# hsinnan75/Dart

Hardware: AMD Instinct MI355X
Metric: M paired-end reads/sec (2x101 bp vs GRCh38-sized index), host to host; records bit-identical to CPU dart (higher is better)
Workload: dtype u64/u8 integer

## Files before the change

dart_amd/csrc/dg_api.hip:

```cpp
#include "../../include/dartgpu.h"
#include "dg_common.h"
#include "dg_fm.h"
#include "dg_seedq.h"
#include "dg_chain.h"
#include "dg_report.h"
#include "dg_pair.h"
#include "dg_reseed.h"
#include "dg_sort.h"
#include "dg_samfmt.h"
#include <stdio.h>
#include <stdlib.h>
#include <string.h>
#include <string>
#include <algorithm>
#include <vector>
#include <atomic>
#include <mutex>
#include <chrono>
#include <thread>
#include <condition_variable>
#include <fcntl.h>
#include <unistd.h>
#include <sys/stat.h>

static char g_init_error[512] = "";

#define DG_HW_QUEUES_NEED 16
static_assert(DG_HW_QUEUES_NEED <= 32, "more hardware queues than 32 are not asked for");
static char g_hwq_found[24] = "unset";
static int g_hwq_left = DG_HW_QUEUES_NEED;
__attribute__((constructor)) static void dg_default_hw_queues()
{
    const char *v = getenv("GPU_MAX_HW_QUEUES");
    long have = 0;
    if (v) {
        size_t i = 0;
        for (; v[i] && i + 1 < sizeof g_hwq_found; i++) g_hwq_found[i] = (v[i] > ' ' && v[i] < 127 && v[i] != ';' && v[i] != '=') ? v[i] : '?';
        g_hwq_found[i] = 0;
        if (!i) snprintf(g_hwq_found, sizeof g_hwq_found, "empty");
        char *end = nullptr;
        have = strtol(v, &end, 10);
        if (end == v || *end) have = 0; else if (have > 1000000) have = 1000000;
    }
    if (have < DG_HW_QUEUES_NEED) {
        char b[8];
        snprintf(b, sizeof b, "%d", DG_HW_QUEUES_NEED);
        setenv("GPU_MAX_HW_QUEUES", b, 1);
        have = DG_HW_QUEUES_NEED;
    }
    g_hwq_left = (int)have;
}
static std::atomic<int> g_live_ctx[64];
static std::atomic<bool> g_hwq_warned{false};

template <typename T> struct DBuf {
    T *p = nullptr; size_t cap = 0;
    hipError_t ensure(size_t n) {
        if (n <= cap) return hipSuccess;
        if (p) (void)hipFree(p);
        p = nullptr; cap = 0;
        size_t want = n + n / 8 + 64;
        hipError_t e = hipMalloc((void **)&p, want * sizeof(T));
        if (e == hipSuccess) cap = want;
        return e;
    }
    void release() { if (p) (void)hipFree(p); p = nullptr; cap = 0; }
};

#define N_TIMERS 20
#define N_TOPS 128
enum { TOP_CIG = 0, TOP_SJ, TOP_JOBS, TOP_REPORT_MAIN, TOP_REPORT_JOBS , TOP_HEAVY_UNITS, TOP_SEED_NEXT, TOP_SEED_HEAVY,
       TOP_WORK = 16, TOP_TICKET_PAIR = 17, TOP_TICKET_EMIT = 18, TOP_RESEED_COUNT = 19 , TOP_RESEED_TICKET = 23 , TOP_TICKET_SEED = 26, TOP_RS_POOL = 27, TOP_RS_OUT = 31,
       TOP_ORDER_INFO = 28 , TOP_CLASS_HIST = 32 , TOP_CLASS_FILL = 64  };

struct IndexShared {
    std::mutex mu;
    std::condition_variable cv;
    DIndex ix{};
    std::atomic<uint32_t> gen{1};
    std::thread aids;
    std::atomic<int> aids_state{0};
    char aids_msg[256] = "";
    bool upload_done = false, upload_ok = false;
    void *d_ktab = nullptr, *d_sa_dense = nullptr;
    std::string report, report_out;
    int device = 0;
    uint32_t *d_chr_name_off = nullptr; char *d_chr_names = nullptr; bool chr_names_set = false; uint64_t chr_names_gen = 0;
};

struct dg_ctx {
    int device = 0;
    IndexShared *shared_ix = nullptr; uint32_t ix_gen = 0;
    bool owns_index = true;
    hipStream_t stream = nullptr;
    hipEvent_t ev_dl = nullptr, ev_dl_block = nullptr;
    bool dl_on_copy_stream = false;
    int env_copy_stream = 1;
    hipEvent_t ev_wait = nullptr;
    char err[512] = "";
    DIndex ix{};
    DParams pr{};
    void *d_bwt = nullptr, *d_sa = nullptr, *d_pac = nullptr, *d_lockey = nullptr, *d_locchr = nullptr, *d_chroff = nullptr;
    int n_reads = 0, max_rlen = 0;
    size_t seq_bytes = 0;
    bool enc_ready = false;
    DBuf<unsigned char> seq; DBuf<uint32_t> seq_off; DBuf<uint16_t> rlen; DBuf<uint32_t> enc; DBuf<uint32_t> packed_in, nlist_in;
    DBuf<DHit> hits; DBuf<uint32_t> nhits, nseeds, seed_off, ncand, rep_off, tile_sums, tile_read, slow_units;
    DBuf<SKey> seeds; DBuf<DSeed> work; DBuf<DCand> cands; DBuf<DJob> jobs; DBuf<unsigned long long> job_items, job_pool; DBuf<RsChunkOut> job_outs; DBuf<uint32_t> job_pool_next; DBuf<unsigned long long> items; DBuf<uint32_t> hist, heavy; DBuf<DHeavy> seed_heavy; DBuf<int32_t> seed_heavy_sfail; DBuf<int16_t> chain_picks; DBuf<uint8_t> chain_todo;
    DBuf<dg_read_out> reads_out; DBuf<dg_report_out> reports; DBuf<uint32_t> cigpool, cigfinal;
    DBuf<dg_sj_out> sjpool, sjfinal;
    DBuf<dg_read_c> reads_c; DBuf<dg_report_c> reports_c; DBuf<uint32_t> cig_c;
    DBuf<unsigned char> ws;
    DBuf<unsigned long long> scan_state, scan_trace;
    int wall_khz = 100000;
    uint32_t scan_epoch = 0;
    size_t cap_seeds = 0, cap_rep = 0, cap_work = 0, cap_cig = 0;
    struct SharedCaps { std::atomic<size_t> seeds{0}, rep{0}, work{0}, cig{0}; } *shared_caps = nullptr;
    bool owns_shared_caps = false;
    unsigned long long *d_ctr = nullptr; unsigned int *d_tops = nullptr; int *d_err = nullptr; DSizes *d_sizes = nullptr; unsigned int *d_input_bad = nullptr;
    struct HostTail { DSizes sizes; int err; unsigned int input_bad; unsigned int tops[N_TOPS]; unsigned long long ctr[CTR_STRIDE]; __host__ __device__ uint32_t *sizes_words() { return (uint32_t *)&sizes; } } *h_tail = nullptr;
    bool state_zeroed = false;
    size_t used[3] = {0, 0, 0};
    bool enqueued = false;
    hipEvent_t ev[N_TIMERS + 1]; const char *tname[N_TIMERS]; int n_t = 0; float tms[N_TIMERS];
    uint64_t counters[CTR_N];
    uint64_t reruns_capacity = 0, reruns_scan = 0;
    bool want_compact = true, packed_valid = false;
    DBuf<uint32_t> sam_hdr_off, sam_qual_off, sam_qlen; DBuf<char> sam_hdr, sam_qual, sam_text; DBuf<uint64_t> sam_read_off, sam_tile;
    unsigned long long *d_sam_stat = nullptr, *h_sam_stat = nullptr;
    hipEvent_t ev_sam[2] = {nullptr, nullptr};
    bool batch_done = false, sam_valid = false; size_t sam_bytes = 0;
    size_t env_sam_first_cap = 0;
    bool want_full = true, full_valid = false;
    int n_cu = 256, runs_of_last_batch = 0, attempt_no = 0;
    int env_seed_waves = 4, env_bail_trips = 0 , env_report_bpc = 8, env_no_fast = 0, env_seed_legacy = 0, env_seed_slots_lg = 0, env_seed_wgs = 0, env_blocking_sync = 0;
    int env_seed_phases = 0, env_seed_wg_waves = 4, env_seed_partial = 32, env_seed_multi = 4;
    bool seed_qf_used = false;
    int env_scan_mask = 7;
    int env_chain_bpc = 8, env_seedh_bpc = 8, env_reseed_pct = 100;
    int env_rs_chunk = RS_CHUNK_DIAGS, env_rs_inline = RS_ENT_INLINE, env_rs_pool = 0;
    int env_scan_budget = 0;
};

static void read_env(dg_ctx *c)
{
    auto geti = [](const char *k, int dflt) { const char *v = getenv(k); return v ? atoi(v) : dflt; };
    c->env_seed_waves = geti("DG_SEED_WAVES", 4); c->env_bail_trips = geti("DG_SEED_BAIL_TRIPS", 0);
    c->env_seed_legacy = geti("DG_SEED_LEGACY", 0); c->env_seed_slots_lg = geti("DG_SEED_SLOTS_LG", 0); c->env_seed_wgs = geti("DG_SEED_WGS", 0); c->env_blocking_sync = geti("DG_BLOCKING_SYNC", 0);
    c->env_report_bpc = geti("DG_REPORT_BPC", 8); c->env_no_fast = geti("DG_NO_FAST_PAIR", 0);
    c->env_scan_budget = geti("DG_SCAN_POLL_BUDGET", 0); c->env_scan_mask = geti("DG_SCAN_POLL_SCANS", 7);
    c->env_seed_phases = geti("DG_SEED_PHASES", 0); c->env_seed_wg_waves = geti("DG_SEED_WG_WAVES", 4); c->env_seed_partial = geti("DG_SEED_PARTIAL_MIN", 32);
    c->env_copy_stream = geti("DG_COPY_STREAM", 1);
    c->env_chain_bpc = std::max(1, geti("DG_CHAIN_BPC", 8)); c->env_seedh_bpc = std::max(1, geti("DG_SEEDH_BPC", 8)); c->env_reseed_pct = std::max(10, geti("DG_RESEED_PCT", 100));
    c->env_rs_chunk = geti("DG_RS_CHUNK", RS_CHUNK_DIAGS); c->env_rs_chunk = std::min(1 << 24, std::max(RS_SUPER, c->env_rs_chunk / RS_SUPER * RS_SUPER));
    c->env_rs_inline = std::min(RS_ENT_INLINE, std::max(0, geti("DG_RS_ENT_MAX", RS_ENT_INLINE))); c->env_rs_pool = std::max(0, geti("DG_RS_POOL_BLOCKS", 0));
    c->env_sam_first_cap = (size_t)std::max(0, geti("DG_SAM_TEXT_FIRST_CAP", 0));
    c->env_seed_multi = geti("DG_SEED_MULTI", 4); if (c->env_seed_multi < 0 || c->env_seed_multi > SQF_MULTI_MAX) c->env_seed_multi = SQF_MULTI_MAX;
}

static inline void refresh_index(dg_ctx *c)
{
    IndexShared *sh = c->shared_ix;
    if (sh && c->ix_gen != sh->gen.load(std::memory_order_acquire)) { std::lock_guard<std::mutex> lk(sh->mu); c->ix = sh->ix; c->ix_gen = sh->gen.load(); }
}

static int fail(dg_ctx *c, int code, const char *what, hipError_t e)
{
    snprintf(c ? c->err : g_init_error, 512, "%s: %s", what, e == hipSuccess ? "error" : hipGetErrorString(e));
    return code;
}
#define HIPCHK(call) do { hipError_t _e = (call); if (_e != hipSuccess) return fail(c, DG_ERR_HIP, #call, _e); } while (0)

#define SCAN_TILE 2048
__global__ void __launch_bounds__(256) k_scan_tiles(const uint32_t *in, uint32_t *out, uint32_t *tile_sums, uint32_t n)
{
    __shared__ uint32_t sh[256];
    const uint32_t base = blockIdx.x * SCAN_TILE + threadIdx.x * 8;
    uint32_t v[8], sum = 0;
    for (int i = 0; i < 8; i++) { v[i] = base + i < n ? in[base + i] : 0; sum += v[i]; }
    sh[threadIdx.x] = sum;
    __syncthreads();
    for (int o = 1; o < 256; o <<= 1) {
        uint32_t t = threadIdx.x >= o ? sh[threadIdx.x - o] : 0;
        __syncthreads();
        sh[threadIdx.x] += t;
        __syncthreads();
    }
    uint32_t run = sh[threadIdx.x] - sum;
    for (int i = 0; i < 8; i++) { if (base + i < n) out[base + i] = run; run += v[i]; }
    if (threadIdx.x == 255) tile_sums[blockIdx.x] = sh[255];
}
__global__ void __launch_bounds__(256) k_scan_top(uint32_t *tile_sums, uint32_t n_tiles, uint32_t *total_out, uint32_t *total_copy, uint32_t cap, int *err, int code)
{
    __shared__ uint32_t sh[256];
    __shared__ uint32_t carry;
    if (threadIdx.x == 0) carry = 0;
    __syncthreads();
    for (uint32_t b = 0; b < n_tiles; b += 256) {
        const uint32_t i = b + threadIdx.x;
        const uint32_t v = i < n_tiles ? tile_sums[i] : 0;
        sh[threadIdx.x] = v;
        __syncthreads();
        for (int o = 1; o < 256; o <<= 1) {
            uint32_t t = threadIdx.x >= o ? sh[threadIdx.x - o] : 0;
            __syncthreads();
            sh[threadIdx.x] += t;
            __syncthreads();
        }
        if (i < n_tiles) tile_sums[i] = carry + sh[threadIdx.x] - v;
        __syncthreads();
        if (threadIdx.x == 255) carry += sh[255];
        __syncthreads();
    }
    if (threadIdx.x == 0) {
        *total_out = carry;
        if (total_copy) *total_copy = carry;
        if (err && carry > cap) atomicMax(err, code);
    }
}
__global__ void __launch_bounds__(256) k_scan_add(uint32_t *out, const uint32_t *tile_sums, uint32_t n)
{
    const uint32_t i = blockIdx.x * 256 + threadIdx.x;
    if (i < n) out[i] += tile_sums[i / SCAN_TILE];
}

#define SO_PER 8
__global__ void __launch_bounds__(256)
k_seed_offsets(int n_reads, int paired, const uint32_t *__restrict__ nseeds, uint32_t *__restrict__ seed_off, uint32_t *__restrict__ tile_read, uint32_t n_tile_read,
               uint32_t *__restrict__ heavy_list, unsigned int *n_heavy, uint32_t *total_copy, uint32_t cap, TileScan ts, int *err)
{
    __shared__ unsigned long long s_scan[20];
    __shared__ unsigned int s_tile;
    const unsigned int tile = d_tile_ticket_unless(ts, &s_tile, threadIdx.x == 0 && __hip_atomic_load(err, __ATOMIC_RELAXED, __HIP_MEMORY_SCOPE_AGENT) >= DG_ABORT);
    if (tile == SCAN_LEAVE) return;
    const uint32_t first = tile * (256u * SO_PER) + threadIdx.x * SO_PER;
    uint32_t v[SO_PER], sum = 0;
    if (first + SO_PER <= (uint32_t)n_reads) {
        const uint4 a = *(const uint4 *)(nseeds + first), b = *(const uint4 *)(nseeds + first + 4);
        v[0] = a.x; v[1] = a.y; v[2] = a.z; v[3] = a.w; v[4] = b.x; v[5] = b.y; v[6] = b.z; v[7] = b.w;
    } else {
#pragma unroll
        for (int i = 0; i < SO_PER; i++) v[i] = first + i < (uint32_t)n_reads ? nseeds[first + i] : 0u;
    }
#pragma unroll
    for (int i = 0; i < SO_PER; i++) sum += v[i];
    Triple mine, tot;
    mine.x = sum; mine.y = 0; mine.z = 0; mine.w = 0;
    const Triple inb = d_block_exclusive(mine, tot, s_scan);
    const Triple base = d_tile_exclusive(ts, tile, tot, s_scan + 16, err);
    uint32_t run = base.x + inb.x;
    const int lane = threadIdx.x & 63;
#pragma unroll
    for (int i = 0; i < SO_PER; i++) {
        const uint32_t r = first + i;
        if (r < (uint32_t)n_reads) {
            seed_off[r] = run;
            for (uint32_t t = (run + 63u) >> 6; (t << 6) < run + v[i] && t < n_tile_read; t++) tile_read[t] = r;
        }
        const bool unit_end = paired ? (i & 1) == 1 : true;
        const uint32_t useeds = paired ? ((i & 1) ? v[i - ((i & 1) ? 1 : 0)] + v[i] : 0u) : v[i];
        const bool heavy = unit_end && r < (uint32_t)n_reads && useeds > (uint32_t)UNIT_MAX_SEEDS;
        const unsigned long long m = __ballot(heavy);
        if (m) {
            unsigned int hb = 0;
            const int leader = __ffsll((long long)m) - 1;
            if (lane == leader) hb = atomicAdd(n_heavy, (unsigned int)__popcll(m));
            hb = (unsigned int)__shfl((int)hb, leader, 64);
            if (heavy) heavy_list[hb + (unsigned int)__popcll(m & ((1ull << lane) - 1ull))] = paired ? r >> 1 : r;
        }
        run += v[i];
    }
    if (tile == gridDim.x - 1 && threadIdx.x == 0) {
        const uint32_t total = base.x + tot.x;
        seed_off[n_reads] = total;
        if (total_copy) *total_copy = total;
        if (total > cap) atomicMax(err, DG_E_SEEDS);
    }
}

static std::atomic<uint64_t> g_phase_ns[4];
static void caps_publish(std::atomic<size_t> &a, size_t v) { size_t cur = a.load(); while (cur < v && !a.compare_exchange_weak(cur, v)) { } }
static void caps_adopt(size_t &mine, const std::atomic<size_t> &a) { const size_t v = a.load(); if (v > mine) mine = v; }
static std::mutex g_copy_mu[64];
static hipStream_t g_copy_stream[64][2];
static hipError_t copy_stream(int device, int dir, hipStream_t *out)
{
    hipStream_t &sl = g_copy_stream[device & 63][dir];
    if (!sl) {
        int lo = 0, hi = 0;
        hipError_t e = hipDeviceGetStreamPriorityRange(&lo, &hi);
        if (e == hipSuccess) e = hipStreamCreateWithPriority(&sl, hipStreamNonBlocking, hi);
        if (e != hipSuccess) { sl = nullptr; return e; }
    }
    *out = sl;
    return hipSuccess;
}

static bool host_page_locked(const void *p)
{
    if (!p) return false;
    hipPointerAttribute_t a;
    if (hipPointerGetAttributes(&a, p) != hipSuccess) { (void)hipGetLastError(); return false; }
    return a.type == hipMemoryTypeHost;
}

static hipError_t wait_stream(dg_ctx *c)
{
    if (!c->env_blocking_sync || !c->ev_wait) return hipStreamSynchronize(c->stream);
    const hipError_t e = hipEventRecord(c->ev_wait, c->stream);
    return e != hipSuccess ? e : hipEventSynchronize(c->ev_wait);
}

#ifdef DG_PROFILE_CLASSES
__device__ unsigned long long g_class_cycles[DG_COST_CLASSES + 1], g_class_chunks[DG_COST_CLASSES + 1];
#endif
template <int MINW>
__global__ void __launch_bounds__(64, MINW)
k_report(const DIndex ix, const DParams pr, int n_reads, int paired, const unsigned char *__restrict__ seq,
         const uint32_t *__restrict__ seq_off, const uint16_t *__restrict__ rlen, const uint32_t *__restrict__ seed_off,
         const DJob *__restrict__ jobs, DCand *__restrict__ cands,
         const uint32_t *__restrict__ rep_off, DSeed *__restrict__ work, const unsigned long long *__restrict__ items,
         const uint32_t *__restrict__ n_items_p, dg_report_out *__restrict__ reports, uint32_t *cigpool, uint32_t cigcap,
         unsigned int *tops, unsigned char *ws, const WSLayout L, unsigned long long *ctr, int *err)
{
    const unsigned long long t_wave0 = wall_clock64();
    const int lane = blockIdx.x * blockDim.x + threadIdx.x;
    __shared__ uint32_t lds_pm[64 * PM_LDS_WORDS];
    if (*err >= DG_ABORT) return;
    LaneCtx cx;
#ifdef DG_PROFILE_CLASSES
    __shared__ unsigned long long ph_acc[DG_NCLS * DG_NPHASE], cls_acc[2 * DG_NCLS];
    for (int q = threadIdx.x; q < DG_NCLS * DG_NPHASE; q += 64) ph_acc[q] = 0;
    for (int q = threadIdx.x; q < 2 * DG_NCLS; q += 64) cls_acc[q] = 0;
    __syncthreads();
    cx.ph = ph_acc;
#endif
    cx.lds = lds_pm + (threadIdx.x & 63) * PM_LDS_WORDS;
    cx.ix = &ix; cx.pr = &pr; cx.L = &L;
    cx.ws = ws + (size_t)lane * L.stride;
    cx.n_nw = cx.nw_cells = cx.n_reseed = cx.reseed_w = 0;
    const unsigned int lo = 0u, hi = *n_items_p;
    unsigned int *next = tops + TOP_REPORT_MAIN;
    while (true) {
        unsigned int ticket = 0;
        if ((threadIdx.x & 63) == 0) ticket = atomicAdd(next, 1u);
        ticket = (unsigned int)__shfl((int)ticket, 0, 64);
        const unsigned int base = lo + ticket * 64u;
        if (base >= hi) break;
        const unsigned int idx = base + (threadIdx.x & 63);
        const bool valid = idx < hi;
        const unsigned long long item = valid ? items[idx] : 0ull;
        const int r = (int)(item >> 32);
        const uint32_t ci = (uint32_t)item, rep_i = valid ? rep_off[r] + (ci - seed_off[r]) : 0u;
        DRead rd;
        rd.sub_score = 0; rd.mis_num = 0; rd.mapq = 0;
        cx.seq = seq + seq_off[r]; cx.rlen = rlen[r];
#ifdef DG_PROFILE_CLASSES
        const long long t_begin = clock64();
        cx.cls = (int)(cands[(uint32_t)items[base]].final_n & 31); cx.t_last = t_begin;
#endif
        d_gen_mapping_report(cx, valid, paired ? (r & 1) == 0 : true, rd, cands + ci, valid ? 1 : 0, jobs, work,
                             reports + rep_i, rep_i, cigpool, tops + 0, cigcap, err, 0, 1, true);
#ifdef DG_PROFILE_CLASSES
        if ((threadIdx.x & 63) == 0) { cls_acc[cx.cls] += (unsigned long long)(clock64() - t_begin); cls_acc[DG_NCLS + cx.cls] += 1ull; }
#endif
    }
#ifdef DG_PROFILE_CLASSES
    __syncthreads();
    for (int q = threadIdx.x; q < DG_NCLS * DG_NPHASE; q += 64) if (ph_acc[q]) atomicAdd(&g_phase[q / DG_NPHASE][q % DG_NPHASE], ph_acc[q]);
    if (threadIdx.x < DG_NCLS && cls_acc[DG_NCLS + threadIdx.x]) { atomicAdd(&g_class_cycles[threadIdx.x], cls_acc[threadIdx.x]); atomicAdd(&g_class_chunks[threadIdx.x], cls_acc[DG_NCLS + threadIdx.x]); }
#endif
    d_wave_add(ctr + CTR_NW, cx.n_nw);
    d_wave_add(ctr + CTR_NWCELLS, cx.nw_cells);
    d_wave_add(ctr + CTR_RESEED, cx.n_reseed);
    d_wave_add(ctr + CTR_RESEEDW, cx.reseed_w);
    d_wave_resident(ctr, CTR_WT_REPORT, t_wave0);
}

__global__ void __launch_bounds__(256)
k_finalize(const DIndex ix, const DParams pr, int paired, const uint32_t *__restrict__ slow_units, const DSizes *__restrict__ sizes,
           const uint32_t *__restrict__ seed_off, const DCand *__restrict__ cands, const uint32_t *__restrict__ ncand, const uint32_t *__restrict__ rep_off, const DSeed *__restrict__ work,
           dg_read_out *__restrict__ rout, dg_report_out *__restrict__ reports, dg_sj_out *sjpool, uint32_t sjcap, unsigned int *tops, int *err)
{
    if (*err >= DG_ABORT) return;
    const unsigned int n_units = sizes->n_slow_units;
    for (unsigned int it = blockIdx.x * blockDim.x + threadIdx.x; it < n_units; it += gridDim.x * blockDim.x) {
        const int u = (int)slow_units[it];
        const int nm = paired ? 2 : 1;
        DRead rd[2];
        dg_read_out o[2];
        RepMem<dg_report_out> rp[2];
        for (int m = 0; m < nm; m++) {
            const int r = paired ? 2 * u + m : u;
            const int nc = (int)ncand[r];
            dg_report_out *rep = reports + rep_off[r];
            rd[m].score = 0; rd[m].sub_score = 0; rd[m].mis_num = 0; rd[m].mapq = 0; rd[m].iBest = 0; rd[m].CanNum = nc > 0 ? nc : 1;
            for (int i = 0; i < nc; i++) {
                const int aln = rep[i].aln_score, mis_num = rep[i].flag;
                if (mis_num) rep[i].flag = 0;
                if (aln <= 0) continue;
                if (aln > rd[m].score) { rd[m].iBest = i; rd[m].mis_num = mis_num; rd[m].sub_score = rd[m].score; rd[m].score = aln; }
                else if (aln == rd[m].score) rd[m].sub_score = rd[m].score;
            }
            o[m].score = rd[m].score; o[m].sub_score = rd[m].sub_score; o[m].mis_num = rd[m].mis_num; o[m].mapq = 0;
            o[m].n_rep = rd[m].CanNum; o[m].best = rd[m].iBest; o[m].rep_off = (int32_t)rep_off[r]; o[m].sj_off = 0; o[m].n_sj = 0;
            rp[m].p = rep;
        }
        if (paired) {
            d_settle_pair(pr, rd[0], rp[0], rd[1], rp[1]);
            d_flag_pair(rd[0], rp[0], rd[1], rp[1]);
        } else d_flag_single(rd[0], rp[0]);
        for (int m = 0; m < nm; m++) {
            const int r = paired ? 2 * u + m : u;
            d_mapq(rd[m], rp[m]);
            o[m].score = rd[m].score; o[m].mapq = rd[m].mapq; o[m].best = rd[m].iBest;
            if (ncand[r] > 0 && (rd[m].mapq == 50 || (pr.all_sj && rd[m].score > 0)))
                d_collect_sj(ix, pr, cands[seed_off[r] + rd[m].iBest], work, r, sjpool, tops + TOP_SJ, sjcap, o[m].sj_off, o[m].n_sj, err);
            rout[r] = o[m];
        }
    }
}

__global__ void __launch_bounds__(256)
k_emit_slow(int paired, const uint32_t *__restrict__ slow_units, DSizes *sizes, dg_read_out *__restrict__ rout, dg_report_out *__restrict__ reports,
            const uint32_t *__restrict__ cigpool, uint32_t *__restrict__ cigfinal, uint32_t cap_cig, const dg_sj_out *__restrict__ sjpool, dg_sj_out *__restrict__ sjfinal,
            TileScan ts, int *err, const uint16_t *__restrict__ rlen, const CompactOut co)
{
    __shared__ unsigned long long s_scan[20];
    __shared__ unsigned int s_tile;
    bool leave = false;
    if (threadIdx.x == 0) { const int e0 = __hip_atomic_load(err, __ATOMIC_RELAXED, __HIP_MEMORY_SCOPE_AGENT); leave = e0 >= DG_ABORT && e0 != DG_E_CIGFINAL; }
    const unsigned int tile = d_tile_ticket_unless(ts, &s_tile, leave);
    if (tile == SCAN_LEAVE) return;
    const unsigned int n_items = sizes->n_slow_units * (paired ? 2u : 1u);
    if (tile > 0 && tile * 256u >= n_items) return;
    const unsigned int it = tile * 256u + threadIdx.x;
    const bool on = it < n_items;
    const int r = on ? (paired ? (int)(2u * slow_units[it >> 1] + (it & 1u)) : (int)slow_units[it]) : 0;
    dg_read_out o;
    o.n_rep = 0; o.rep_off = 0; o.n_sj = 0; o.sj_off = 0;
    if (on) o = rout[r];
    uint32_t ncig = 0, ncigc = 0;
    const uint32_t full_match = on ? (uint32_t)rlen[r] << 4 : 0u;
    for (int i = 0; i < (on ? o.n_rep : 0); i++) {
        const dg_report_out &rp = reports[o.rep_off + i];
        ncig += rp.n_cigar;
        if (co.reads) ncigc += (rp.n_cigar == 1u && cigpool[rp.cigar_off] == full_match) ? 0u : rp.n_cigar;
    }
    Triple mine, tot;
    mine.x = ncig; mine.y = on ? (uint32_t)o.n_sj : 0u; mine.z = 0; mine.w = ncigc;
    const Triple inb = d_block_exclusive(mine, tot, s_scan);
    const Triple base = d_tile_exclusive(ts, tile, tot, s_scan + 16, err);
    const uint32_t cig_fast = sizes->cig_fast, cigc_fast = sizes->pad[2];
    if (on) {
        uint32_t dst = cig_fast + base.x + inb.x, dstc = cigc_fast + base.w + inb.w;
        bool fits = true;
        if ((uint64_t)dst + ncig > cap_cig) atomicMax(err, DG_E_CIGFINAL);
        else for (int i = 0; i < o.n_rep; i++) {
            dg_report_out &rp = reports[o.rep_off + i];
            const uint32_t m = rp.n_cigar, src = rp.cigar_off;
            const bool plain = m == 1u && cigpool[src] == full_match;
            for (uint32_t k = 0; k < m; k++) cigfinal[dst + k] = cigpool[src + k];
            if (co.reads) {
                if (!plain) { for (uint32_t k = 0; k < m; k++) co.cigar[dstc + k] = cigpool[src + k]; dstc += m; }
                dg_report_c q; fits = d_compact_report(rp, plain, true, q) && fits; co.reports[o.rep_off + i] = q;
            }
            rp.cigar_off = dst; dst += m;
        }
        if (o.n_sj > 0) {
            const uint32_t sd = base.y + inb.y;
            for (int k = 0; k < o.n_sj; k++) sjfinal[sd + k] = sjpool[o.sj_off + k];
            rout[r].sj_off = (int32_t)sd;
        }
        if (co.reads) { dg_read_c oc; fits = d_compact_read(o, oc) && fits; co.reads[r] = oc; if (!fits) *co.bad = 1u; }
    }
    const unsigned int last = n_items ? (n_items - 1u) / 256u : 0u;
    if (tile == last && threadIdx.x == 0) { sizes->total_cig = cig_fast + base.x + tot.x; sizes->total_sj = base.y + tot.y; sizes->pad[0] = cigc_fast + base.w + tot.w; }
}

extern "C" void dg_params_default(dg_params *p)
{
    p->max_gaps = 5; p->max_dup = 100; p->max_intron = 500000; p->min_intron = 5;
    p->max_mismatch = 0; p->multi_hit = 0; p->all_sj = 0; p->paired = 0;
}

static void set_params(dg_ctx *c, const dg_params *p)
{
    c->pr.max_gaps = p->max_gaps; c->pr.max_dup = p->max_dup; c->pr.max_intron = p->max_intron; c->pr.min_intron = p->min_intron;
    c->pr.max_mismatch = p->max_mismatch; c->pr.multi_hit = p->multi_hit; c->pr.all_sj = p->all_sj; c->pr.paired = p->paired;
}

extern "C" int dg_set_params(dg_ctx *c, const dg_params *p)
{
    if (!c || !p) return DG_ERR_ARG;
    set_params(c, p);
    read_env(c);
    return DG_OK;
}

extern "C" int dg_device_count(void)
{
    int n = 0;
    return hipGetDeviceCount(&n) == hipSuccess ? n : 0;
}

extern "C" const char *dg_last_error(const dg_ctx *c) { return c ? c->err : g_init_error; }

extern "C" void dg_destroy(dg_ctx *c)
{
    if (!c) return;
    (void)hipSetDevice(c->device);
    if (c->stream) (void)hipStreamSynchronize(c->stream);
    if (c->owns_index && c->shared_ix) {
        IndexShared *sh = c->shared_ix;
        { std::lock_guard<std::mutex> lk(sh->mu); if (!sh->upload_done) { sh->upload_done = true; sh->upload_ok = false; } }
        sh->cv.notify_all();
        if (sh->aids.joinable()) sh->aids.join();
        if (sh->d_ktab) (void)hipFree(sh->d_ktab);
        if (sh->d_sa_dense) (void)hipFree(sh->d_sa_dense);
        if (sh->d_chr_name_off) (void)hipFree(sh->d_chr_name_off);
        if (sh->d_chr_names) (void)hipFree(sh->d_chr_names);
        delete sh; c->shared_ix = nullptr;
    }
    void *ptrs[] = { c->d_bwt, c->d_sa, c->d_pac, c->d_lockey, c->d_locchr, c->d_chroff };
    if (c->owns_index) for (void *p : ptrs) if (p) (void)hipFree(p);
    void *own[] = { c->d_ctr, c->d_tops, c->d_err, c->d_sizes, c->d_input_bad };
    for (void *p : own) if (p) (void)hipFree(p);
    if (c->h_tail) (void)hipHostFree(c->h_tail);
    c->seq.release(); c->seq_off.release(); c->rlen.release(); c->enc.release(); c->packed_in.release(); c->nlist_in.release(); c->hits.release(); c->nhits.release(); c->nseeds.release();
    c->seed_off.release(); c->ncand.release(); c->rep_off.release(); c->tile_sums.release(); c->tile_read.release(); c->slow_units.release();
    c->seeds.release(); c->work.release(); c->cands.release(); c->jobs.release(); c->job_items.release(); c->job_outs.release(); c->job_pool.release(); c->job_pool_next.release(); c->items.release(); c->hist.release(); c->heavy.release(); c->seed_heavy.release(); c->seed_heavy_sfail.release(); c->chain_picks.release(); c->chain_todo.release();
    c->reads_out.release(); c->reports.release(); c->cigpool.release(); c->cigfinal.release(); c->sjpool.release(); c->sjfinal.release();
    c->sam_hdr_off.release(); c->sam_qual_off.release(); c->sam_qlen.release(); c->sam_hdr.release(); c->sam_qual.release(); c->sam_text.release(); c->sam_read_off.release(); c->sam_tile.release();
    if (c->d_sam_stat) (void)hipFree(c->d_sam_stat);
    if (c->h_sam_stat) (void)hipHostFree(c->h_sam_stat);
    for (hipEvent_t e : c->ev_sam) if (e) (void)hipEventDestroy(e);
    c->ws.release(); c->scan_state.release(); c->scan_trace.release(); c->reads_c.release(); c->reports_c.release(); c->cig_c.release();
    for (int i = 0; i <= N_TIMERS; i++) if (c->ev[i]) (void)hipEventDestroy(c->ev[i]);
    if (c->ev_wait) (void)hipEventDestroy(c->ev_wait);
    if (c->ev_dl) (void)hipEventDestroy(c->ev_dl);
    if (c->ev_dl_block) (void)hipEventDestroy(c->ev_dl_block);
    if (c->stream) { (void)hipStreamDestroy(c->stream); g_live_ctx[c->device & 63].fetch_sub(1); }
    if (c->owns_shared_caps) delete c->shared_caps;
    delete c;
}

static hipError_t make_ctx_objects(dg_ctx *c)
{
    hipError_t e;
    for (int i = 0; i <= N_TIMERS; i++) c->ev[i] = nullptr;
    if ((e = hipStreamCreate(&c->stream)) != hipSuccess) return e;
    g_live_ctx[c->device & 63].fetch_add(1);
    if ((e = hipEventCreateWithFlags(&c->ev_wait, hipEventBlockingSync | hipEventDisableTiming)) != hipSuccess ||
        (e = hipEventCreateWithFlags(&c->ev_dl, hipEventDisableTiming)) != hipSuccess || (e = hipEventCreateWithFlags(&c->ev_dl_block, hipEventBlockingSync | hipEventDisableTiming)) != hipSuccess) return e;
    for (int i = 0; i <= N_TIMERS; i++) if ((e = hipEventCreate(&c->ev[i])) != hipSuccess) return e;
    if ((e = hipMalloc((void **)&c->d_ctr, CTR_STRIPES * CTR_STRIDE * 8)) != hipSuccess || (e = hipMalloc((void **)&c->d_tops, N_TOPS * 4)) != hipSuccess ||
        (e = hipMalloc((void **)&c->d_err, 4)) != hipSuccess || (e = hipMalloc((void **)&c->d_sizes, sizeof(DSizes))) != hipSuccess ||
        (e = hipMalloc((void **)&c->d_input_bad, 4)) != hipSuccess) return e;
    if ((e = hipHostMalloc((void **)&c->h_tail, sizeof(dg_ctx::HostTail), hipHostMallocDefault)) != hipSuccess) return e;
    memset(c->h_tail, 0, sizeof(dg_ctx::HostTail));
    { int khz = 0; if (hipDeviceGetAttribute(&khz, hipDeviceAttributeWallClockRate, c->device) == hipSuccess && khz > 0) c->wall_khz = khz; }
    read_env(c);
    return hipSuccess;
}

static double now_s() { return std::chrono::duration<double>(std::chrono::steady_clock::now().time_since_epoch()).count(); }

struct UpSrc { int fd = -1; const uint8_t *mem = nullptr; };
struct UpChunk { UpSrc src; uint64_t src_off; uint8_t *dst; size_t bytes; uint64_t relayout_blocks; };

static hipError_t upload_chunks(int device, const std::vector<UpChunk> &chunks, size_t chunk_cap, int n_threads, std::string &what)
{
    std::atomic<size_t> next{0};
    std::atomic<int> failed{0};
    std::mutex mu;
    hipError_t first = hipSuccess;
    auto fail_with = [&](hipError_t e, const char *w) { std::lock_guard<std::mutex> lk(mu); if (!failed.exchange(1)) { first = e == hipSuccess ? hipErrorUnknown : e; what = w; } };
    auto work = [&]() {
        hipError_t e;
        if ((e = hipSetDevice(device)) != hipSuccess) { fail_with(e, "hipSetDevice (index upload)"); return; }
        hipStream_t s = nullptr; uint8_t *pin[2] = {nullptr, nullptr}; hipEvent_t ev[2] = {nullptr, nullptr}; bool used[2] = {false, false};
        if ((e = hipStreamCreateWithFlags(&s, hipStreamNonBlocking)) != hipSuccess) { fail_with(e, "hipStreamCreate (index upload)"); return; }
        for (int b = 0; b < 2 && e == hipSuccess; b++) {
            if ((e = hipHostMalloc((void **)&pin[b], chunk_cap, hipHostMallocDefault)) == hipSuccess) e = hipEventCreateWithFlags(&ev[b], hipEventDisableTiming);
        }
        if (e != hipSuccess) fail_with(e, "page-locked staging buffers (index upload)");
        int b = 0;
        while (e == hipSuccess && !failed.load()) {
            const size_t i = next.fetch_add(1);
            if (i >= chunks.size()) break;
            const UpChunk &ch = chunks[i];
            if (used[b] && (e = hipEventSynchronize(ev[b])) != hipSuccess) { fail_with(e, "hipEventSynchronize (index upload)"); break; }
            if (ch.src.mem) memcpy(pin[b], ch.src.mem + ch.src_off, ch.bytes);
            else {
                size_t got = 0;
                while (got < ch.bytes) {
                    const ssize_t r = pread(ch.src.fd, pin[b] + got, ch.bytes - got, (off_t)(ch.src_off + got));
                    if (r <= 0) break;
                    got += (size_t)r;
                }
                if (got < ch.bytes) { fail_with(hipErrorUnknown, "an index file is shorter than its header says"); break; }
            }
            if (ch.bytes && (e = hipMemcpyAsync(ch.dst, pin[b], ch.bytes, hipMemcpyHostToDevice, s)) != hipSuccess) { fail_with(e, "hipMemcpyAsync (index upload)"); break; }
            if (ch.relayout_blocks) {
                k_relayout_bwt<<<(unsigned)((ch.relayout_blocks + 255) / 256), 256, 0, s>>>((uint4 *)ch.dst, ch.relayout_blocks);
                if ((e = hipGetLastError()) != hipSuccess) { fail_with(e, "k_relayout_bwt"); break; }
            }
            if ((e = hipEventRecord(ev[b], s)) != hipSuccess) { fail_with(e, "hipEventRecord (index upload)"); break; }
            used[b] = true; b ^= 1;
        }
        if (s && (e = hipStreamSynchronize(s)) != hipSuccess) fail_with(e, "index upload");
        for (int k = 0; k < 2; k++) { if (ev[k]) (void)hipEventDestroy(ev[k]); if (pin[k]) (void)hipHostFree(pin[k]); }
        if (s) (void)hipStreamDestroy(s);
    };
    std::vector<std::thread> th;
    for (int t = 0; t < n_threads; t++) th.emplace_back(work);
    for (auto &t : th) t.join();
    return failed.load() ? first : hipSuccess;
}

static void add_chunks(std::vector<UpChunk> &out, UpSrc src, uint64_t src_off, uint8_t *dst, size_t bytes, size_t chunk, bool relayout, uint64_t total_blocks)
{
    for (size_t o = 0; o < bytes || (relayout && o / 64 < total_blocks); o += chunk) {
        const size_t nb = o < bytes ? std::min(chunk, bytes - o) : 0;
        uint64_t rb = 0;
        if (relayout) { const uint64_t first = o / 64; rb = std::min<uint64_t>(chunk / 64, total_blocks > first ? total_blocks - first : 0); }
        out.push_back(UpChunk{src, src_off + o, dst + o, nb, rb});
    }
}

static void aids_thread(IndexShared *sh, int sa_file_intv, uint64_t n_sa, bool async, uint64_t expected_reads)
{
    auto failed = [&](const char *w, hipError_t e) {
        std::lock_guard<std::mutex> lk(sh->mu);
        snprintf(sh->aids_msg, sizeof sh->aids_msg, "%s: %s", w, hipGetErrorString(e));
        sh->aids_state.store(-1); sh->cv.notify_all();
    };
    hipError_t e;
    if ((e = hipSetDevice(sh->device)) != hipSuccess) return failed("hipSetDevice (aids)", e);
    DIndex ix;
    { std::lock_guard<std::mutex> lk(sh->mu); ix = sh->ix; }
    const uint64_t seq_len = ix.seq_len;
    double t0 = now_s();
    const bool lean = expected_reads != 0 && expected_reads < 400000000ull;
    int intv = seq_len <= (12ull << 30) ? 1 : (seq_len <= (24ull << 30) ? 2 : 4);
    if (lean && intv < 4) intv = 4;
    if (const char *v = getenv("DG_SA_DENSE")) intv = atoi(v);
    const bool want_dense = intv >= 1 && intv < sa_file_intv && (intv & (intv - 1)) == 0 && seq_len < (1ull << 39);
    const uint64_t n_entries = want_dense ? seq_len / (uint64_t)intv + 1 : 0;
    int K = 8;
    while (K < 16 && (1ull << (2 * K)) < seq_len) K++;
    if (lean && K > 14) K = 14;
    if (async) {
        std::unique_lock<std::mutex> lk(sh->mu);
        sh->cv.wait(lk, [&]() { return sh->upload_done; });
        if (!sh->upload_ok) { lk.unlock(); sh->aids_state.store(-1); sh->cv.notify_all(); return; }
    }
    if (want_dense && (e = hipMalloc(&sh->d_sa_dense, n_entries * 8)) != hipSuccess) return failed("hipMalloc dense SA", e);
    {
        size_t free_b = 0, total_b = 0;
        if (hipMemGetInfo(&free_b, &total_b) == hipSuccess)
            while (K > 8 && ((size_t)16 << (2 * K)) + ((size_t)48 << 30) > free_b) K--;
    }
    if (const char *v = getenv("DG_KTAB_K")) K = atoi(v);
    if (K > 16) K = 16;
    if (K >= 2 && (e = hipMalloc(&sh->d_ktab, ((size_t)16) << (2 * K))) != hipSuccess) return failed("hipMalloc k-mer table", e);
    const double t_alloc = now_s() - t0;
    int lo = 0, hi = 0;
    hipStream_t s = nullptr;
    (void)hipDeviceGetStreamPriorityRange(&lo, &hi);
    if ((e = hipStreamCreateWithPriority(&s, hipStreamNonBlocking, lo)) != hipSuccess) return failed("hipStreamCreate (aids)", e);
    {
        std::unique_lock<std::mutex> lk(sh->mu);
        sh->cv.wait(lk, [&]() { return sh->upload_done; });
        if (!sh->upload_ok) { lk.unlock(); (void)hipStreamDestroy(s); sh->aids_state.store(-1); sh->cv.notify_all(); return; }
    }
    double t_dense = 0, t_ktab = 0;
    int n_cu = 256;
    { hipDeviceProp_t prop; if (hipGetDeviceProperties(&prop, sh->device) == hipSuccess && prop.multiProcessorCount > 0) n_cu = prop.multiProcessorCount; }
    int per_cu = 4;
    if (const char *v = getenv("DG_AIDS_WGS_PER_CU")) per_cu = std::max(1, atoi(v));
    const uint64_t grid_cap = async ? (uint64_t)n_cu * (uint64_t)per_cu : (uint64_t)1 << 22;
    if (want_dense) {
// ... 271 lines not shown
    const uint32_t bit = 3u << (30 - 2 * (pos & 15u));
    atomicAnd(&enc[(size_t)r * 2 * W2 + (pos >> 4)], ~bit);
    atomicOr(&enc[(size_t)r * 2 * W2 + W2 + (pos >> 4)], bit);
}

static int enqueue_upload_packed(dg_ctx *c, int n_reads, int rlen_all, const uint16_t *rlen, int words_per_read, const uint32_t *words, const uint32_t *nlist, size_t n_n)
{
    if (!c || n_reads < 0 || words_per_read < 1 || (n_reads > 0 && !words) || (n_n > 0 && !nlist)) return DG_ERR_ARG;
    HIPCHK(hipSetDevice(c->device));
    const int W2 = words_per_read;
    int mx = rlen_all;
    if (rlen) { mx = 0; for (int i = 0; i < n_reads; i++) mx = rlen[i] > mx ? rlen[i] : mx; }
    if (mx > DG_MAX_RLEN || mx > 16 * W2 || (size_t)n_reads * 16 * W2 > 0xFFFFFFF0ull) { snprintf(c->err, 512, "packed batch: read length %d does not fit %d words (or exceeds DG_MAX_RLEN / 2^32 bases)", mx, W2); return DG_ERR_ARG; }
    if (n_reads && (mx + 15) / 16 != W2) { snprintf(c->err, 512, "packed batch: words_per_read must be ceil(longest read / 16) = %d", (mx + 15) / 16); return DG_ERR_ARG; }
    const size_t nw = (size_t)n_reads * W2, bytes = nw * 16;
    c->n_reads = n_reads; c->max_rlen = mx; c->seq_bytes = bytes; c->enqueued = false; c->batch_done = false; c->sam_valid = false;
    HIPCHK(c->seq.ensure(bytes + 64)); HIPCHK(c->seq_off.ensure((size_t)n_reads + 1)); HIPCHK(c->rlen.ensure((size_t)n_reads + 1));
    HIPCHK(c->enc.ensure(2 * nw + 16)); HIPCHK(c->packed_in.ensure(nw + 1)); HIPCHK(c->nlist_in.ensure(n_n + 1));
    c->enc_ready = true;
    if (n_reads == 0) return DG_OK;
    HIPCHK(hipMemcpyAsync(c->packed_in.p, words, nw * 4, hipMemcpyHostToDevice, c->stream));
    if (rlen) HIPCHK(hipMemcpyAsync(c->rlen.p, rlen, (size_t)n_reads * 2, hipMemcpyHostToDevice, c->stream));
    if (n_n) HIPCHK(hipMemcpyAsync(c->nlist_in.p, nlist, n_n * 4, hipMemcpyHostToDevice, c->stream));
    k_unpack<<<(unsigned)((nw + 255) / 256), 256, 0, c->stream>>>(c->packed_in.p, (uint32_t)nw, W2, 1.0 / (double)W2, rlen_all, rlen ? c->rlen.p : nullptr, c->seq.p, c->seq_off.p, c->rlen.p, c->enc.p, c->d_input_bad);
    if (n_n) {
        k_unpack_n<<<(unsigned)((n_n + 255) / 256), 256, 0, c->stream>>>(c->nlist_in.p, (uint32_t)n_n, W2, (uint32_t)(nw * 16), c->seq.p, c->enc.p, c->d_input_bad);
        HIPCHK(hipMemcpyAsync(&c->h_tail->input_bad, c->d_input_bad, 4, hipMemcpyDeviceToHost, c->stream));
    } else c->h_tail->input_bad = 0;
    HIPCHK(hipGetLastError());
    return DG_OK;
}

extern "C" int dg_batch_upload_packed(dg_ctx *c, int n_reads, int rlen_all, const uint16_t *rlen, int words_per_read, const uint32_t *words, const uint32_t *nlist, size_t n_n)
{
    const int rc = enqueue_upload_packed(c, n_reads, rlen_all, rlen, words_per_read, words, nlist, n_n);
    if (rc) return rc;
    HIPCHK(hipStreamSynchronize(c->stream));
    return DG_OK;
}

extern "C" void *dg_host_alloc(size_t bytes)
{
    void *p = nullptr;
    return hipHostMalloc(&p, bytes ? bytes : 1, hipHostMallocDefault) == hipSuccess ? p : nullptr;
}
extern "C" void dg_host_free(void *p) { if (p) (void)hipHostFree(p); }

static WSLayout make_ws_layout(int R)
{
    WSLayout L;
    auto al = [](uint32_t x) { return (x + 15u) & ~15u; };
    uint32_t o = 0;
    const uint32_t nmax = 2u * (uint32_t)R + 32u;
    L.max_rlen = (uint32_t)R;
    L.cig_off = o; L.cig_cap = 4u * (uint32_t)R + 64u; o = al(o + L.cig_cap * 4u);
    L.nwbits_off = o; L.nwbits_words = ((uint32_t)R + 1u) * ((nmax + 7u) / 8u); o = al(o + L.nwbits_words * 4u);
    L.rows_off = o; L.row_cap = (uint32_t)R + 8u; o = al(o + 2u * L.row_cap * 4u);
    L.str_off = o; L.str_cap = al(3u * (uint32_t)R + 64u); o = al(o + 6u * L.str_cap);
    L.kmer_off = o; L.kmer_cap = (uint32_t)R + 8u > 48u ? (uint32_t)R + 8u : 48u; o = al(o + L.kmer_cap * 8u);
    uint32_t rd = 64; while (rd < (uint32_t)R + 1u) rd <<= 1;
    L.ring_diag = rd; L.ring_words = ((uint32_t)R + 64u) / 64u; L.ring_off = o; o = al(o + rd * L.ring_words * 8u);
    L.stride = (o + 255u) & ~255u;
    return L;
}

#define DG_MAX_DEVICES 64
static std::mutex g_lds_mu;
static size_t g_lds_set[2][DG_MAX_DEVICES];
static hipError_t raise_dynamic_lds(const void *fn, int which, int device, size_t lds)
{
    std::lock_guard<std::mutex> lk(g_lds_mu);
    size_t &cur = g_lds_set[which][device & (DG_MAX_DEVICES - 1)];
    if (lds <= cur) return hipSuccess;
    const hipError_t e = hipFuncSetAttribute(fn, hipFuncAttributeMaxDynamicSharedMemorySize, (int)lds);
    if (e == hipSuccess) cur = lds;
    return e;
}

static hipError_t launch_seed(dg_ctx *c, int n, int H, hipEvent_t after_encode = nullptr)
{
    const int W = 2 * ((c->max_rlen + 15) / 16 > 0 ? (c->max_rlen + 15) / 16 : 1);
    hipError_t e = c->enc.ensure((size_t)W * n + 16);
    if (e != hipSuccess) return e;
    int lg = 0;
    while ((1 << lg) < W / 2) lg++;
    if (!c->enc_ready) k_encode<<<(unsigned)((((size_t)n << lg) + 255) / 256), 256, 0, c->stream>>>(c->seq.p, c->seq_off.p, c->rlen.p, n, W, lg, c->enc.p);
    if (after_encode) { e = hipEventRecord(after_encode, c->stream); if (e != hipSuccess) return e; }
    if ((e = c->seed_heavy.ensure((size_t)n + 16)) != hipSuccess) return e;
    unsigned blocks = (unsigned)c->n_cu * (unsigned)c->env_seed_waves;
    if ((size_t)blocks * 64 > (size_t)n) blocks = (unsigned)((n + 63) / 64);
    const bool use_qf = !c->env_seed_legacy && !c->env_seed_phases && W <= 62 && c->pr.max_dup <= 30000;
    const int bail_trips = c->env_bail_trips > 0 ? c->env_bail_trips : (use_qf ? 64 : 128);
    unsigned int *tops = c->d_tops;
    c->seed_qf_used = false;
    if (use_qf) {
        int lg = c->env_seed_slots_lg >= 6 && c->env_seed_slots_lg <= 11 ? c->env_seed_slots_lg : 9;
        int nw = c->env_seed_wg_waves >= 1 && c->env_seed_wg_waves <= 8 ? c->env_seed_wg_waves : 4;
        while (lg > 6 && sqf_lds_bytes(lg, W, nw) > (size_t)156 * 1024) lg--;
        if (c->env_seed_slots_lg == 0) while (lg > 6 && sqf_lds_bytes(lg, W, nw) > (size_t)80 * 1024) lg--;
        const size_t lds = sqf_lds_bytes(lg, W, nw);
        if ((e = raise_dynamic_lds((const void *)k_seed_qf, 0, c->device, lds)) != hipSuccess) return e;
        unsigned per_cu = (unsigned)(((size_t)160 * 1024) / lds);
        if (per_cu * (unsigned)nw > 16u) per_cu = 16u / (unsigned)nw;
        if (per_cu > 2u) per_cu = 2u;
        if (per_cu < 1u) per_cu = 1u;
        if (c->env_seed_wgs > 0) per_cu = (unsigned)c->env_seed_wgs;
        unsigned wgs = (unsigned)c->n_cu * per_cu;
        const unsigned need = (unsigned)(((size_t)n + ((size_t)1 << lg) - 1) >> lg);
        if (wgs > need) wgs = need;
        c->seed_qf_used = true;
        k_seed_qf<<<wgs, nw * 64, lds, c->stream>>>(c->ix, c->pr, c->enc.p, c->rlen.p, n, W, H, lg, c->hits.p, c->nhits.p, c->nseeds.p, tops + TOP_SEED_NEXT,
                                                    c->seed_heavy.p, tops + TOP_SEED_HEAVY, c->d_ctr, bail_trips, c->env_seed_partial, c->env_seed_multi, c->d_err, bail_trips);
    } else
    if (!c->env_seed_legacy && W <= 62) {
        int lg = c->env_seed_slots_lg >= 6 && c->env_seed_slots_lg <= 10 ? c->env_seed_slots_lg : 9;
        while (lg > 6 && sq_lds_bytes(lg, W) > (size_t)80 * 1024) lg--;
        const size_t lds = sq_lds_bytes(lg, W);
        if ((e = raise_dynamic_lds((const void *)k_seed_q, 1, c->device, lds)) != hipSuccess) return e;
        unsigned per_cu = (unsigned)(((size_t)160 * 1024) / lds);
        if (per_cu > 4u) per_cu = 4u;
        if (c->env_seed_wgs > 0) per_cu = (unsigned)c->env_seed_wgs;
        unsigned wgs = (unsigned)c->n_cu * per_cu;
        const unsigned need = (unsigned)(((size_t)n + ((size_t)1 << lg) - 1) >> lg);
        if (wgs > need) wgs = need;
        k_seed_q<<<wgs, SQ_THREADS, lds, c->stream>>>(c->ix, c->pr, c->enc.p, c->rlen.p, n, W, H, lg, c->hits.p, c->nhits.p, c->nseeds.p, tops + TOP_SEED_NEXT,
                                                      c->seed_heavy.p, tops + TOP_SEED_HEAVY, c->d_ctr, bail_trips, c->d_err);
    } else
    if (W <= 78) k_seed<true><<<blocks, 64, ((size_t)2 * W * 64 + 64) * 4, c->stream>>>(c->ix, c->pr, c->enc.p, c->rlen.p, n, W, H, c->hits.p, c->nhits.p, c->nseeds.p, tops + TOP_SEED_NEXT, c->seed_heavy.p, tops + TOP_SEED_HEAVY, c->d_ctr, bail_trips);
    else k_seed<false><<<blocks, 64, 0, c->stream>>>(c->ix, c->pr, c->enc.p, c->rlen.p, n, W, H, c->hits.p, c->nhits.p, c->nseeds.p, tops + TOP_SEED_NEXT, c->seed_heavy.p, tops + TOP_SEED_HEAVY, c->d_ctr, bail_trips);
    if ((e = c->seed_heavy_sfail.ensure((size_t)n + 16)) != hipSuccess) return e;
    k_seed_heavy_walk<<<(unsigned)c->n_cu * 8u, 64, 0, c->stream>>>(c->ix, c->pr, c->enc.p, c->rlen.p, W, c->seed_heavy.p, tops + TOP_SEED_HEAVY, c->seed_heavy_sfail.p, c->d_ctr);
    k_seed_heavy<<<(unsigned)c->n_cu * (unsigned)c->env_seedh_bpc, 64, (size_t)W * 4 + 16, c->stream>>>(c->ix, c->pr, c->enc.p, c->rlen.p, W, H, c->hits.p, c->nhits.p, c->nseeds.p, c->seed_heavy.p, tops + TOP_SEED_HEAVY, c->seed_heavy_sfail.p, c->d_ctr);
    return hipGetLastError();
}

static TileScan make_tile_scan(dg_ctx *c, size_t first_tile, unsigned int *ticket, int which )
{
    TileScan ts;
    ts.w = c->scan_state.p + SCAN_WORDS * first_tile; ts.ticket = ticket; ts.epoch = c->scan_epoch;
    ts.budget = (c->env_scan_budget > 0 && c->attempt_no == 0 && (c->env_scan_mask & which)) ? (uint32_t)c->env_scan_budget : 0u;
    ts.dbg = c->d_sizes->scan_dbg;
    ts.ticks = (unsigned long long)c->wall_khz * 2000ull;
    ts.trace = c->scan_trace.p ? c->scan_trace.p + SCAN_TRACE_WORDS * first_tile : nullptr;
    return ts;
}

#define TICK(name) do { if (c->n_t < N_TIMERS) { c->tname[c->n_t] = name; HIPCHK(hipEventRecord(c->ev[c->n_t + 1], c->stream)); c->n_t++; } } while (0)

static int enqueue_seeding(dg_ctx *c, int n, int H, bool timed, bool paired_units)
{
    HIPCHK(c->hits.ensure((size_t)n * H)); HIPCHK(c->nhits.ensure(n)); HIPCHK(c->nseeds.ensure(n)); HIPCHK(c->seed_off.ensure((size_t)n + 1));
    if (c->shared_caps) caps_adopt(c->cap_seeds, c->shared_caps->seeds);
    if (c->cap_seeds < (size_t)n * 3 + 1024) c->cap_seeds = (size_t)n * 3 + 1024;
    HIPCHK(c->seeds.ensure(c->cap_seeds + 1)); HIPCHK(c->cands.ensure(c->cap_seeds + 1)); HIPCHK(c->tile_read.ensure(c->cap_seeds / 64 + 16));
    if (timed) c->tname[c->n_t] = "k_encode";
    HIPCHK(launch_seed(c, n, H, timed ? c->ev[c->n_t + 1] : nullptr));
    if (timed) { c->n_t++; TICK("k_seed"); }
    {
        const int paired = (paired_units && (n % 2 == 0)) ? 1 : 0;
        HIPCHK(c->heavy.ensure((size_t)n + 16));
        const TileScan ts_seed = make_tile_scan(c, 0, c->d_tops + TOP_TICKET_SEED, 1);
        k_seed_offsets<<<(unsigned)((n + 256 * SO_PER - 1) / (256 * SO_PER)), 256, 0, c->stream>>>(n, paired, c->nseeds.p, c->seed_off.p, c->tile_read.p, (uint32_t)c->tile_read.cap,
                                                                                                 c->heavy.p, c->d_tops + TOP_HEAVY_UNITS, &c->d_sizes->total_seeds, (uint32_t)c->cap_seeds, ts_seed, c->d_err);
        HIPCHK(hipGetLastError());
    }
    if (timed) TICK("seed_offsets");
    k_locate<<<(unsigned)((c->cap_seeds + 255) / 256), 256, 0, c->stream>>>(c->ix, n, H, c->hits.p, c->tile_read.p, c->seed_off.p, c->seeds.p, c->d_ctr, c->d_err);
    HIPCHK(hipGetLastError());
    if (timed) TICK("k_locate");
    return DG_OK;
}

__global__ void __launch_bounds__(256)
k_batch_begin(unsigned long long *ctr, unsigned int *tops, int *err, DSizes *sizes)
{
    for (int i = threadIdx.x; i < CTR_STRIPES * CTR_STRIDE; i += 256) ctr[i] = 0ull;
    if (threadIdx.x < N_TOPS) tops[threadIdx.x] = 0u;
    if (threadIdx.x < (int)(sizeof(DSizes) / 4)) ((uint32_t *)sizes)[threadIdx.x] = 0u;
    if (threadIdx.x == 0) *err = 0;
}

static size_t scan_tiles_seed(int n_reads) { return (size_t)(n_reads + 256 * SO_PER - 1) / (256 * SO_PER) + 1; }
static size_t scan_tiles_pair(int n_units) { return (size_t)(n_units + PU_THREADS - 1) / PU_THREADS + 1; }

__global__ void __launch_bounds__(256)
k_batch_end(DSizes *__restrict__ sizes, int *__restrict__ err, unsigned int *__restrict__ tops, unsigned long long *__restrict__ ctr, dg_ctx::HostTail *out)
{
    const int t = threadIdx.x;
    if (t < (int)(sizeof(DSizes) / 4)) { out->sizes_words()[t] = ((const uint32_t *)sizes)[t]; ((uint32_t *)sizes)[t] = 0u; }
    if (t < N_TOPS) { out->tops[t] = tops[t]; tops[t] = 0u; }
    if (t == 0) { out->err = *err; *err = 0; }
    if (t < CTR_STRIDE) {
        const bool is_max = t == CTR_MAXTRIPS || t == CTR_WTRIPS_MAX;
        unsigned long long v = 0;
        for (int s_ = 0; s_ < CTR_STRIPES; s_++) { const unsigned long long x = ctr[s_ * CTR_STRIDE + t]; ctr[s_ * CTR_STRIDE + t] = 0ull; v = is_max ? (x > v ? x : v) : v + x; }
        out->ctr[t] = v;
    }
}

static int zero_batch_state(dg_ctx *c, int n_reads, int n_units)
{
    if (!c->state_zeroed) {
        k_batch_begin<<<1, 256, 0, c->stream>>>(c->d_ctr, c->d_tops, c->d_err, c->d_sizes);
        HIPCHK(hipGetLastError());
    }
    c->state_zeroed = false;
    const size_t tiles2 = (size_t)(2 * n_units + 255) / 256 + 1;
    const size_t words = SCAN_WORDS * (scan_tiles_seed(n_reads) + scan_tiles_pair(n_units) + tiles2);
    if (words > c->scan_state.cap) {
        HIPCHK(c->scan_state.ensure(words));
        HIPCHK(hipMemsetAsync(c->scan_state.p, 0, c->scan_state.cap * 8, c->stream));
        static_assert(SCAN_TRACE_WORDS == SCAN_WORDS, "the trace array is sized like the state array");
        HIPCHK(c->scan_trace.ensure(c->scan_state.cap));
        HIPCHK(hipMemsetAsync(c->scan_trace.p, 0, c->scan_trace.cap * 8, c->stream));
    }
    c->scan_epoch = (c->scan_epoch + 1u) & 0x3FFFFFFFu;
    if (c->scan_epoch == 0) c->scan_epoch = 1;
    return DG_OK;
}


static int enqueue_run(dg_ctx *c)
{
    const int n = c->n_reads;
    const int paired = (c->pr.paired && (n % 2 == 0)) ? 1 : 0;
    const int n_units = paired ? n / 2 : n;
    refresh_index(c);
    c->n_t = 0;
    const int H = c->max_rlen / 16 + 1;
    const uint32_t nb = (uint32_t)((n + 255) / 256);
    { const int zr = zero_batch_state(c, n, n_units); if (zr) return zr; }
    HIPCHK(hipEventRecord(c->ev[0], c->stream));
    { const int rc = enqueue_seeding(c, n, H, true, c->pr.paired != 0); if (rc) return rc; }

    if (c->shared_caps) { caps_adopt(c->cap_rep, c->shared_caps->rep); caps_adopt(c->cap_cig, c->shared_caps->cig); caps_adopt(c->cap_work, c->shared_caps->work); }
    if (c->cap_rep < (size_t)n + (size_t)n / 4 + 1024) c->cap_rep = (size_t)n + (size_t)n / 4 + 1024;
    if (c->cap_cig < 3 * c->cap_rep) c->cap_cig = 3 * c->cap_rep;
    if (c->cap_work < (size_t)n * 8 + 65536) c->cap_work = (size_t)n * 8 + 65536;
    const size_t cigcap = (size_t)n * 48 + c->cap_rep * (16 + CIG_SLOT) + 4096, sjcap = (size_t)n * 4 + 1024;
    HIPCHK(c->ncand.ensure(n)); HIPCHK(c->rep_off.ensure((size_t)n + 1)); HIPCHK(c->reads_out.ensure(n));
    HIPCHK(c->heavy.ensure((size_t)n_units + 16)); HIPCHK(c->slow_units.ensure((size_t)n_units + 16));
    HIPCHK(c->reports.ensure(c->cap_rep + 1)); HIPCHK(c->work.ensure(c->cap_work + 16)); HIPCHK(c->jobs.ensure(c->cap_seeds + 16));
    const uint32_t rs_out_cap = (uint32_t)std::max<size_t>(16384, (size_t)n / 8), rs_list_cap = (uint32_t)std::min<size_t>(c->jobs.cap + rs_out_cap, 0xFFFFFFF0u);
    HIPCHK(c->job_outs.ensure(rs_out_cap)); HIPCHK(c->job_items.ensure(3 * (size_t)rs_list_cap + 16));
    const uint32_t rs_pool_cap = (uint32_t)std::max<size_t>(16384, (size_t)n / 32);
    HIPCHK(c->job_pool.ensure((size_t)rs_pool_cap * 64)); HIPCHK(c->job_pool_next.ensure(rs_pool_cap));
    HIPCHK(c->cigpool.ensure(cigcap)); HIPCHK(c->cigfinal.ensure(c->cap_cig + 16)); HIPCHK(c->sjpool.ensure(sjcap)); HIPCHK(c->sjfinal.ensure(sjcap));
    HIPCHK(c->items.ensure(c->cap_seeds + 16));
    unsigned int *tops = c->d_tops;

    HIPCHK(c->chain_picks.ensure(c->cap_seeds + 16)); HIPCHK(c->chain_todo.ensure((size_t)n_units + 16));
    k_chain_heavy<<<c->n_cu * c->env_chain_bpc, 64, 0, c->stream>>>(c->ix, c->pr, n_units, paired, c->rlen.p, c->seed_off.p, c->seeds.p, c->cands.p, c->ncand.p,
                                                     c->heavy.p, tops + TOP_HEAVY_UNITS, c->chain_picks.p, c->chain_todo.p, c->d_ctr, c->d_err);
    k_chain_rules<<<c->n_cu * 4, 64, 0, c->stream>>>(paired, c->seed_off.p, c->cands.p, c->ncand.p, c->heavy.p, tops + TOP_HEAVY_UNITS, c->chain_picks.p, c->chain_todo.p, c->d_err);
    HIPCHK(hipGetLastError());
#ifdef DG_PROFILE_CLASSES
    {
        unsigned long long v[3], z = 0;
        HIPCHK(hipStreamSynchronize(c->stream));
        HIPCHK(hipMemcpyFromSymbol(&v[0], HIP_SYMBOL(g_chain_max), 8)); HIPCHK(hipMemcpyFromSymbol(&v[1], HIP_SYMBOL(g_chain_units), 8)); HIPCHK(hipMemcpyFromSymbol(&v[2], HIP_SYMBOL(g_chain_cycles), 8));
        HIPCHK(hipMemcpyToSymbol(HIP_SYMBOL(g_chain_max), &z, 8)); HIPCHK(hipMemcpyToSymbol(HIP_SYMBOL(g_chain_units), &z, 8)); HIPCHK(hipMemcpyToSymbol(HIP_SYMBOL(g_chain_cycles), &z, 8));
        fprintf(stderr, "[chain_heavy] units %llu  mean cycles %llu  max cycles %llu (seeds %llu/%llu cands %llu/%llu)\n", v[1], v[1] ? v[2] / v[1] : 0, v[0] >> 40,
                (v[0] >> 30) & 1023, (v[0] >> 20) & 1023, (v[0] >> 10) & 1023, v[0] & 1023);
    }
#endif
    TICK("k_chain_heavy");
    const size_t tiles_s = scan_tiles_seed(n), tiles = scan_tiles_pair(n_units);
    const TileScan ts_pair = make_tile_scan(c, tiles_s, tops + TOP_TICKET_PAIR, 2), ts_emit = make_tile_scan(c, tiles_s + tiles, tops + TOP_TICKET_EMIT, 4);
    const int try_fast = (c->env_no_fast || c->ix.n_chr > 0xFFFF) ? 0 : 1;
    CompactOut co{nullptr, nullptr, nullptr, nullptr};
    if (c->want_compact) {
        HIPCHK(c->reads_c.ensure((size_t)n + 1)); HIPCHK(c->reports_c.ensure(c->cap_rep + 1)); HIPCHK(c->cig_c.ensure(c->cap_cig + 16));
        co = CompactOut{c->reads_c.p, c->reports_c.p, c->cig_c.p, &c->d_sizes->pad[1]};
    }
    const int W2p = (c->max_rlen + 15) / 16 > 0 ? (c->max_rlen + 15) / 16 : 1;
    const bool packed_pair = c->enc_ready;
    auto launch_pair = [&](auto kernel) {
        kernel<<<(unsigned)((n_units + PU_THREADS - 1) / PU_THREADS), PU_THREADS, 0, c->stream>>>(
            c->ix, c->pr, n_units, paired, try_fast, (c->want_full || !c->want_compact) ? 0 : 2, c->seq.p, c->seq_off.p, c->enc.p, W2p, c->rlen.p, c->seed_off.p, c->seeds.p, c->cands.p, c->ncand.p, c->rep_off.p,
            c->slow_units.p, c->reads_out.p, c->reports.p, c->cigfinal.p, (uint32_t)c->cap_rep, (uint32_t)c->cap_cig, ts_pair, c->d_sizes, tops + TOP_CIG, c->d_ctr, c->d_err, co);
    };
    if (packed_pair) launch_pair(k_pair<true>); else launch_pair(k_pair<false>);
    HIPCHK(hipGetLastError());
    TICK("k_pair");

    const WSLayout L = make_ws_layout(c->max_rlen < 32 ? 32 : c->max_rlen);
    int blocks = c->n_cu * c->env_report_bpc;
    if ((size_t)blocks * 64 > (size_t)n) blocks = (n + 63) / 64;
    {
        const size_t budget = (size_t)12 << 30, per_block = (size_t)64 * L.stride;
        if ((size_t)blocks * per_block > budget) blocks = (int)(budget / per_block);
        if (blocks < 1) blocks = 1;
    }
    HIPCHK(c->ws.ensure((size_t)blocks * 64 * L.stride));
    unsigned slow_grid = (unsigned)c->n_cu * 4u;
    if ((size_t)slow_grid * 256 > (size_t)n) slow_grid = nb;
    k_prep<dg_report_out><<<slow_grid, 256, 0, c->stream>>>(c->pr, paired, c->slow_units.p, c->d_sizes, c->seed_off.p, c->seeds.p, c->cands.p, c->ncand.p, c->work.p, tops + TOP_WORK,
                                             (uint32_t)c->cap_work, c->jobs.p, tops + TOP_JOBS, (uint32_t)c->jobs.cap, c->d_err, c->rlen.p, c->rep_off.p, c->reports.p, tops + TOP_CLASS_HIST,
                                             packed_pair ? c->enc.p : nullptr, W2p, c->seq.p);
    HIPCHK(hipGetLastError());
    TICK("k_prep");
    const uint32_t jobcap = (uint32_t)c->jobs.cap;
    const RsPool rs_pool{c->job_pool.p, c->job_pool_next.p, tops + TOP_RS_POOL, c->env_rs_pool > 0 ? std::min<uint32_t>((uint32_t)c->env_rs_pool, rs_pool_cap) : rs_pool_cap};
    const int rs_gap_max = c->max_rlen - 32, rs_need = rs_gap_max >= 8 ? (rs_gap_max - 8) / 64 + 1 : 1;
    const RsOrder rs_order{c->jobs.p, tops + TOP_JOBS, jobcap, c->job_items.p, rs_list_cap, rs_out_cap, rs_need <= 1 ? 1 : (rs_need <= 2 ? 2 : 4), (uint32_t)c->env_rs_chunk, tops + TOP_RESEED_COUNT, tops + TOP_RS_OUT};
    k_order<<<slow_grid, 256, 0, c->stream>>>(paired, c->slow_units.p, c->d_sizes, c->seed_off.p, c->cands.p, c->ncand.p, tops + TOP_CLASS_HIST, tops + TOP_CLASS_FILL, c->items.p, tops + TOP_ORDER_INFO, rs_order, c->d_err);
    HIPCHK(hipGetLastError());
    TICK("order");
    k_reseed<1><<<c->n_cu * 10 * c->env_reseed_pct / 100, 64, 0, c->stream>>>(c->ix, c->seq.p, c->seq_off.p, c->jobs.p, c->job_items.p, tops + TOP_RESEED_COUNT, tops + TOP_RESEED_COUNT + 3, tops + TOP_RESEED_TICKET, c->job_outs.p, rs_pool, c->env_rs_inline, c->d_ctr, c->d_err);
    if (rs_need > 1) k_reseed<2><<<c->n_cu * 6 * c->env_reseed_pct / 100, 64, 0, c->stream>>>(c->ix, c->seq.p, c->seq_off.p, c->jobs.p, c->job_items.p + rs_list_cap, tops + TOP_RESEED_COUNT + 1, tops + TOP_RESEED_COUNT + 3, tops + TOP_RESEED_TICKET + 1, c->job_outs.p, rs_pool, c->env_rs_inline, c->d_ctr, c->d_err);
    if (rs_need > 2) k_reseed<4><<<c->n_cu * 4 * c->env_reseed_pct / 100, 64, 0, c->stream>>>(c->ix, c->seq.p, c->seq_off.p, c->jobs.p, c->job_items.p + 2 * (size_t)rs_list_cap, tops + TOP_RESEED_COUNT + 2, tops + TOP_RESEED_COUNT + 3, tops + TOP_RESEED_TICKET + 2, c->job_outs.p, rs_pool, c->env_rs_inline, c->d_ctr, c->d_err);
    HIPCHK(hipGetLastError());
    TICK("k_reseed");
    const uint32_t *n_items_p = tops + TOP_ORDER_INFO + 1;
    k_report<2><<<blocks, 64, 0, c->stream>>>(c->ix, c->pr, n, paired, c->seq.p, c->seq_off.p, c->rlen.p, c->seed_off.p, c->jobs.p, c->cands.p,
                                               c->rep_off.p, c->work.p, c->items.p, n_items_p, c->reports.p, c->cigpool.p,
                                               (uint32_t)cigcap, tops, c->ws.p, L, c->d_ctr, c->d_err);
    HIPCHK(hipGetLastError());
#ifdef DG_PROFILE_CLASSES
    {
        unsigned long long cyc[DG_COST_CLASSES + 1], cnt[DG_COST_CLASSES + 1], z[DG_COST_CLASSES + 1] = {0};
        HIPCHK(hipStreamSynchronize(c->stream));
        HIPCHK(hipMemcpyFromSymbol(cyc, HIP_SYMBOL(g_class_cycles), sizeof cyc)); HIPCHK(hipMemcpyFromSymbol(cnt, HIP_SYMBOL(g_class_chunks), sizeof cnt));
        HIPCHK(hipMemcpyToSymbol(HIP_SYMBOL(g_class_cycles), z, sizeof z)); HIPCHK(hipMemcpyToSymbol(HIP_SYMBOL(g_class_chunks), z, sizeof z));
        unsigned long long tot = 0; for (int k = 0; k <= DG_COST_CLASSES; k++) tot += cyc[k];
        unsigned long long ph[DG_NCLS][DG_NPHASE], zp[DG_NCLS][DG_NPHASE] = {{0}};
        HIPCHK(hipMemcpyFromSymbol(ph, HIP_SYMBOL(g_phase), sizeof ph)); HIPCHK(hipMemcpyToSymbol(HIP_SYMBOL(g_phase), zp, sizeof zp));
        for (int k = 0; k < DG_COST_CLASSES; k++) if (cnt[k]) {
            fprintf(stderr, "[class %2d] chunks %7llu  cycles/chunk %8llu  share %5.1f %%  phases/chunk:", k, cnt[k], cyc[k] / cnt[k], 100.0 * cyc[k] / (tot ? tot : 1));
            for (int q = 0; q < DG_NPHASE; q++) fprintf(stderr, " %llu", ph[k][q] / cnt[k]);
            fprintf(stderr, "\n");
        }
    }
#endif
    TICK("k_report");
    k_finalize<<<slow_grid, 256, 0, c->stream>>>(c->ix, c->pr, paired, c->slow_units.p, c->d_sizes, c->seed_off.p, c->cands.p, c->ncand.p, c->rep_off.p, c->work.p,
                                                 c->reads_out.p, c->reports.p, c->sjpool.p, (uint32_t)sjcap, tops, c->d_err);
    k_emit_slow<<<(unsigned)((n + 255) / 256), 256, 0, c->stream>>>(paired, c->slow_units.p, c->d_sizes, c->reads_out.p, c->reports.p, c->cigpool.p, c->cigfinal.p,
                                                                    (uint32_t)c->cap_cig, c->sjpool.p, c->sjfinal.p, ts_emit, c->d_err, c->rlen.p, co);
    HIPCHK(hipGetLastError());
    TICK("k_finalize");
    k_batch_end<<<1, 256, 0, c->stream>>>(c->d_sizes, c->d_err, c->d_tops, c->d_ctr, c->h_tail);
    HIPCHK(hipGetLastError());
    c->state_zeroed = true;
    TICK("tail");
    c->enqueued = true;
    return DG_OK;
}

static int finish_run(dg_ctx *c, size_t used[3])
{
    c->runs_of_last_batch = 0;
    for (int attempt = 0; attempt < 6; attempt++) {
        c->runs_of_last_batch++;
        HIPCHK(wait_stream(c));
        if (c->enc_ready && c->h_tail->input_bad) { snprintf(c->err, 512, "packed batch: the N list holds a position outside the batch"); c->enqueued = false; return DG_ERR_ARG; }
        const DSizes &sz = c->h_tail->sizes;
        const int derr = c->h_tail->err;
        if (derr < DG_ABORT) break;
        auto grow = [](size_t need) { return need + need / 4 + 1024; };
        if (derr == DG_E_SEEDS) c->cap_seeds = grow(sz.total_seeds);
        else if (derr == DG_E_REPORTS) {
            c->cap_rep = std::max(grow(sz.total_rep), 2 * c->cap_rep);
            if (c->cap_cig < 3 * c->cap_rep) c->cap_cig = 3 * c->cap_rep;
        }
        else if (derr == DG_E_WORK) c->cap_work = grow(c->h_tail->tops[TOP_WORK]);
        else if (derr == DG_E_CIGFINAL) c->cap_cig = grow(sz.total_cig > 2 * c->cap_cig ? sz.total_cig : 2 * c->cap_cig);
        if (c->shared_caps) { caps_publish(c->shared_caps->seeds, c->cap_seeds); caps_publish(c->shared_caps->rep, c->cap_rep); caps_publish(c->shared_caps->work, c->cap_work); caps_publish(c->shared_caps->cig, c->cap_cig); }
        if (derr == DG_E_SEEDS || derr == DG_E_REPORTS || derr == DG_E_WORK || derr == DG_E_CIGFINAL) {  }
        else if ((derr == DG_E_SCAN || derr == DG_E_SEEDQ) && attempt < 5) {
            c->reruns_scan++;
            const unsigned long long *d = sz.scan_dbg;
            const double tick_ms = 1.0 / (double)c->wall_khz;
            const bool same_epoch = (d[8] >> 32) == d[5];
            snprintf(c->err, 512, "batch run again (device status %d): look-back of tile %llu gave up on tile %lld after %llu polls / %.1f ms (lane %llu, epoch %llu): words %016llx %016llx %016llx; "
                     "stuck tile's trace: epoch %llu%s HW_ID %08llx (wave %llu simd %llu cu %llu sh %llu se %llu) XCC %llu, ticket %.3f ms before the give-up, own totals %s, prefix %s",
                     derr, d[0] ? d[0] - 1 : 0ull, (long long)d[1], d[6], (double)(d[12] - d[13]) * tick_ms, d[7], d[5], d[2], d[3], d[4],
                     d[8] >> 32, same_epoch ? "" : " (NOT this run's: it never took its ticket here)", d[8] & 0xFFFFFFFFull, d[8] & 15, (d[8] >> 4) & 3, (d[8] >> 8) & 15, (d[8] >> 12) & 1, (d[8] >> 13) & 7, d[11] >> 56,
                     (double)(d[12] - d[9]) * tick_ms, d[10] ? "published" : "NOT published", (d[11] & 0x00FFFFFFFFFFFFFFull) ? "published" : "NOT published");
            if (!c->env_scan_budget) fprintf(stderr, "[libdartgpu] %s\n", c->err);
        }
        else { snprintf(c->err, 512, "device-side scan did not complete (status %d)", derr); return DG_ERR_INTERNAL; }
        if (attempt == 5) { snprintf(c->err, 512, "buffer capacities did not converge (status %d)", derr); return DG_ERR_INTERNAL; }
        if (derr != DG_E_SCAN && derr != DG_E_SEEDQ) c->reruns_capacity++;
        c->attempt_no = attempt + 1;
        const int rc = enqueue_run(c);
        if (rc) return rc;
    }
    c->enqueued = false;
    for (int i = 0; i < c->n_t; i++) { float ms = 0; (void)hipEventElapsedTime(&ms, c->ev[i], c->ev[i + 1]); c->tms[i] = ms; }
    static_assert(CTR_N <= CTR_STRIDE, "the work counters fill one stripe");
    for (int k = 0; k < CTR_N; k++) c->counters[k] = c->h_tail->ctr[k];
    if (c->seed_qf_used) {
        c->counters[CTR_STEPS_ACT] += c->counters[CTR_SQ_LANES + SQ_STEP]; c->counters[CTR_BLOCKS_ACT] += c->counters[CTR_SQ_LANES + SQ_STEP];
        c->counters[CTR_KTAB] += c->counters[CTR_SQ_LANES + SQ_BEGIN]; c->counters[CTR_DIRECT] += c->counters[CTR_SQ_LANES + SQ_LOC] + c->counters[CTR_SQ_LANES + SQ_CMP];
    }
    const DSizes &sz = c->h_tail->sizes;
    c->counters[CTR_SEEDS] = sz.total_seeds;
    const int derr = c->h_tail->err;
    if (derr) { snprintf(c->err, 512, "device pool exhausted (%s)", derr == DG_E_CIGAR ? "cigar" : (derr == DG_E_SJ ? "splice junction" : "reseed jobs")); return DG_ERR_INTERNAL; }
    c->used[0] = sz.total_rep; c->used[1] = sz.total_cig; c->used[2] = sz.total_sj;
    c->packed_valid = c->want_compact; c->full_valid = c->want_full || !c->want_compact;
    if (used) { used[0] = c->used[0]; used[1] = c->used[1]; used[2] = c->used[2]; }
    return DG_OK;
}

extern "C" int dg_batch_run(dg_ctx *c, size_t used[3])
{
    if (!c) return DG_ERR_ARG;
    HIPCHK(hipSetDevice(c->device));
    c->used[0] = c->used[1] = c->used[2] = 0;
    memset(c->counters, 0, sizeof c->counters);
    if (used) used[0] = used[1] = used[2] = 0;
    c->n_t = 0;
    c->packed_valid = false; c->full_valid = false; c->batch_done = false; c->sam_valid = false;
    if (c->n_reads == 0) { c->batch_done = true; return DG_OK; }
    c->attempt_no = 0;
    int rc = enqueue_run(c);
    if (rc) return rc;
    rc = finish_run(c, used);
    c->batch_done = rc == DG_OK;
    return rc;
}

static int enqueue_download(dg_ctx *c, dg_read_out *ro, dg_report_out *po, uint32_t *cig, dg_sj_out *so, const size_t caps[3])
{
    if (caps[0] < c->used[0] || caps[1] < c->used[1] || caps[2] < c->used[2]) {
        snprintf(c->err, 512, "output capacity too small: reports %zu of %zu, cigar ops %zu of %zu, junction tuples %zu of %zu", c->used[0], caps[0], c->used[1], caps[1], c->used[2], caps[2]);
        return DG_ERR_CAPACITY;
    }
    c->dl_on_copy_stream = false;
    if (c->env_copy_stream >= 1 && c->ev_dl && host_page_locked(ro)) {
// ... 294 lines not shown
extern "C" int dg_batch_device_sam(dg_ctx *c, void **ptr, size_t *n_bytes)
{
    if (!c || !ptr || !n_bytes) return DG_ERR_ARG;
    if (!c->sam_valid) { snprintf(c->err, 512, "dg_batch_device_sam: no SAM text (dg_batch_format_sam first)"); return DG_ERR_ARG; }
    *ptr = c->sam_bytes ? c->sam_text.p : nullptr; *n_bytes = c->sam_bytes;
    return DG_OK;
}

__global__ void __launch_bounds__(256)
k_rand_blocks(const uint4 *__restrict__ bwt, uint64_t n_blocks, int iters, int dependent, uint32_t *__restrict__ sink)
{
    uint64_t x = (uint64_t)(blockIdx.x * blockDim.x + threadIdx.x) * 0x9E3779B97F4A7C15ull + 12345;
    uint32_t acc = 0;
    for (int it = 0; it < iters; it++) {
        x ^= x >> 33; x *= 0xff51afd7ed558ccdull; x ^= x >> 33; x *= 0xc4ceb9fe1a85ec53ull; x ^= x >> 33;
        const uint4 *p = bwt + ((x % n_blocks) << 2);
        const uint4 a = p[0], b = p[1], cc = p[2], d = p[3];
        const uint32_t v = a.x ^ b.y ^ cc.z ^ d.w;
        acc += v;
        if (dependent) x += v;
    }
    if (acc == 0x12345678u) sink[0] = acc;
}
__global__ void __launch_bounds__(256)
k_rand_blocks_quad(const uint4 *__restrict__ bwt, uint64_t n_blocks, int iters, int dependent, uint32_t *__restrict__ sink)
{
    const int tid = blockIdx.x * blockDim.x + threadIdx.x;
    uint64_t x = (uint64_t)(tid >> 2) * 0x9E3779B97F4A7C15ull + 12345;
    uint32_t acc = 0;
    for (int it = 0; it < iters; it++) {
        x ^= x >> 33; x *= 0xff51afd7ed558ccdull; x ^= x >> 33; x *= 0xc4ceb9fe1a85ec53ull; x ^= x >> 33;
        const uint4 a = bwt[((x % n_blocks) << 2) + (tid & 3)];
        uint32_t v = a.x ^ a.y ^ a.z ^ a.w;
        v ^= __shfl_xor((int)v, 1, 64); v ^= __shfl_xor((int)v, 2, 64);
        acc += v;
        if (dependent) x += v;
    }
    if (acc == 0x12345678u) sink[0] = acc;
}

extern "C" int dg_debug_random_blocks(dg_ctx *c, int iters, int dependent, int waves_per_cu, float *ms, unsigned long long *n_loads)
{
    if (!c) return DG_ERR_ARG;
    HIPCHK(hipSetDevice(c->device));
    const uint64_t n_blocks = (c->ix.seq_len + 127) / 128;
    const unsigned blocks = (unsigned)(c->n_cu * waves_per_cu / 4);
    hipEvent_t e0, e1;
    HIPCHK(hipEventCreate(&e0)); HIPCHK(hipEventCreate(&e1));
    const int quad = dependent >> 1; dependent &= 1;
    if (quad) k_rand_blocks_quad<<<blocks, 256, 0, c->stream>>>(c->ix.bwt, n_blocks, 4, dependent, (uint32_t *)c->d_err);
    else k_rand_blocks<<<blocks, 256, 0, c->stream>>>(c->ix.bwt, n_blocks, 4, dependent, (uint32_t *)c->d_err);
    HIPCHK(hipEventRecord(e0, c->stream));
    if (quad) k_rand_blocks_quad<<<blocks, 256, 0, c->stream>>>(c->ix.bwt, n_blocks, iters, dependent, (uint32_t *)c->d_err);
    else k_rand_blocks<<<blocks, 256, 0, c->stream>>>(c->ix.bwt, n_blocks, iters, dependent, (uint32_t *)c->d_err);
    HIPCHK(hipEventRecord(e1, c->stream));
    HIPCHK(hipEventSynchronize(e1));
    HIPCHK(hipEventElapsedTime(ms, e0, e1));
    *n_loads = (unsigned long long)blocks * (quad ? 64ull : 256ull) * (unsigned long long)iters;
    (void)hipEventDestroy(e0); (void)hipEventDestroy(e1);
    return DG_OK;
}

extern "C" int dg_debug_jobs(dg_ctx *c, void *out, int cap)
{
    unsigned int n = c->h_tail ? c->h_tail->tops[TOP_JOBS] : 0u;
    if ((int)n > cap) n = (unsigned)cap;
    if (n && hipMemcpy(out, c->jobs.p, (size_t)n * sizeof(DJob), hipMemcpyDeviceToHost) != hipSuccess) return -1;
    return (int)n;
}

extern "C" int dg_last_timings(dg_ctx *c, const char **names, float *ms, int cap)
{
    if (!c) return 0;
    int k = c->n_t < cap ? c->n_t : cap;
    for (int i = 0; i < k; i++) { names[i] = c->tname[i]; ms[i] = c->tms[i]; }
    return k;
}

extern "C" int dg_last_counters(dg_ctx *c, uint64_t *out, int cap)
{
    if (!c) return 0;
    int k = CTR_R4_N < cap ? CTR_R4_N : cap;
    for (int i = 0; i < k; i++) out[i] = c->counters[i];
    const uint64_t extra[5] = { c->h_tail ? c->h_tail->sizes.n_slow_units : 0u, c->h_tail ? c->h_tail->tops[TOP_HEAVY_UNITS] : 0u, (uint64_t)c->runs_of_last_batch,
                                c->reruns_capacity, c->reruns_scan };
    for (int i = 0; i < 5 && k < cap; i++) out[k++] = extra[i];
    for (int i = CTR_R4_N; i < CTR_N && k < cap; i++) out[k++] = c->counters[i];
    return k;
}

extern "C" int dg_debug_scan_trace(dg_ctx *c, int which, uint64_t *out, size_t cap_tiles, size_t *n_tiles, double *ticks_per_ms)
{
    if (!c || !out || !n_tiles || which < 0 || which > 2) return DG_ERR_ARG;
    HIPCHK(hipSetDevice(c->device));
    const int n = c->n_reads, paired = (c->pr.paired && (n % 2 == 0)) ? 1 : 0, n_units = paired ? n / 2 : n;
    const size_t ts = scan_tiles_seed(n), tp = scan_tiles_pair(n_units), te = (size_t)(2 * n_units + 255) / 256 + 1;
    const size_t first = which == 0 ? 0 : (which == 1 ? ts : ts + tp), cnt = (which == 0 ? ts : (which == 1 ? tp : te)) - 1;
    *n_tiles = cnt;
    if (ticks_per_ms) *ticks_per_ms = (double)c->wall_khz;
    if (!c->scan_trace.p || cnt > cap_tiles) return cnt > cap_tiles ? DG_ERR_CAPACITY : DG_ERR_ARG;
    HIPCHK(hipMemcpy(out, c->scan_trace.p + SCAN_TRACE_WORDS * first, cnt * SCAN_TRACE_WORDS * 8, hipMemcpyDeviceToHost));
    return DG_OK;
}

extern "C" int dg_sort_pairs(int device, uint64_t *keys, int64_t *vals, uint64_t *keys_tmp, int64_t *vals_tmp, size_t n, int key_bits)
{
    dg_ctx *c = nullptr;
    if (!keys || !vals || !keys_tmp || !vals_tmp || key_bits < 1 || key_bits > 64 || n >= 0xFFFFF000ull) return DG_ERR_ARG;
    HIPCHK(hipSetDevice(device));
    if (n < 2) return DG_OK;
    const uint32_t tiles = (uint32_t)((n + RS_TILE - 1) / RS_TILE), m = 16u * tiles;
    const uint32_t scan_tiles = (m + SCAN_TILE - 1) / SCAN_TILE;
    uint32_t *hist = nullptr, *sums = nullptr;
    HIPCHK(hipMalloc((void **)&hist, ((size_t)m + 1) * 4));
    if (hipMalloc((void **)&sums, ((size_t)scan_tiles + 1) * 4) != hipSuccess) { (void)hipFree(hist); return DG_ERR_HIP; }
    uint64_t *ka = keys, *kb = keys_tmp; int64_t *va = vals, *vb = vals_tmp;
    hipError_t e = hipSuccess;
    for (int shift = 0; shift < key_bits && e == hipSuccess; shift += 4) {
        k_rs_hist<<<tiles, 256, 0, 0>>>(ka, (uint32_t)n, shift, tiles, hist);
        k_scan_tiles<<<scan_tiles, 256, 0, 0>>>(hist, hist, sums, m);
        k_scan_top<<<1, 256, 0, 0>>>(sums, scan_tiles, hist + m, nullptr, 0, nullptr, 0);
        k_scan_add<<<(m + 255) / 256, 256, 0, 0>>>(hist, sums, m);
        k_rs_scatter<<<tiles, 256, 0, 0>>>(ka, va, kb, vb, (uint32_t)n, shift, tiles, hist);
        e = hipGetLastError();
        std::swap(ka, kb); std::swap(va, vb);
    }
    if (e == hipSuccess && ka != keys) {
        e = hipMemcpyAsync(keys, ka, n * 8, hipMemcpyDeviceToDevice, 0);
        if (e == hipSuccess) e = hipMemcpyAsync(vals, va, n * 8, hipMemcpyDeviceToDevice, 0);
    }
    if (e == hipSuccess) e = hipStreamSynchronize(0);
    (void)hipFree(hist); (void)hipFree(sums);
    if (e != hipSuccess) return fail(nullptr, DG_ERR_HIP, "dg_sort_pairs", e);
    return DG_OK;
}

extern "C" int dg_probe_seeds(dg_ctx *c, int n_reads, const uint32_t *seq_off, const uint16_t *rlen, const char *seq,
                              uint32_t *seed_off, int32_t *rpos, int32_t *slen, int64_t *gpos, size_t cap, size_t *used)
{
    int rc = dg_batch_upload(c, n_reads, seq_off, rlen, seq);
    if (rc) return rc;
    const int n = n_reads;
    if (used) *used = 0;
    if (n == 0) return DG_OK;
    const int H = c->max_rlen / 16 + 1;
    uint32_t total = 0;
    for (int attempt = 0; ; attempt++) {
        c->n_t = 0;
        if ((rc = zero_batch_state(c, n, n))) return rc;
        if ((rc = enqueue_seeding(c, n, H, false, false))) return rc;
        HIPCHK(c->ncand.ensure(n)); HIPCHK(c->rep_off.ensure((size_t)n + 1)); HIPCHK(c->reads_out.ensure(n));
        HIPCHK(c->heavy.ensure((size_t)n + 16)); HIPCHK(c->slow_units.ensure((size_t)n + 16)); HIPCHK(c->reports.ensure(16)); HIPCHK(c->cigfinal.ensure(16));
        HIPCHK(c->chain_picks.ensure(c->cap_seeds + 16)); HIPCHK(c->chain_todo.ensure((size_t)n + 16));
        k_chain_heavy<<<c->n_cu * 4, 64, 0, c->stream>>>(c->ix, c->pr, n, 0, c->rlen.p, c->seed_off.p, c->seeds.p, c->cands.p, c->ncand.p, c->heavy.p, c->d_tops + TOP_HEAVY_UNITS, c->chain_picks.p, c->chain_todo.p, c->d_ctr, c->d_err);
        k_chain_rules<<<c->n_cu * 4, 64, 0, c->stream>>>(0, c->seed_off.p, c->cands.p, c->ncand.p, c->heavy.p, c->d_tops + TOP_HEAVY_UNITS, c->chain_picks.p, c->chain_todo.p, c->d_err);
        const TileScan ts = make_tile_scan(c, scan_tiles_seed(n), c->d_tops + TOP_TICKET_PAIR, 2);
        k_pair<false><<<(unsigned)((n + PU_THREADS - 1) / PU_THREADS), PU_THREADS, 0, c->stream>>>(
            c->ix, c->pr, n, 0, 0, 1, c->seq.p, c->seq_off.p, c->enc.p, 1, c->rlen.p, c->seed_off.p, c->seeds.p, c->cands.p, c->ncand.p, c->rep_off.p,
            c->slow_units.p, c->reads_out.p, c->reports.p, c->cigfinal.p, 0xFFFFFFFFu, 0xFFFFFFFFu, ts, c->d_sizes, c->d_tops + TOP_CIG, c->d_ctr, c->d_err, CompactOut{nullptr, nullptr, nullptr, nullptr});
        HIPCHK(hipGetLastError());
        k_batch_end<<<1, 256, 0, c->stream>>>(c->d_sizes, c->d_err, c->d_tops, c->d_ctr, c->h_tail);
        HIPCHK(hipGetLastError());
        c->state_zeroed = true;
        HIPCHK(hipStreamSynchronize(c->stream));
        total = c->h_tail->sizes.total_seeds;
        if (c->h_tail->err == DG_E_SEEDS && attempt < 3) { c->cap_seeds = (size_t)total + total / 4 + 1024; continue; }
        if (c->h_tail->err) { snprintf(c->err, 512, "dg_probe_seeds: device status %d", c->h_tail->err); return DG_ERR_INTERNAL; }
        break;
    }
    if (used) *used = total;
    if (total > cap) return DG_ERR_CAPACITY;
    std::vector<SKey> h(total);
    HIPCHK(hipMemcpyAsync(seed_off, c->seed_off.p, ((size_t)n + 1) * 4, hipMemcpyDeviceToHost, c->stream));
    if (total) HIPCHK(hipMemcpyAsync(h.data(), c->seeds.p, (size_t)total * sizeof(SKey), hipMemcpyDeviceToHost, c->stream));
    HIPCHK(hipStreamSynchronize(c->stream));
    for (uint32_t i = 0; i < total; i++) { rpos[i] = sk_rpos(h[i]); slen[i] = sk_rlen(h[i]); gpos[i] = sk_gpos(h[i]); }
    return DG_OK;
}

__global__ void __launch_bounds__(64)
k_probe_nw(int n, const uint32_t *a_off, const uint32_t *b_off, const char *a, const char *b, const uint32_t *out_off,
           uint32_t *out_len, char *out_a, char *out_b, unsigned char *ws, const WSLayout L, const DIndex ix, const DParams pr)
{
    const int i = blockIdx.x * blockDim.x + threadIdx.x;
    if (i >= n) return;
    LaneCtx cx;
    cx.ix = &ix; cx.pr = &pr; cx.L = &L; cx.ws = ws + (size_t)i * L.stride; cx.seq = nullptr; cx.rlen = 0; cx.lds = nullptr;
    cx.n_nw = cx.nw_cells = cx.n_reseed = cx.reseed_w = 0;
    out_len[i] = (uint32_t)d_nw(cx, a + a_off[i], (int)(a_off[i + 1] - a_off[i]), b + b_off[i], (int)(b_off[i + 1] - b_off[i]), out_a + out_off[i], out_b + out_off[i]);
}
__global__ void __launch_bounds__(64)
k_probe_nw_strips(int n, const uint32_t *a_off, const uint32_t *b_off, const char *a, const char *b, const uint32_t *out_off,
                  uint32_t *out_len, char *out_a, char *out_b, const DIndex ix, const DParams pr)
{
    __shared__ uint32_t lds_pm[64 * PM_LDS_WORDS];
    const int i = blockIdx.x * blockDim.x + threadIdx.x;
    if (i >= n) return;
    LaneCtx cx;
    cx.ix = &ix; cx.pr = &pr; cx.L = nullptr; cx.ws = nullptr; cx.seq = nullptr; cx.rlen = 0; cx.lds = lds_pm + (threadIdx.x & 63) * PM_LDS_WORDS;
    cx.n_nw = cx.nw_cells = cx.n_reseed = cx.reseed_w = 0;
    const char *pa = a + a_off[i], *pb = b + b_off[i];
    const int m = (int)(a_off[i + 1] - a_off[i]), nn = (int)(b_off[i + 1] - b_off[i]);
    uint64_t w[6] = {0, 0, 0, 0, 0, 0};
    for (int k = 0; k < m; k++) w[k >> 3] |= (uint64_t)(unsigned char)pa[k] << ((k & 7) << 3);
    for (int k = 0; k < nn; k++) w[3 + (k >> 3)] |= (uint64_t)(unsigned char)pb[k] << ((k & 7) << 3);
    PairStr ps; ps.A0 = w[0]; ps.A1 = w[1]; ps.A2 = w[2]; ps.B0 = w[3]; ps.B1 = w[4]; ps.B2 = w[5];
    ColList cl;
    d_pair_nw(cx, m, nn, ps, cl);
    char *oa = out_a + out_off[i], *ob = out_b + out_off[i];
    int x = 0, y = 0;
    for (int p_ = 0; p_ < cl.K; p_++) {
        const uint32_t ty = d_colcode(cl, p_) & 3u;
        oa[p_] = ty == 1 ? '-' : pa[x++];
        ob[p_] = ty == 2 ? '-' : pb[y++];
    }
    out_len[i] = (uint32_t)cl.K;
}
__global__ void __launch_bounds__(64)
k_probe_nw_wave(int n, int all_wide, const uint32_t *a_off, const uint32_t *b_off, const char *a, const uint32_t *out_off,
                uint32_t *out_len, char *out_a, char *out_b, unsigned char *ws, const WSLayout L, const DIndex ix, const DParams pr)
{
    const int i = blockIdx.x * blockDim.x + threadIdx.x, lane = threadIdx.x & 63;
    const bool has = i < n;
    LaneCtx cx;
    cx.ix = &ix; cx.pr = &pr; cx.L = &L; cx.ws = ws + (size_t)(has ? i : 0) * L.stride; cx.seq = nullptr; cx.rlen = 0; cx.lds = nullptr;
    cx.n_nw = cx.nw_cells = cx.n_reseed = cx.reseed_w = 0;
    const int m = has ? (int)(a_off[i + 1] - a_off[i]) : 0, nn = has ? (int)(b_off[i + 1] - b_off[i]) : 0;
    const unsigned char *pa = (const unsigned char *)a + (has ? a_off[i] : 0);
    const int64_t gPos = has ? (int64_t)b_off[i] : 0;
    d_nw_wave(cx, has, pa, m, gPos, nn, lane, all_wide != 0);
    if (has) {
        char *g = ws_str(cx, 0);
        d_ref_fill(ix, gPos, nn, g);
        out_len[i] = (uint32_t)d_tb_traceback(cx, (const char *)pa, m, g, nn, out_a + out_off[i], out_b + out_off[i]);
    }
}

struct DevTmp {
    std::vector<void *> ptrs;
    hipError_t alloc(void **p, size_t bytes) { hipError_t e = hipMalloc(p, bytes ? bytes : 16); if (e == hipSuccess) ptrs.push_back(*p); return e; }
    ~DevTmp() { for (void *p : ptrs) (void)hipFree(p); }
};

extern "C" int dg_probe_nw_mode(dg_ctx *c, int mode, int n, const uint32_t *a_off, const uint32_t *b_off, const char *a, const char *b,
                                uint32_t *out_off, uint32_t *out_len, char *out_a, char *out_b, size_t cap)
{
    if (!c || n < 0 || mode < 0 || mode > 3) return DG_ERR_ARG;
    HIPCHK(hipSetDevice(c->device));
    if (n == 0) return DG_OK;
    size_t tot = 0; int mx = 32;
    for (int i = 0; i < n; i++) {
        const int m = (int)(a_off[i + 1] - a_off[i]), nn = (int)(b_off[i + 1] - b_off[i]);
        out_off[i] = (uint32_t)tot; tot += (size_t)m + nn;
        if (m > mx) mx = m;
        if ((nn + 1) / 2 > mx) mx = (nn + 1) / 2;
        if (mode == 1 && (m > PM_MAX || nn > PM_MAX || m < 1 || nn < 1)) { snprintf(c->err, 512, "dg_probe_nw_mode 1: pair %d is not within %d x %d", i, PM_MAX, PM_MAX); return DG_ERR_ARG; }
    }
    if (tot > cap) return DG_ERR_CAPACITY;
    const size_t la = a_off[n], lb = b_off[n];
    std::vector<uint8_t> pac;
    if (mode >= 2) {
        pac.assign(lb / 4 + 1 + 64, 0);
        for (size_t k = 0; k < lb; k++) {
            const uint8_t code = d_nt4((unsigned char)b[k]);
            if (code > 3) { snprintf(c->err, 512, "dg_probe_nw_mode %d: the genome side must be ACGT (RefSequence holds nothing else)", mode); return DG_ERR_ARG; }
            pac[k >> 2] |= (uint8_t)(code << ((~k & 3) << 1));
        }
    }
    const WSLayout L = make_ws_layout(mx);
    DevTmp tmp;
    unsigned char *d_ws = nullptr, *d_pac = nullptr; char *d_a = nullptr, *d_b = nullptr, *d_oa = nullptr, *d_ob = nullptr; uint32_t *d_off = nullptr;
    const size_t lanes = ((size_t)n + 63) / 64 * 64;
    if (mode != 1) HIPCHK(tmp.alloc((void **)&d_ws, lanes * L.stride));
    HIPCHK(tmp.alloc((void **)&d_a, la + 16)); HIPCHK(tmp.alloc((void **)&d_b, lb + 16));
    HIPCHK(tmp.alloc((void **)&d_oa, tot + 16)); HIPCHK(tmp.alloc((void **)&d_ob, tot + 16)); HIPCHK(tmp.alloc((void **)&d_off, (size_t)(4 * n + 4) * 4));
    uint32_t *d_aoff = d_off, *d_boff = d_off + (n + 1), *d_ooff = d_off + 2 * (n + 1), *d_olen = d_off + 3 * (n + 1);
    HIPCHK(hipMemcpy(d_a, a, la, hipMemcpyHostToDevice)); HIPCHK(hipMemcpy(d_b, b, lb, hipMemcpyHostToDevice));
    HIPCHK(hipMemcpy(d_aoff, a_off, (size_t)(n + 1) * 4, hipMemcpyHostToDevice)); HIPCHK(hipMemcpy(d_boff, b_off, (size_t)(n + 1) * 4, hipMemcpyHostToDevice));
    HIPCHK(hipMemcpy(d_ooff, out_off, (size_t)n * 4, hipMemcpyHostToDevice));
    const unsigned nblk = (unsigned)((n + 63) / 64);
    if (mode == 0) k_probe_nw<<<nblk, 64, 0, c->stream>>>(n, d_aoff, d_boff, d_a, d_b, d_ooff, d_olen, d_oa, d_ob, d_ws, L, c->ix, c->pr);
    else if (mode == 1) k_probe_nw_strips<<<nblk, 64, 0, c->stream>>>(n, d_aoff, d_boff, d_a, d_b, d_ooff, d_olen, d_oa, d_ob, c->ix, c->pr);
    else {
        HIPCHK(tmp.alloc((void **)&d_pac, pac.size()));
        HIPCHK(hipMemcpy(d_pac, pac.data(), pac.size(), hipMemcpyHostToDevice));
        DIndex fx = c->ix;
        fx.pac = d_pac; fx.l_pac = (int64_t)lb;
        k_probe_nw_wave<<<nblk, 64, 0, c->stream>>>(n, mode == 3 ? 1 : 0, d_aoff, d_boff, d_a, d_ooff, d_olen, d_oa, d_ob, d_ws, L, fx, c->pr);
    }
    HIPCHK(hipGetLastError());
    HIPCHK(hipStreamSynchronize(c->stream));
    HIPCHK(hipMemcpy(out_len, d_olen, (size_t)n * 4, hipMemcpyDeviceToHost));
    HIPCHK(hipMemcpy(out_a, d_oa, tot, hipMemcpyDeviceToHost)); HIPCHK(hipMemcpy(out_b, d_ob, tot, hipMemcpyDeviceToHost));
    return DG_OK;
}

extern "C" int dg_probe_nw(dg_ctx *c, int n, const uint32_t *a_off, const uint32_t *b_off, const char *a, const char *b,
                           uint32_t *out_off, uint32_t *out_len, char *out_a, char *out_b, size_t cap)
{
    return dg_probe_nw_mode(c, 0, n, a_off, b_off, a, b, out_off, out_len, out_a, out_b, cap);
}
```

dart_amd/csrc/dg_chain.h:

```cpp
#pragma once
#include "dg_common.h"

__host__ __device__ inline void d_sort_keys(SKey *a, int n)
{
    if (n <= 24) {
        for (int i = 1; i < n; i++) {
            const SKey x = a[i];
            int j = i;
            for (; j > 0 && a[j - 1] > x; j--) a[j] = a[j - 1];
            a[j] = x;
        }
        return;
    }
    auto sift = [&](SKey x, int root, int end) {
        for (int ch = 2 * root + 1; ch < end; ch = 2 * root + 1) {
            if (ch + 1 < end && a[ch] < a[ch + 1]) ch++;
            if (!(x < a[ch])) break;
            a[root] = a[ch]; root = ch;
        }
        a[root] = x;
    };
    for (int st = n / 2 - 1; st >= 0; st--) sift(a[st], st, n);
    for (int end = n - 1; end > 0; end--) { const SKey x = a[end]; a[end] = a[0]; sift(x, 0, end); }
}

template <class KeyAt, class Emit>
__host__ __device__ inline int d_cluster_seeds(const LocTab &lt, const DParams &pr, int rlen, int num, KeyAt key, Emit emit)
{
    const int need = (int)(rlen * 0.3);
    int made = 0, head = 0;
    while (head < num && sk_diag(key(head)) < 0) head++;
    while (head < num) {
        SKey tail = key(head);
        const int64_t d_head = sk_diag(tail);
        int covered = sk_rlen(tail), next = head + 1;
        for (; next < num; next++) {
            const SKey cand = key(next);
            int64_t jump = sk_diag(cand) - sk_diag(tail);
            if (jump < 0) jump = -jump;
            bool joins = jump < pr.max_gaps;
            if (!joins && jump < pr.max_intron)
                joins = sk_gpos(cand) < lt.key[d_loc_lower_bound(lt, sk_gpos(tail))] && sk_rpos(cand) > sk_rpos(tail);
            if (!joins) break;
            covered += sk_rlen(cand);
            tail = cand;
        }
        if (covered > need) { emit(head, next - head, covered, d_head < 0 ? (int64_t)0 : d_head); made++; }
        head = next;
    }
    return made;
}
template <class KeyAt, class Emit>
__host__ __device__ inline int d_cluster_seeds(const DIndex &ix, const DParams &pr, int rlen, int num, KeyAt key, Emit emit)
{
    return d_cluster_seeds(d_loc_tab(ix), pr, rlen, num, key, emit);
}

__host__ __device__ __forceinline__ void d_top2_push(int &top, int &runner, int sc)
{
    if (sc == runner) runner = top;
    else if (sc > runner) { const int t = top; top = t > sc ? t : sc; runner = t < sc ? t : sc; }
}
template <class V>
__host__ __device__ inline void d_keep_top(V &v)
{
    const int n = v.n();
    if (n < 2) return;
    int top = 0, runner = 0;
    for (int i = 0; i < n; i++) d_top2_push(top, runner, v.score(i));
    const int cut = (top == runner || top - runner > 20) ? top : runner;
    for (int i = 0; i < n; i++) if (v.score(i) < cut) v.set_score(i, 0);
}

template <class V1, class V2>
__host__ __device__ inline bool d_pair_mates(V1 &a, V2 &b)
{
    const int na = a.n(), nb = b.n();
    if (na * nb > 1000) { d_keep_top(a); d_keep_top(b); }
    bool formed = false;
    for (int i = 0; i < na; i++) {
        const int mine = a.score(i);
        if (mine == 0) continue;
        const int64_t here = a.diag(i);
        int pick = -1;
        int64_t reach = 2000000;
        for (int j = 0; j < nb; j++) {
            if (b.score(j) == 0) continue;
            const int64_t ahead = b.diag(j) - here;
            if (ahead >= 0 && ahead < reach) { reach = ahead; pick = j; }
        }
        if (pick < 0) continue;
        const int holder = b.mate(pick);
        if (holder < 0) formed = true;
        else if (mine > a.score(holder)) a.set_mate(holder, -1);
        else continue;
        a.set_mate(i, pick); b.set_mate(pick, i);
    }
    return formed;
}

template <class V1, class V2>
__host__ __device__ inline void d_settle_mates(V1 &a, V2 &b)
{
    for (int i = 0, na = a.n(); i < na; i++) {
        const int m = a.mate(i);
        if (m < 0) { a.set_score(i, 0); continue; }
        const int sum = a.score(i) + b.score(m);
        a.set_score(i, sum); b.set_score(m, sum);
    }
    for (int j = 0, nb = b.n(); j < nb; j++) if (b.mate(j) < 0) b.set_score(j, 0);
}

template <class V1, class V2>
__host__ __device__ inline void d_candidate_rules(bool paired, V1 &a, V2 &b)
{
    if (paired) {
        if (d_pair_mates(a, b)) d_settle_mates(a, b);
        d_keep_top(a); d_keep_top(b);
    } else d_keep_top(a);
}

struct CandMem {
    DCand *c; int cnt;
    __host__ __device__ int n() const { return cnt; }
    __host__ __device__ int score(int i) const { return c[i].Score; }
    __host__ __device__ void set_score(int i, int v) { c[i].Score = v; }
    __host__ __device__ int64_t diag(int i) const { return c[i].PosDiff; }
    __host__ __device__ int mate(int i) const { return c[i].PairedIdx; }
    __host__ __device__ void set_mate(int i, int v) { c[i].PairedIdx = v; }
};

__host__ __device__ __forceinline__ DCand d_new_cand(uint32_t first_abs, int count, int score, int64_t pos_diff)
{
    DCand c;
    c.PosDiff = pos_diff; c.first = (int32_t)first_abs; c.count = count; c.Score = score; c.PairedIdx = -1; c.SJtype = -1;
    c.work_off = 0; c.final_n = 0; c.n_a = 0; c.job_first = 0; c.job_count = 0;
    return c;
}

__host__ __device__ inline int d_gen_candidates(const DIndex &ix, const DParams &pr, int rlen, const SKey *s, int num, uint32_t base, DCand *out)
{
    int k = 0;
    return d_cluster_seeds(ix, pr, rlen, num, [&](int i) { return s[i]; },
                           [&](int first, int count, int score, int64_t pd) { out[k++] = d_new_cand(base + (uint32_t)first, count, score, pd); });
}

__host__ __device__ __forceinline__ uint32_t d_work_need(int count) { return 14u * (uint32_t)count + 8u; }

#ifndef UNIT_MAX_SEEDS
#define UNIT_MAX_SEEDS 16
#endif
__device__ __forceinline__ bool d_unit_is_heavy(const uint32_t *seed_off, int paired, int u)
{
    const int r1 = paired ? 2 * u : u;
    return seed_off[r1 + (paired ? 2 : 1)] - seed_off[r1] > UNIT_MAX_SEEDS;
}

#define CH_MAXS 1024
#define CH_MAXC 192
#define CH_LOC_MAX 64

__device__ inline int d_gen_candidates_wave(const LocTab &lt, const DParams &pr, int rlen, const SKey *s, int num, uint32_t base, DCand *out,
                                            uint32_t *pref, unsigned long long *starts, int lane)
{
    const int need = (int)(rlen * 0.3), rounds = (num + 63) >> 6;
    int head0 = num;
    for (int r = 0; r < rounds && head0 == num; r++) {
        const int i = r * 64 + lane;
        const unsigned long long m = __ballot(i < num && sk_diag(s[i]) >= 0);
        if (m) head0 = r * 64 + __ffsll((long long)m) - 1;
    }
    uint32_t run = 0;
    if (lane == 0) pref[0] = 0;
    for (int r = 0; r < rounds; r++) {
        const int i = r * 64 + lane;
        bool start = false;
        uint32_t len = 0;
        if (i < num && i >= head0) {
            const SKey cand = s[i];
            len = (uint32_t)sk_rlen(cand);
            if (i == head0) start = true;
            else {
                const SKey tail = s[i - 1];
                int64_t jump = sk_diag(cand) - sk_diag(tail);
                if (jump < 0) jump = -jump;
                bool joins = jump < pr.max_gaps;
                if (!joins && jump < pr.max_intron)
                    joins = sk_gpos(cand) < lt.key[d_loc_lower_bound(lt, sk_gpos(tail))] && sk_rpos(cand) > sk_rpos(tail);
                start = !joins;
            }
        }
        const unsigned long long m = __ballot(start);
        if (lane == 0) starts[r] = m;
        uint32_t incl = len;
        for (int o = 1; o < 64; o <<= 1) { const uint32_t v = (uint32_t)__shfl_up((int)incl, o, 64); if (lane >= o) incl += v; }
        if (i < num) pref[i + 1] = run + incl;
        run += (uint32_t)__shfl((int)incl, 63, 64);
    }
    __syncthreads();
    int made = 0;
    for (int r = 0; r < rounds; r++) {
        const int i = r * 64 + lane;
        const unsigned long long sm = starts[r];
        const bool start = (sm >> lane) & 1ull;
        int end = num;
        if (start) {
            const unsigned long long later = lane == 63 ? 0ull : sm >> (lane + 1);
            if (later) end = i + 1 + (__ffsll((long long)later) - 1);
            else for (int q = r + 1; q < rounds; q++) if (starts[q]) { end = q * 64 + __ffsll((long long)starts[q]) - 1; break; }
        }
        const int covered = start ? (int)(pref[end] - pref[i]) : 0;
        const bool emit = start && covered > need;
        const unsigned long long em = __ballot(emit);
        if (emit) {
            const int64_t d = sk_diag(s[i]);
            out[made + __popcll(em & ((1ull << lane) - 1ull))] = d_new_cand(base + (uint32_t)i, end - i, covered, d < 0 ? (int64_t)0 : d);
        }
        made += __popcll(em);
    }
    __syncthreads();
    return made;
}

__device__ inline void d_bitonic_sort_keys(SKey *a, int n, int lane)
{
    int m = 1; while (m < n) m <<= 1;
    for (int i = n + lane; i < m; i += 64) a[i] = ~0ull;
    __syncthreads();
    for (int k = 2; k <= m; k <<= 1) {
        for (int j = k >> 1; j > 0; j >>= 1) {
            for (int t = lane; t < m / 2; t += 64) {
                const int i = ((t & ~(j - 1)) << 1) | (t & (j - 1)), l = i | j;
                const bool up = (i & k) == 0;
                const SKey x = a[i], y = a[l];
                if ((y < x) == up) { a[i] = y; a[l] = x; }
            }
            __syncthreads();
        }
    }
}

#ifdef DG_PROFILE_CLASSES
__device__ unsigned long long g_chain_max, g_chain_units, g_chain_cycles;
#endif
struct __attribute__((aligned(8))) CandLite { int64_t PosDiff; int32_t Score, PairedIdx; };
struct CandLiteView {
    CandLite *c; int cnt;
    __host__ __device__ int n() const { return cnt; }
    __host__ __device__ int score(int i) const { return c[i].Score; }
    __host__ __device__ void set_score(int i, int v) { c[i].Score = v; }
    __host__ __device__ int64_t diag(int i) const { return c[i].PosDiff; }
    __host__ __device__ int mate(int i) const { return c[i].PairedIdx; }
    __host__ __device__ void set_mate(int i, int v) { c[i].PairedIdx = v; }
};
#define CH_LDS_SORT (CH_MAXS * 8 + (CH_MAXS + 1) * 4 + 4 + (CH_MAXS / 64) * 8)
#define CH_LDS_PAIR (2 * CH_MAXC * 16 + CH_MAXC * 2)
#define CH_LDS_BYTES (CH_LDS_SORT > CH_LDS_PAIR ? CH_LDS_SORT : CH_LDS_PAIR)
__global__ void __launch_bounds__(64)
k_chain_heavy(const DIndex ix, const DParams pr, int n_units, int paired, const uint16_t *__restrict__ rlen,
              const uint32_t *__restrict__ seed_off, SKey *__restrict__ seeds, DCand *__restrict__ cands,
              uint32_t *__restrict__ ncand, const uint32_t *__restrict__ heavy_list, const unsigned int *__restrict__ n_heavy_p,
              int16_t *__restrict__ picks, uint8_t *__restrict__ todo, unsigned long long *ctr, const int *__restrict__ abort_p)
{
    const unsigned long long t_wave0 = wall_clock64();
    __shared__ __attribute__((aligned(16))) unsigned char s_mem[CH_LDS_BYTES];
    SKey *ls = (SKey *)s_mem;
    uint32_t *s_pref = (uint32_t *)(s_mem + CH_MAXS * 8);
    unsigned long long *s_starts = (unsigned long long *)(s_mem + CH_MAXS * 8 + (CH_MAXS + 1) * 4 + 4);
    CandLite *lc0 = (CandLite *)s_mem, *lc1 = lc0 + CH_MAXC;
    int16_t *s_pick = (int16_t *)(s_mem + 2 * CH_MAXC * 16);
    __shared__ int s_n[2];
    __shared__ int64_t s_lkey[CH_LOC_MAX];
    const bool tab_in_lds = 2 * ix.n_chr <= CH_LOC_MAX;
    if (tab_in_lds) for (int i = threadIdx.x; i < 2 * ix.n_chr; i += 64) s_lkey[i] = ix.loc_key[i];
    __syncthreads();
    const LocTab lt = tab_in_lds ? LocTab{s_lkey, ix.loc_chr, ix.chr_off, 2 * ix.n_chr} : d_loc_tab(ix);
    if (*abort_p >= DG_ABORT) return;
    const int lane = threadIdx.x;
    const unsigned int n_heavy = *n_heavy_p;
    unsigned long long nc_total = 0;
    for (unsigned int hi = blockIdx.x; hi < n_heavy; hi += gridDim.x) {
        const int u = (int)heavy_list[hi];
        const int nm = paired ? 2 : 1;
#ifdef DG_PROFILE_CLASSES
        const long long t_begin = clock64();
#endif
        const int r1 = paired ? 2 * u : u;
        uint32_t b[2] = {0, 0}, n[2] = {0, 0};
        for (int m = 0; m < nm; m++) { b[m] = seed_off[r1 + m]; n[m] = seed_off[r1 + m + 1] - b[m]; }
        __syncthreads();
        for (int m = 0; m < nm; m++) {
            if (n[m] <= 64) {
                SKey key = (uint32_t)lane < n[m] ? seeds[b[m] + lane] : ~0ull;
                int mm = 2; while ((uint32_t)mm < n[m]) mm <<= 1;
                for (int k = 2; k <= mm; k <<= 1)
                    for (int j = k >> 1; j > 0; j >>= 1) {
                        const SKey other = d_u64((uint32_t)__shfl_xor((int)(uint32_t)key, j, 64), (uint32_t)__shfl_xor((int)(uint32_t)(key >> 32), j, 64));
                        const bool keep_small = ((lane & k) == 0) == ((lane & j) == 0);
                        key = (other < key) == keep_small ? other : key;
                    }
                if ((uint32_t)lane < n[m]) { ls[lane] = key; seeds[b[m] + lane] = key; }
                __syncthreads();
                const int made = d_gen_candidates_wave(lt, pr, rlen[r1 + m], ls, (int)n[m], b[m], cands + b[m], s_pref, s_starts, lane);
                if (lane == 0) s_n[m] = made;
            } else if (n[m] <= CH_MAXS) {
                for (uint32_t i = lane; i < n[m]; i += 64) ls[i] = seeds[b[m] + i];
                __syncthreads();
                d_bitonic_sort_keys(ls, (int)n[m], lane);
                for (uint32_t i = lane; i < n[m]; i += 64) seeds[b[m] + i] = ls[i];
                __syncthreads();
                const int made = d_gen_candidates_wave(lt, pr, rlen[r1 + m], ls, (int)n[m], b[m], cands + b[m], s_pref, s_starts, lane);
                if (lane == 0) s_n[m] = made;
            } else if (lane == 0) {
                d_sort_keys(seeds + b[m], (int)n[m]);
                s_n[m] = d_gen_candidates(ix, pr, rlen[r1 + m], seeds + b[m], (int)n[m], b[m], cands + b[m]);
            }
            __syncthreads();
        }
        const int n1 = s_n[0], n2 = paired ? s_n[1] : 0;
        DCand *c1 = cands + b[0], *c2 = paired ? cands + b[1] : nullptr;
        __syncthreads();
        if (paired) {
            const bool stage = n1 <= CH_MAXC && n2 <= CH_MAXC;
            if (stage) {
                for (int i = lane; i < n1; i += 64) { const DCand &c = c1[i]; lc0[i] = CandLite{c.PosDiff, c.Score, c.PairedIdx}; }
                for (int i = lane; i < n2; i += 64) { const DCand &c = c2[i]; lc1[i] = CandLite{c.PosDiff, c.Score, c.PairedIdx}; }
                __syncthreads();
                CandLiteView a1{lc0, n1}, a2{lc1, n2};
                if (n1 * n2 > 1000) { if (lane == 0) { d_keep_top(a1); d_keep_top(a2); } __syncthreads(); }
                for (int i = lane; i < n1; i += 64) {
                    int pick = -1;
                    if (a1.score(i) != 0) {
                        const int64_t here = a1.diag(i);
                        int64_t reach = 2000000;
                        for (int j = 0; j < n2; j++) {
                            if (a2.score(j) == 0) continue;
                            const int64_t ahead = a2.diag(j) - here;
                            if (ahead >= 0 && ahead < reach) { reach = ahead; pick = j; }
                        }
                    }
                    s_pick[i] = (int16_t)pick;
                }
                __syncthreads();
                for (int i = lane; i < n1; i += 64) picks[b[0] + i] = s_pick[i];
                if (n1 * n2 > 1000) {
                    for (int i = lane; i < n1; i += 64) c1[i].Score = lc0[i].Score;
                    for (int i = lane; i < n2; i += 64) c2[i].Score = lc1[i].Score;
                }
                if (lane == 0) todo[hi] = 1;
            } else if (lane == 0) { CandMem a1{c1, n1}, a2{c2, n2}; d_candidate_rules(true, a1, a2); todo[hi] = 0; }
        } else if (lane == 0) todo[hi] = 2;
        __syncthreads();
        if (lane == 0) {
            ncand[r1] = (uint32_t)n1; nc_total += (unsigned long long)n1;
            if (paired) { ncand[r1 + 1] = (uint32_t)n2; nc_total += (unsigned long long)n2; }
#ifdef DG_PROFILE_CLASSES
            const unsigned long long cyc = (unsigned long long)(clock64() - t_begin);
            auto cl = [](unsigned long long v) { return v > 1023 ? 1023ull : v; };
            atomicMax(&g_chain_max, (cyc << 40) | (cl(n[0]) << 30) | (cl(paired ? n[1] : 0) << 20) | (cl(n1) << 10) | cl(n2));
            atomicAdd(&g_chain_units, 1ull); atomicAdd(&g_chain_cycles, cyc);
#endif
        }
    }
    if (lane == 0 && nc_total) atomicAdd(d_ctr_stripe(ctr) + CTR_CANDS, nc_total);
    d_wave_resident(ctr, CTR_WT_CHAIN, t_wave0);
}

__global__ void __launch_bounds__(64)
k_chain_rules(int paired, const uint32_t *__restrict__ seed_off, DCand *__restrict__ cands, const uint32_t *__restrict__ ncand, const uint32_t *__restrict__ heavy_list,
              const unsigned int *__restrict__ n_heavy_p, const int16_t *__restrict__ picks, const uint8_t *__restrict__ todo, const int *__restrict__ abort_p)
{
    if (*abort_p >= DG_ABORT) return;
    const unsigned int n_heavy = *n_heavy_p;
    for (unsigned int hi = blockIdx.x * blockDim.x + threadIdx.x; hi < n_heavy; hi += gridDim.x * blockDim.x) {
        const int what = todo[hi];
        if (what == 0) continue;
        const int u = (int)heavy_list[hi], r1 = paired ? 2 * u : u;
        const uint32_t b0 = seed_off[r1];
        CandMem a1{cands + b0, (int)ncand[r1]};
        if (what == 2) { d_keep_top(a1); continue; }
        const uint32_t b1 = seed_off[r1 + 1];
        CandMem a2{cands + b1, (int)ncand[r1 + 1]};
        bool pairing = false;
        for (int i = 0; i < a1.cnt; i++) {
            const int pick = picks[b0 + i];
            if (pick < 0) continue;
            const int holder = a2.mate(pick);
            if (holder < 0) pairing = true;
            else if (a1.score(i) > a1.score(holder)) a1.set_mate(holder, -1);
            else continue;
            a1.set_mate(i, pick); a2.set_mate(pick, i);
        }
        if (pairing) d_settle_mates(a1, a2);
        d_keep_top(a1); d_keep_top(a2);
    }
}
```

dart_amd/csrc/dg_fm.h:

```cpp
#pragma once
#include "dg_common.h"

struct OccBlock { uint4 q0, q1, q2, q3; };

__device__ __forceinline__ OccBlock d_load_block(const DIndex &ix, uint64_t blk)
{
    const uint4 *p = ix.bwt + (blk << 2);
    OccBlock b;
    b.q0 = p[0]; b.q1 = p[1]; b.q2 = p[2]; b.q3 = p[3];
    return b;
}

__device__ __forceinline__ uint64_t d_sel4(uint64_t a0, uint64_t a1, uint64_t a2, uint64_t a3, int i)
{
    uint64_t lo = (i & 1) ? a1 : a0, hi = (i & 1) ? a3 : a2;
    return (i & 2) ? hi : lo;
}
__device__ __forceinline__ uint64_t d_L2(const DIndex &ix, int i)
{
    return i == 4 ? ix.L2[4] : d_sel4(ix.L2[0], ix.L2[1], ix.L2[2], ix.L2[3], i);
}

__device__ __forceinline__ void d_plane_counts(const uint4 H, const uint4 Lo, uint32_t hmask, uint32_t o, uint32_t &P, uint32_t &Q)
{
    const uint32_t wi = o >> 5;
    const uint32_t pm = (2u << (o & 31)) - 1u;
    const uint32_t m0 = wi == 0 ? pm : 0xFFFFFFFFu;
    const uint32_t m1 = wi == 1 ? pm : (wi > 1 ? 0xFFFFFFFFu : 0u);
    const uint32_t m2 = wi == 2 ? pm : (wi > 2 ? 0xFFFFFFFFu : 0u);
    const uint32_t m3 = wi == 3 ? pm : 0u;
    const uint32_t e0 = (H.x ^ hmask) & m0, e1 = (H.y ^ hmask) & m1, e2 = (H.z ^ hmask) & m2, e3 = (H.w ^ hmask) & m3;
    P = __popc(e0) + __popc(e1) + __popc(e2) + __popc(e3);
    Q = __popc(e0 & Lo.x) + __popc(e1 & Lo.y) + __popc(e2 & Lo.z) + __popc(e3 & Lo.w);
}

__device__ __forceinline__ uint4 d_pick4(bool first, const uint4 a, const uint4 b)
{
    return make_uint4(first ? a.x : b.x, first ? a.y : b.y, first ? a.z : b.z, first ? a.w : b.w);
}
__device__ __forceinline__ void d_occ_pair(const OccBlock B, int b, uint32_t o, uint64_t &cb, uint64_t &cp)
{
    const bool hi = (b & 2) != 0, lo = (b & 1) != 0;
    uint32_t P, Q;
    d_plane_counts(B.q2, B.q3, hi ? 0u : 0xFFFFFFFFu, o, P, Q);
    const uint4 C = d_pick4(hi, B.q1, B.q0);
    const uint64_t c_even = d_u64(C.x, C.y) + (P - Q), c_odd = d_u64(C.z, C.w) + Q;
    cb = lo ? c_odd : c_even;
    cp = lo ? c_even : c_odd;
}

__device__ __forceinline__ uint64_t d_lf(const DIndex &ix, uint64_t k)
{
    if (k == ix.primary) return 0;
    const uint64_t x = k - (k > ix.primary);
    const OccBlock B = d_load_block(ix, x >> 7);
    const uint32_t o = (uint32_t)(x & 127), wi = o >> 5, bit = o & 31;
    const uint32_t hw = wi == 0 ? B.q2.x : wi == 1 ? B.q2.y : wi == 2 ? B.q2.z : B.q2.w;
    const uint32_t lw = wi == 0 ? B.q3.x : wi == 1 ? B.q3.y : wi == 2 ? B.q3.z : B.q3.w;
    const int c = (int)(((hw >> bit) & 1u) * 2u + ((lw >> bit) & 1u));
    uint64_t cb, cp;
    d_occ_pair(B, c, o, cb, cp);
    return d_L2(ix, c) + cb;
}

__global__ void __launch_bounds__(256) k_relayout_bwt(uint4 *blk, uint64_t n_blocks)
{
    const uint64_t b = (uint64_t)blockIdx.x * blockDim.x + threadIdx.x;
    if (b >= n_blocks) return;
    const uint4 s2 = blk[b * 4 + 2], s3 = blk[b * 4 + 3];
    const uint32_t w[8] = { s2.x, s2.y, s2.z, s2.w, s3.x, s3.y, s3.z, s3.w };
    uint32_t H[4] = {0, 0, 0, 0}, L[4] = {0, 0, 0, 0};
#pragma unroll
    for (int q = 0; q < 8; q++) {
        uint32_t h = 0, l = 0;
#pragma unroll
        for (int j = 0; j < 16; j++) {
            const uint32_t sym = (w[q] >> ((15 - j) << 1)) & 3u;
            h |= (sym >> 1) << j;
            l |= (sym & 1u) << j;
        }
        H[q >> 1] |= h << (16 * (q & 1));
        L[q >> 1] |= l << (16 * (q & 1));
    }
    blk[b * 4 + 2] = make_uint4(H[0], H[1], H[2], H[3]);
    blk[b * 4 + 3] = make_uint4(L[0], L[1], L[2], L[3]);
}

typedef uint4 __attribute__((aligned(1))) uint4_a1;
__host__ __device__ __forceinline__ void d_enc4(uint32_t x, uint32_t keep, uint32_t &b8, uint32_t &m8)
{
    const uint32_t u = x & 0xDFDFDFDFu;
    auto nz = [](uint32_t z) { return ((z & 0x7F7F7F7Fu) + 0x7F7F7F7Fu) | z; };
    const uint32_t none = nz(u ^ 0x41414141u) & nz(u ^ 0x43434343u) & nz(u ^ 0x47474747u) & nz(u ^ 0x54545454u);
    const uint32_t inv = ((none & 0x80808080u) >> 7) | (~keep & 0x01010101u);
    const uint32_t code = ((u >> 1) ^ (u >> 2)) & 0x03030303u & ~(inv * 3u);
    b8 = (code * 0x40100401u) >> 24;
    m8 = ((inv * 0x40100401u) >> 24) * 3u;
}

__global__ void __launch_bounds__(256)
k_encode(const unsigned char *__restrict__ seq, const uint32_t *__restrict__ seq_off, const uint16_t *__restrict__ rlen,
         int n_reads, int W, int lg, uint32_t *__restrict__ enc)
{
    const int W2 = W >> 1;
    const size_t t = (size_t)blockIdx.x * blockDim.x + threadIdx.x;
    const size_t rr = t >> lg;
    const int ww = (int)(t & ((1u << lg) - 1u));
    if (rr >= (size_t)n_reads || ww >= W2) return;
    const int r = (int)rr;
    const int left = (int)rlen[r] - ww * 16;
    uint4 q = make_uint4(0, 0, 0, 0);
    if (left > 0) q = *(const uint4_a1 *)(seq + seq_off[r] + ww * 16);
    auto keep = [left](int w) -> uint32_t { const int k = left - 4 * w; return k >= 4 ? 0xFFFFFFFFu : (k <= 0 ? 0u : (1u << (8 * k)) - 1u); };
    uint32_t b0, b1, b2, b3, m0, m1, m2, m3;
    d_enc4(q.x, keep(0), b0, m0); d_enc4(q.y, keep(1), b1, m1); d_enc4(q.z, keep(2), b2, m2); d_enc4(q.w, keep(3), b3, m3);
    enc[(size_t)r * W + ww] = (b0 << 24) | (b1 << 16) | (b2 << 8) | b3;
    enc[(size_t)r * W + W2 + ww] = (m0 << 24) | (m1 << 16) | (m2 << 8) | m3;
}

__device__ __forceinline__ bool d_extend_finish(const DIndex &ix, int c, const OccBlock B, const OccBlock B2, uint64_t kk, uint64_t ll,
                                                uint64_t &x0, uint64_t &x1, uint64_t &x2)
{
    const int b = 3 - c;
    uint64_t tkb, tkp, tlb, tlp;
    d_occ_pair(B, b, (uint32_t)(kk & 127), tkb, tkp);
    const bool same = (ll >> 7) == (kk >> 7);
    OccBlock E;
    E.q0 = d_pick4(same, B.q0, B2.q0); E.q1 = d_pick4(same, B.q1, B2.q1); E.q2 = d_pick4(same, B.q2, B2.q2); E.q3 = d_pick4(same, B.q3, B2.q3);
    d_occ_pair(E, b, (uint32_t)(ll & 127), tlb, tlp);
    const uint64_t n2 = tlb - tkb;
    if (n2 == 0) return false;
    uint64_t above;
    if (b == 0) above = (ll - kk) - n2;
    else if (b == 1) above = (ll - kk) - n2 - (tlp - tkp);
    else if (b == 2) above = tlp - tkp;
    else above = 0;
    x0 = x0 + ((x1 <= ix.primary && x1 + x2 - 1 >= ix.primary) ? 1 : 0) + above;
    x1 = d_L2(ix, b) + 1 + tkb;
    x2 = n2;
    return true;
}
__device__ __forceinline__ void d_extend_rows(const DIndex &ix, uint64_t x1, uint64_t x2, uint64_t &kk, uint64_t &ll)
{
    const uint64_t k = x1 - 1, l = k + x2;
    kk = k - (k >= ix.primary); ll = l - (l >= ix.primary);
}
__device__ __forceinline__ bool d_extend(const DIndex &ix, int c, uint64_t &x0, uint64_t &x1, uint64_t &x2, uint32_t &nblk)
{
    uint64_t kk, ll;
    d_extend_rows(ix, x1, x2, kk, ll);
    const OccBlock B = d_load_block(ix, kk >> 7);
    OccBlock B2;
    B2.q0 = B2.q1 = B2.q2 = B2.q3 = make_uint4(0, 0, 0, 0);
    nblk = 1;
    if ((ll >> 7) != (kk >> 7)) { B2 = d_load_block(ix, ll >> 7); nblk = 2; }
    return d_extend_finish(ix, c, B, B2, kk, ll, x0, x1, x2);
}
__device__ __forceinline__ uint64_t d_lf_finish(const DIndex &ix, const OccBlock B, uint64_t x)
{
    const uint32_t o = (uint32_t)(x & 127), wi = o >> 5, bit = o & 31;
    const uint32_t hw = wi == 0 ? B.q2.x : wi == 1 ? B.q2.y : wi == 2 ? B.q2.z : B.q2.w;
    const uint32_t lw = wi == 0 ? B.q3.x : wi == 1 ? B.q3.y : wi == 2 ? B.q3.z : B.q3.w;
    const int c = (int)(((hw >> bit) & 1u) * 2u + ((lw >> bit) & 1u));
    uint64_t cb, cp;
    d_occ_pair(B, c, o, cb, cp);
    return d_L2(ix, c) + cb;
}

__global__ void __launch_bounds__(256)
k_build_ktab(const DIndex ix, int K, uint64_t *__restrict__ tab)
{
    for (uint64_t id = (uint64_t)blockIdx.x * blockDim.x + threadIdx.x; id < (1ull << (2 * K)); id += (uint64_t)gridDim.x * blockDim.x) {
    int c = (int)((id >> (2 * (K - 1))) & 3u);
    uint64_t x0 = d_L2(ix, c) + 1, x1 = d_L2(ix, 3 - c) + 1, x2 = d_L2(ix, c + 1) - d_L2(ix, c);
    uint32_t steps = 0, blocks = 0;
    for (int i = 1; i < K; i++) {
        c = (int)((id >> (2 * (K - 1 - i))) & 3u);
        uint32_t nb;
        steps++;
        const bool ok = d_extend(ix, c, x0, x1, x2, nb);
        blocks += nb;
        if (!ok) { x2 = 0; break; }
    }
    uint64_t lfc = 0;
    if (x2 == 1 && ix.sa_dense) {
        uint64_t k = x0, st = 0;
        const uint64_t mask = (uint64_t)ix.sa_dense_intv - 1;
        while (k & mask) { k = d_lf(ix, k); st++; }
        const uint64_t e = ix.sa_dense[k >> ix.sa_dense_shift];
        x1 = (st + (e & 0xFFFFFFFFFFull)) & 0xFFFFFFFFFFull;
        lfc = st + (e >> 40);
    }
    uint64_t w0 = (x0 & 0xFFFFFFFFFFull) | ((x1 & 0xFFFFFFull) << 40);
    const bool located = x2 == 1 && ix.sa_dense;
    uint64_t w1 = ((x1 >> 24) & 0xFFFFull) | (((located ? lfc : x2) & 0x7FFFFFFFull) << 16) | ((uint64_t)steps << 47) | ((uint64_t)blocks << 52);
    if (located) w1 |= 1ull << 62;
    if (x2 >> 31) w1 |= 1ull << 63;
    tab[id * 2 + 0] = w0; tab[id * 2 + 1] = w1;
    }
}

#define SEED_REFILL 8

__device__ __forceinline__ uint32_t d_text16_slow(const DIndex &ix, int64_t t, int &nv)
// ... 373 lines not shown
                    if ((d_win16(rm, len - K) >> sft) == 0) {
                        const uint4 e4 = *(const uint4_a4 *)(ix.ktab + (size_t)(d_win16(rb, len - K) >> sft) * 2);
                        const uint64_t w0 = d_u64(e4.x, e4.y), w1 = d_u64(e4.z, e4.w);
                        c.ktab++;
                        if (!(w1 >> 63)) {
                            have = true;
                            if ((w1 >> 62) & 1ull) x2 = 1;
                            else { x2 = (w1 >> 16) & 0x7FFFFFFFull; x0 = w0 & 0xFFFFFFFFFFull; x1 = (w0 >> 40) | ((w1 & 0xFFFFull) << 24); q = len - K; }
                        }
                    }
                }
                if (!have) { const int cc = (int)d_at(rb, q); x0 = d_L2(ix, cc) + 1; x1 = d_L2(ix, 3 - cc) + 1; x2 = d_L2(ix, cc + 1) - d_L2(ix, cc); }
                if (x2 >= thr) {
                    sfail = q;
                    while (q > pos) {
                        const int qq = q - 1;
                        if (d_at(rm, qq)) break;
                        uint64_t y0 = x1, y1 = x0, y2 = x2;
                        uint32_t nb;
                        const bool ok = d_extend(ix, 3 - (int)d_at(rb, qq), y0, y1, y2, nb);
                        c.steps_act++; c.blocks_act += nb;
                        if (!ok || y2 < thr) break;
                        x1 = y0; x0 = y1; x2 = y2; q = qq; sfail = q;
                    }
                }
            }
        }
        sfail_out[hi] = sfail;
    }
    d_wave_add(ctr + CTR_STEPS_ACT, c.steps_act);
    d_wave_add(ctr + CTR_BLOCKS_ACT, c.blocks_act);
    d_wave_add(ctr + CTR_KTAB, c.ktab);
}

__global__ void __launch_bounds__(64)
k_seed_heavy(const DIndex ix, const DParams pr, const uint32_t *__restrict__ enc, const uint16_t *__restrict__ rlen, int W, int H,
             DHit *__restrict__ hits, uint32_t *__restrict__ nhits, uint32_t *__restrict__ nseeds,
             const DHeavy *__restrict__ heavy, const unsigned int *__restrict__ n_heavy_p, const int32_t *__restrict__ sfail_in, unsigned long long *ctr)
{
    const unsigned long long t_wave0 = wall_clock64();
    extern __shared__ uint32_t sh[];
    const int W2 = W >> 1;
    const int lane = threadIdx.x;
    const unsigned int n_heavy = *n_heavy_p;
    SeedCtr c = {0, 0, 0, 0, 0, 0, 0, 0};
    const int K = ix.ktab ? ix.ktab_k : 0;
    const bool direct = ix.sa_dense != nullptr;
    for (unsigned int hi = blockIdx.x; hi < n_heavy; hi += gridDim.x) {
        const DHeavy hv = heavy[hi];
        const int r = (int)hv.read, len = rlen[r], end_pos = len - 13;
        __syncthreads();
        for (int w = lane; w < W; w += 64) sh[w] = enc[(size_t)r * W + w];
        __syncthreads();
        auto rb = [&](int w) -> uint32_t { const uint32_t v = sh[w < W2 ? w : W2 - 1]; return w < W2 ? v : 0u; };
        auto rm = [&](int w) -> uint32_t { const uint32_t v = sh[W2 + (w < W2 ? w : W2 - 1)]; return w < W2 ? v : 0xFFFFFFFFu; };
        int pos = hv.pos, nh = hv.nh;
        uint32_t ns = hv.ns;
        const int sfail = sfail_in[hi];
        while (pos < end_pos) {
            if (pos >= sfail) {
                if (lane == 0) {
                    const unsigned long long n = (unsigned long long)(end_pos - pos), st2 = n * (unsigned long long)((len - pos - 1) + (len - end_pos));
                    c.steps += st2 / 2; c.blocks += st2;
                }
                pos = end_pos;
                break;
            }
            Search s; s.mode = 0; s.hit_len = 0; s.located = false; s.ref_steps = s.ref_blocks = 0; s.start = pos + lane; s.x2 = 0; s.x0 = 0; s.tpos = 0; s.lsteps = 0; s.lk = 0;
            const int st = pos + lane;
            const bool doomed = st >= sfail && st < end_pos;
            const bool acgt = st < end_pos && st < sfail && d_at(rm, st) == 0;
            {
                TripData t; t.aux = T_NONE;
                TripAddr ta = {nullptr, nullptr, nullptr, nullptr};
                if (acgt) d_begin_issue(ix, K, rb, rm, st, s, c, ta, t);
                d_trip_load(ta, t);
                if (acgt) d_begin_finish(ix, K, rb, s, c, t);
                if (acgt && direct && s.mode == 1 && s.x2 == 1) { s.mode = 3; s.lk = s.x0; s.lsteps = 0; }
                while (__ballot(acgt && s.mode != 0)) {
                    t.aux = T_NONE; ta.pa = ta.pb = ta.p16 = nullptr; ta.p8 = nullptr;
                    const int sel = __popcll(__ballot(acgt && s.mode == 1)) >= __popcll(__ballot(acgt && s.mode == 2)) ? 1 : 2;
                    if (acgt && (s.mode == 3 || s.mode == sel)) d_trip_issue(ix, rm, len, direct, s, c, ta, t);
                    d_trip_load(ta, t);
                    if (t.aux != T_NONE) d_trip_finish(ix, pr, rb, rm, len, s, c, t);
                    if (acgt && direct && s.mode == 1 && s.x2 == 1) { s.mode = 3; s.lk = s.x0; s.lsteps = 0; }
                }
            }
            const int nlim = (pos + 64 < end_pos ? pos + 64 : end_pos) - pos;
            const unsigned long long in_round = nlim >= 64 ? ~0ull : ((1ull << nlim) - 1ull);
            const unsigned long long hitm = __ballot(acgt && s.hit_len > 0) & in_round;
            unsigned long long vis = 0;
            int cur = 0;
            while (cur < nlim) {
                const unsigned long long m = hitm >> cur;
                if (!m) { vis |= in_round & ~((1ull << cur) - 1ull); cur = nlim; break; }
                const int j = cur + (__ffsll((long long)m) - 1);
                vis |= (j >= 63 ? ~0ull : ((1ull << (j + 1)) - 1ull)) & ~((1ull << cur) - 1ull);
                cur = j + __shfl(s.hit_len, j, 64);
            }
            const bool seen = (vis >> lane) & 1ull;
            if (seen && doomed) { c.steps += (unsigned long long)(len - st - 1); c.blocks += 2ull * (unsigned long long)(len - st - 1); }
            if (seen && acgt) { c.steps += s.ref_steps; c.blocks += s.ref_blocks; }
            const unsigned long long vh = vis & hitm;
            if ((vh >> lane) & 1ull) {
                const int at = nh + __popcll(vh & ((1ull << lane) - 1ull));
                if (at < H) {
                    DHit h; h.rPos = (uint16_t)s.start; h.len = (uint16_t)s.hit_len;
                    if (s.located) { h.x0 = (uint64_t)s.tpos; h.freq = 1u | 0x80000000u; c.lf_ref += s.lsteps + (uint32_t)(s.lk >> 40); }
                    else { h.x0 = s.x0; h.freq = (uint32_t)s.x2; }
                    hits[(size_t)r * H + at] = h;
                }
            }
            uint32_t fr = ((vh >> lane) & 1ull) ? (uint32_t)s.x2 : 0u;
            for (int o = 32; o > 0; o >>= 1) fr += (uint32_t)__shfl_xor((int)fr, o, 64);
            nh += __popcll(vh); ns += fr;
            cur += pos;
            pos = cur;
        }
        if (lane == 0) { nhits[r] = (uint32_t)nh; nseeds[r] = ns; }
    }
    d_wave_add(ctr + CTR_STEPS, c.steps);
    d_wave_add(ctr + CTR_BLOCKS, c.blocks);
    d_wave_add(ctr + CTR_STEPS_ACT, c.steps_act);
    d_wave_add(ctr + CTR_BLOCKS_ACT, c.blocks_act);
    d_wave_add(ctr + CTR_KTAB, c.ktab);
    d_wave_add(ctr + CTR_LF, c.lf_ref);
    d_wave_add(ctr + CTR_LF_ACT, c.lf_act);
    d_wave_add(ctr + CTR_DIRECT, c.n_direct);
    d_wave_resident(ctr, CTR_WT_SEEDH, t_wave0);
}

__global__ void __launch_bounds__(256)
k_build_sa_dense(const DIndex ix, int intv, uint64_t n_entries, uint64_t *__restrict__ dense)
{
    const uint64_t smask = (uint64_t)ix.sa_intv - 1, dmask = (uint64_t)intv - 1;
    const uint64_t n_sampled = (ix.seq_len + (uint64_t)ix.sa_intv) / (uint64_t)ix.sa_intv;
    int dsh = 0;
    while ((1 << dsh) < intv) dsh++;
    for (uint64_t q = (uint64_t)blockIdx.x * blockDim.x + threadIdx.x; q < n_sampled; q += (uint64_t)gridDim.x * blockDim.x) {
        const uint64_t r0 = q * (uint64_t)ix.sa_intv;
        if ((r0 >> dsh) < n_entries) dense[r0 >> dsh] = ((ix.sa[q] + 1) & 0xFFFFFFFFFFull);
        uint64_t k = d_lf(ix, r0), T = 1;
        while (k & smask) { k = d_lf(ix, k); T++; }
        const uint64_t base = ix.sa[k / (uint64_t)ix.sa_intv];
        k = d_lf(ix, r0);
        for (uint64_t t = 1; t < T; t++) {
            const uint64_t steps = T - t;
            if (!(k & dmask) && (k >> dsh) < n_entries) dense[k >> dsh] = ((steps + base + 1) & 0xFFFFFFFFFFull) | (steps << 40);
            k = d_lf(ix, k);
        }
    }
}


__global__ void __launch_bounds__(256)
k_locate(const DIndex ix, int n_reads, int H, const DHit *__restrict__ hits, const uint32_t *__restrict__ tile_read,
         const uint32_t *__restrict__ seed_off, SKey *__restrict__ seeds, unsigned long long *ctr, const int *__restrict__ abort_p)
{
    if (*abort_p >= DG_ABORT) return;
    const uint32_t total = seed_off[n_reads];
    const int lane = threadIdx.x & 63;
    const uint32_t tile = blockIdx.x * (blockDim.x >> 6) + (threadIdx.x >> 6);
    const uint32_t u = (tile << 6) + (uint32_t)lane;
    unsigned long long lf = 0, lf_act = 0, nsa = 0;
    if ((tile << 6) < total) {
        int r0 = (int)tile_read[tile];
        const uint32_t u_last = (tile << 6) + 63 < total ? (tile << 6) + 63 : total - 1;
        int r = -1;
        uint32_t first = 0;
        while (true) {
            const int rr = r0 + lane;
            const uint32_t nxt = rr + 1 <= n_reads ? seed_off[rr + 1] : 0xFFFFFFFFu;
            int lo = 0;
#pragma unroll
            for (int step = 32; step > 0; step >>= 1) {
                const uint32_t v = __shfl(nxt, lo + step - 1, 64);
                if (v <= u) lo += step;
            }
            if (__shfl(nxt, lo, 64) <= u) lo++;
            const uint32_t win_end = __shfl(nxt, 63, 64);
            if (r < 0 && u < total && lo < 64) { r = r0 + lo; first = seed_off[r]; }
            if (win_end > u_last) break;
            r0 += 64;
        }
        if (u < total) {
            uint32_t w = u - first;
            const DHit *h = hits + (size_t)r * H;
            uint32_t fr = h->freq;
            while (w >= (fr & 0x7FFFFFFFu)) { w -= fr & 0x7FFFFFFFu; h++; fr = h->freq; }
            uint64_t k = h->x0 + w;
            uint64_t steps = 0, pos;
            if (fr & 0x80000000u) pos = h->x0;
            else if (ix.sa_dense) {
                const uint64_t mask = (uint64_t)ix.sa_dense_intv - 1;
                while (k & mask) { k = d_lf(ix, k); steps++; }
                const uint64_t e = ix.sa_dense[k >> ix.sa_dense_shift];
                pos = steps + (e & 0xFFFFFFFFFFull) - 1;
                lf += steps + (e >> 40); lf_act += steps;
            } else {
                const uint64_t mask = (uint64_t)ix.sa_intv - 1;
                while (k & mask) { k = d_lf(ix, k); steps++; }
                pos = steps + ix.sa[k / (uint64_t)ix.sa_intv];
                lf += steps; lf_act += steps;
            }
            nsa++;
            seeds[u] = sk_make((int64_t)pos, (int)h->rPos, (int)h->len);
        }
    }
    d_wave_add(ctr + CTR_LF, lf);
    d_wave_add(ctr + CTR_LF_ACT, lf_act);
    d_wave_add(ctr + CTR_SA, nsa);
}
```

dart_amd/csrc/dg_pair.h:

```cpp
#pragma once
#include "../../include/dartgpu.h"
#include "dg_common.h"
#include "dg_chain.h"
#include "dg_report.h"

template <class R1, class R2>
__host__ __device__ inline void d_settle_pair(const DParams &pr, DRead &m1, R1 &p1, DRead &m2, R2 &p2)
{
    bool linked = p1.mate(m1.iBest) == m2.iBest;
    if (linked && !pr.multi_hit) return;
    if (!linked && m1.score > 0 && m2.score > 0) {
        int best_sum = 0;
        for (int i = 0; i < m1.CanNum; i++) {
            const int a = p1.aln(i), j = p1.mate(i);
            if (a <= 0 || j < 0) continue;
            const int b = p2.aln(j);
            if (b <= 0) continue;
            linked = true;
            if (a + b > best_sum) { best_sum = a + b; m1.iBest = i; m1.score = a; m2.iBest = j; m2.score = b; }
        }
    }
    if (linked) {
        for (int i = 0; i < m1.CanNum; i++) {
            const int j = p1.mate(i);
// ... 251 lines not shown
        const int slot = n_slot++;
        uint64_t w0 = 0;
        if (aln > 0) {
            const int lb = d_loc_lower_bound(lt, gPos);
            const int chr = lt.chr[lb];
            int64_t pos; int bdir;
            if (gPos < L) { bdir = first ? 1 : 0; pos = gPos + 1 - lt.off[chr]; }
            else { bdir = first ? 0 : 1; pos = lt.key[lb] - end_gPos + 1; }
            if (pos <= 0 || pos > 0xFFFFFFFFll || chr > 0xFFFF) return false;
            w0 = (uint64_t)pos | ((uint64_t)chr << 32) | ((uint64_t)aln << 48) | ((uint64_t)bdir << 60) | (1ull << 61);
            n_cig += 1u + (head > 0) + (tail > 0);
            if (aln > rd.score) { rd.iBest = i; rd.mis_num = mis; rd.sub_score = rd.score; rd.score = aln; }
            else if (aln == rd.score) rd.sub_score = rd.score;
        }
        rw[(2 * slot) * S] = w0;
        rw[(2 * slot + 1) * S] = (uint64_t)head | ((uint64_t)span << 12) | ((uint64_t)tail << 24) | ((uint64_t)mis << 48);
        cw[i * S] = (w & ~(15u << 27)) | ((uint32_t)slot << 27);
        n_nw += calls; n_cells += cells;
    }
    return true;
}

template <int S, class RD>
__host__ __device__ inline void d_unit_process_rd(const DIndex &ix, const LocTab &lt, const DParams &pr, bool paired, int n1, int n2, int len1, int len2,
                                               const RD seq1, const RD seq2, SKey *key, uint32_t *cw, uint64_t *rw,
                                               bool try_fast, UnitState &st)
{
    d_unit_sort<S>(key, n1);
    if (paired) d_unit_sort<S>(key + n1 * S, n2);
    int k = 0;
    st.nc[0] = d_cluster_seeds(lt, pr, len1, n1, [&](int i) { return key[i * S]; },
                               [&](int first, int count, int score, int64_t) { cw[(k++) * S] = cw_make(first, count, score); });
    st.nc[1] = 0;
    CandLds<S> a{key, cw, st.nc[0]}, b{key + n1 * S, cw + st.nc[0] * S, 0};
    if (paired) {
        st.nc[1] = b.cnt = d_cluster_seeds(lt, pr, len2, n2, [&](int i) { return key[(n1 + i) * S]; },
                                           [&](int first, int count, int score, int64_t) { cw[(k++) * S] = cw_make(first, count, score); });
    }
    PP_STAMP(st.pp, st.pt, 1);
    d_candidate_rules(paired, a, b);
    PP_STAMP(st.pp, st.pt, 2);
    st.fast = false; st.n_cig = 0; st.n_nw = st.n_cells = 0; st.flag0[0] = st.flag0[1] = 0;
    if (!try_fast) return;
    int n_slot = 0;
    uint32_t n_cig = 0, n_nw = 0, n_cells = 0;
    if (!d_unit_reports<S>(ix, lt, pr, true, seq1, len1, key, cw, st.nc[0], rw, n_slot, st.rd[0], n_cig, n_nw, n_cells)) return;
    if (paired && !d_unit_reports<S>(ix, lt, pr, false, seq2, len2, key + n1 * S, cw + st.nc[0] * S, st.nc[1], rw, n_slot, st.rd[1], n_cig, n_nw, n_cells)) return;
    PP_STAMP(st.pp, st.pt, 3);
    RepLds<S> p1{cw, rw, st.nc[0], 0}, p2{cw + st.nc[0] * S, rw, st.nc[1], 0};
    if (paired) {
        d_settle_pair(pr, st.rd[0], p1, st.rd[1], p2);
        d_flag_pair(st.rd[0], p1, st.rd[1], p2);
        d_mapq(st.rd[1], p2);
    } else d_flag_single(st.rd[0], p1);
    d_mapq(st.rd[0], p1);
    st.flag0[0] = p1.flag0; st.flag0[1] = p2.flag0;
    st.fast = true; st.n_cig = n_cig; st.n_nw = n_nw; st.n_cells = n_cells;
    PP_STAMP(st.pp, st.pt, 4);
}
template <int S>
__host__ __device__ inline void d_unit_process(const DIndex &ix, const DParams &pr, bool paired, int n1, int n2, int len1, int len2,
                                               const unsigned char *seq1, const unsigned char *seq2, SKey *key, uint32_t *cw, uint64_t *rw,
                                               bool try_fast, UnitState &st)
{
    d_unit_process_rd<S, ReadAscii>(ix, d_loc_tab(ix), pr, paired, n1, n2, len1, len2, ReadAscii{seq1}, ReadAscii{seq2}, key, cw, rw, try_fast, st);
}

struct CompactOut { dg_read_c *reads; dg_report_c *reports; uint32_t *cigar; unsigned int *bad; };
__host__ __device__ __forceinline__ bool d_compact_read(const dg_read_out &r, dg_read_c &o)
{
    o.score = (uint16_t)r.score; o.sub_score = (uint16_t)r.sub_score; o.mis_num = (uint16_t)r.mis_num; o.mapq = (uint8_t)r.mapq; o.n_sj = (uint8_t)r.n_sj;
    o.n_rep = (uint16_t)r.n_rep; o.best = (uint16_t)r.best;
    return !((uint32_t)r.score > 0xFFFFu || (uint32_t)r.sub_score > 0xFFFFu || (uint32_t)r.mis_num > 0xFFFFu || (uint32_t)r.mapq > 0xFFu || (uint32_t)r.n_sj > 0xFFu ||
             (uint32_t)r.n_rep > 0xFFFFu || (uint32_t)r.best > 0xFFFFu);
}
__host__ __device__ __forceinline__ bool d_compact_report(const dg_report_out &p, bool plain, bool slow, dg_report_c &q)
{
    q.pos = (int32_t)p.pos; q.aln_score = (uint16_t)p.aln_score; q.flag = (uint16_t)p.flag; q.paired_idx = (int16_t)p.paired_idx;
    q.chr = p.chr < 0 ? (uint16_t)0xFFFFu : (uint16_t)p.chr; q.sj_type = (int8_t)p.sj_type; q.bdir = (uint8_t)p.bdir; q.pad = slow ? 1u : 0u;
    q.n_cigar = plain ? (uint8_t)DG_CIGAR_FULL_MATCH : (uint8_t)p.n_cigar;
    return !(p.pos != (int64_t)(int32_t)p.pos || (uint32_t)p.aln_score > 0xFFFFu || (uint32_t)p.flag > 0xFFFFu || p.paired_idx > 32767 || p.paired_idx < -1 ||
             p.chr >= 0xFFFF || p.n_cigar > 254u || p.sj_type < -128 || p.sj_type > 127 || (uint32_t)p.bdir > 1u);
}

template <int S>
__host__ __device__ inline uint32_t d_unit_compact_ops(const DRead &rd, const RepLds<S> &p)
{
    uint32_t n = 0;
    for (int i = 0; i < rd.CanNum; i++) {
        const int s = p.slot(i);
        if (s == 15) continue;
        const uint64_t w0 = p.rw[(2 * s) * S], w1 = p.rw[(2 * s + 1) * S];
        if (!((w0 >> 61) & 1ull)) continue;
        const uint32_t head = (uint32_t)(w1 & 0xFFFu), tail = (uint32_t)((w1 >> 24) & 0xFFFu);
        n += (head || tail) ? 1u + (head > 0) + (tail > 0) : 0u;
    }
    return n;
}

template <int S>
__host__ __device__ inline uint32_t d_unit_emit_read(bool first, const DRead &rd, const RepLds<S> &p, uint32_t rep_off, uint32_t cig_off,
                                                     dg_read_out *rout_r, dg_report_out *reports, uint32_t *cigar, const CompactOut &co = CompactOut{nullptr, nullptr, nullptr, nullptr},
                                                     dg_read_c *rc_r = nullptr, uint32_t cigc_off = 0, bool full = true)
{
    dg_read_out o;
    o.score = rd.score; o.sub_score = rd.sub_score; o.mis_num = rd.mis_num; o.mapq = rd.mapq; o.n_rep = rd.CanNum; o.best = rd.iBest;
    o.rep_off = (int32_t)rep_off; o.sj_off = 0; o.n_sj = 0;
    if (full) *rout_r = o;
    bool fits = true;
    if (co.reads) { dg_read_c oc; fits = d_compact_read(o, oc); *rc_r = oc; }
    uint32_t used = 0, used_c = 0;
    for (int i = 0; i < rd.CanNum; i++) {
        dg_report_out rp;
        rp.aln_score = 0; rp.sj_type = -1; rp.flag = p.flag(i); rp.paired_idx = p.mate(i); rp.chr = -1; rp.bdir = 0; rp.pos = 0;
        rp.cigar_off = cig_off + used; rp.n_cigar = 0;
        const int s = p.slot(i);
        if (s != 15) {
            const uint64_t w0 = p.rw[(2 * s) * S], w1 = p.rw[(2 * s + 1) * S];
            if ((w0 >> 61) & 1ull) {
                rp.aln_score = (int32_t)((w0 >> 48) & 0xFFFu); rp.chr = (int32_t)((w0 >> 32) & 0xFFFFu); rp.bdir = (int32_t)((w0 >> 60) & 1u);
                rp.pos = (int64_t)(w0 & 0xFFFFFFFFull);
                const uint32_t head = (uint32_t)(w1 & 0xFFFu), span = (uint32_t)((w1 >> 12) & 0xFFFu), tail = (uint32_t)((w1 >> 24) & 0xFFFu);
                const bool rev = (rp.bdir != 0) != first;
                const uint32_t lead = rev ? tail : head, trail = rev ? head : tail;
                const uint32_t o_mid = CIG(span, OP_M), o_trail = CIG(trail, OP_S);
                const uint32_t a0 = lead ? CIG(lead, OP_S) : o_mid, a1 = lead ? o_mid : o_trail, a2 = o_trail;
                const uint32_t m = 1u + (lead ? 1u : 0u) + (trail ? 1u : 0u);
                if (full) { uint32_t *c = cigar + cig_off + used; c[0] = a0; if (m > 1) c[1] = a1; if (m > 2) c[2] = a2; }
                rp.n_cigar = m; used += m;
                if (co.reads && m > 1) { uint32_t *c = co.cigar + cigc_off + used_c; c[0] = a0; c[1] = a1; if (m > 2) c[2] = a2; used_c += m; }
            }
        }
        if (full) reports[rep_off + (uint32_t)i] = rp;
        if (co.reads) { dg_report_c q; fits = d_compact_report(rp, rp.n_cigar == 1u, false, q) && fits; co.reports[rep_off + (uint32_t)i] = q; }
    }
    if (co.reads && !fits) *co.bad = 1u;
    return used;
}

#include "dg_scan.h"

__device__ __forceinline__ uint32_t d_pac_touch(const DIndex &ix, SKey k)
{
    const int64_t L = ix.l_pac, g = sk_gpos(k) + sk_rlen(k);
    if (g >= 0 && g + 8 <= L) return *(const uint32_a1 *)(ix.pac + (g >> 2));
    if (g >= L && g + 8 <= 2 * L) return *(const uint32_a1 *)(ix.pac + ((2 * L - 1 - g - 7) >> 2));
    return 0u;
}

template <bool PACKED>
__global__ void __launch_bounds__(PU_THREADS)
k_pair(const DIndex ix, const DParams pr, int n_units, int paired, int try_fast, int write_all_sorted ,
       const unsigned char *__restrict__ seq, const uint32_t *__restrict__ seq_off, const uint32_t *__restrict__ enc, int W2, const uint16_t *__restrict__ rlen,
       const uint32_t *__restrict__ seed_off, SKey *__restrict__ seeds, DCand *__restrict__ cands, uint32_t *__restrict__ ncand,
       uint32_t *__restrict__ rep_off, uint32_t *__restrict__ slow_units,
       dg_read_out *__restrict__ rout, dg_report_out *__restrict__ reports, uint32_t *__restrict__ cigar,
       uint32_t cap_rep, uint32_t cap_cig, TileScan ts, DSizes *sizes, unsigned int *pool_top, unsigned long long *ctr, int *err, const CompactOut co)
{
    const unsigned long long t_wave0 = wall_clock64();
    __shared__ SKey s_key[PU_SEEDS * PU_THREADS];
    __shared__ uint32_t s_cw[PU_SEEDS * PU_THREADS];
    __shared__ uint64_t s_rw[2 * PU_SLOTS * PU_THREADS];
    __shared__ unsigned long long s_scan[20];
    __shared__ unsigned int s_tile;
    __shared__ int64_t s_lkey[PU_LOC_MAX]; __shared__ int64_t s_coff[PU_LOC_MAX / 2]; __shared__ int32_t s_lchr[PU_LOC_MAX];
    const bool tab_in_lds = 2 * ix.n_chr <= PU_LOC_MAX;
    if (tab_in_lds) {
        for (int i = threadIdx.x; i < 2 * ix.n_chr; i += PU_THREADS) { s_lkey[i] = ix.loc_key[i]; s_lchr[i] = ix.loc_chr[i]; }
        for (int i = threadIdx.x; i < ix.n_chr; i += PU_THREADS) s_coff[i] = ix.chr_off[i];
    }
    const LocTab lt = tab_in_lds ? LocTab{s_lkey, s_lchr, s_coff, 2 * ix.n_chr} : d_loc_tab(ix);
    bool leave = false;
    if (threadIdx.x == 0) { const int e0 = __hip_atomic_load(err, __ATOMIC_RELAXED, __HIP_MEMORY_SCOPE_AGENT); leave = e0 == DG_E_SEEDS || e0 == DG_E_SEEDQ || e0 == DG_E_SCAN; }
    const unsigned int tile = d_tile_ticket_unless(ts, &s_tile, leave);
    if (tile == SCAN_LEAVE) return;
    const int u = (int)(tile * PU_THREADS + threadIdx.x);
    const bool valid = u < n_units;
    SKey *key = s_key + threadIdx.x;
    uint32_t *cw = s_cw + threadIdx.x;
    uint64_t *rw = s_rw + threadIdx.x;
    UnitState st;
    st.fast = false; st.n_cig = 0; st.n_nw = st.n_cells = 0; st.nc[0] = st.nc[1] = 0; st.flag0[0] = st.flag0[1] = 0;
#ifdef DG_PAIR_PROF
    for (int i = 0; i < 10; i++) st.pp[i] = 0;
    st.pt = __builtin_amdgcn_s_memtime();
    const unsigned long long pp_t0 = st.pt;
#endif
    int r1 = 0, n1 = 0, n2 = 0, len1 = 0, len2 = 0;
    uint32_t b1 = 0;
    uint32_t pf = 0, pf2 = 0, pf3 = 0, pf4 = 0, pf5 = 0, pf6 = 0;
    bool heavy = false;
    if (valid) {
        r1 = paired ? 2 * u : u;
        len1 = rlen[r1]; len2 = paired ? rlen[r1 + 1] : 0;
        if (PACKED) { pf = enc[(size_t)r1 * 2 * W2 + (W2 >> 1)]; if (paired) pf2 = enc[(size_t)(r1 + 1) * 2 * W2 + (W2 >> 1)]; }
        b1 = seed_off[r1];
        const uint32_t e1 = seed_off[r1 + 1], e2 = paired ? seed_off[r1 + 2] : e1;
        n1 = (int)(e1 - b1); n2 = (int)(e2 - e1);
        heavy = n1 + n2 > PU_SEEDS;
        if (!heavy) {
            const SKey *src = seeds + b1;
            const int nt = n1 + n2;
            for (int i0 = 0; i0 < nt; i0 += 4) {
                const SKey k0 = src[i0], k1 = i0 + 1 < nt ? src[i0 + 1] : 0, k2 = i0 + 2 < nt ? src[i0 + 2] : 0, k3 = i0 + 3 < nt ? src[i0 + 3] : 0;
                key[i0 * PU_THREADS] = k0;
                if (i0 + 1 < nt) key[(i0 + 1) * PU_THREADS] = k1;
                if (i0 + 2 < nt) key[(i0 + 2) * PU_THREADS] = k2;
                if (i0 + 3 < nt) key[(i0 + 3) * PU_THREADS] = k3;
            }
#ifdef __HIP_DEVICE_COMPILE__
            __asm__ volatile("" ::: "memory");
#endif
            if (n1 > 1) { pf3 = d_pac_touch(ix, key[0]); if (n1 > 2) pf4 = d_pac_touch(ix, key[1 * PU_THREADS]); }
            if (n2 > 1) { pf5 = d_pac_touch(ix, key[n1 * PU_THREADS]); if (n2 > 2) pf6 = d_pac_touch(ix, key[(n1 + 1) * PU_THREADS]); }
            PP_STAMP(st.pp, st.pt, 0);
            if (PACKED) {
                const ReadWords a{enc + (size_t)r1 * 2 * W2, W2}, b{enc + (size_t)(r1 + (paired ? 1 : 0)) * 2 * W2, W2};
                d_unit_process_rd<PU_THREADS, ReadWords>(ix, lt, pr, paired != 0, n1, n2, len1, len2, a, b, key, cw, rw, try_fast != 0, st);
            } else d_unit_process_rd<PU_THREADS, ReadAscii>(ix, lt, pr, paired != 0, n1, n2, len1, len2, ReadAscii{seq + seq_off[r1]}, ReadAscii{seq + seq_off[r1 + (paired ? 1 : 0)]}, key, cw, rw, try_fast != 0, st);
        } else { st.nc[0] = (int)ncand[r1]; st.nc[1] = paired ? (int)ncand[r1 + 1] : 0; }
    }
    const uint32_t nrep1 = valid ? (uint32_t)(st.nc[0] > 0 ? st.nc[0] : 1) : 0u, nrep2 = (valid && paired) ? (uint32_t)(st.nc[1] > 0 ? st.nc[1] : 1) : 0u;
    Triple mine, tot;
    mine.x = nrep1 + nrep2; mine.y = (valid && !st.fast) ? 1u : 0u; mine.z = st.fast ? st.n_cig : 0u;
    uint32_t cc1 = 0;
    mine.w = 0;
    if (co.reads && st.fast) {
        RepLds<PU_THREADS> q1{cw, rw, st.nc[0], st.flag0[0]}, q2{cw + st.nc[0] * PU_THREADS, rw, st.nc[1], st.flag0[1]};
        cc1 = d_unit_compact_ops<PU_THREADS>(st.rd[0], q1);
        mine.w = cc1 + (paired ? d_unit_compact_ops<PU_THREADS>(st.rd[1], q2) : 0u);
    }
    PP_STAMP(st.pp, st.pt, 5);
    const Triple inb = d_block_exclusive(mine, tot, s_scan);
    PP_STAMP(st.pp, st.pt, 6);
    const Triple base = d_tile_exclusive(ts, tile, tot, s_scan + 16, err);
    PP_STAMP(st.pp, st.pt, 7);
    const uint32_t rep0 = base.x + inb.x, slow_at = base.y + inb.y;
    const uint64_t cig0 = base.z + inb.z;
    unsigned long long n_cands = 0, n_nw = 0, n_cells = 0;
    if (valid) {
        rep_off[r1] = rep0;
        if (paired) rep_off[r1 + 1] = rep0 + nrep1;
        if (!heavy) n_cands = (unsigned long long)(st.nc[0] + st.nc[1]);
        if (st.fast) {
            if ((uint64_t)rep0 + mine.x > cap_rep) atomicMax(err, DG_E_REPORTS);
            else if (cig0 + st.n_cig > cap_cig) atomicMax(err, DG_E_CIGFINAL);
            else {
                RepLds<PU_THREADS> p1{cw, rw, st.nc[0], st.flag0[0]}, p2{cw + st.nc[0] * PU_THREADS, rw, st.nc[1], st.flag0[1]};
                const uint32_t cigc0 = base.w + inb.w;
                const bool full = !(write_all_sorted & 2) || !co.reads;
                const uint32_t c1 = d_unit_emit_read<PU_THREADS>(true, st.rd[0], p1, rep0, (uint32_t)cig0, rout + r1, reports, cigar, co, co.reads ? co.reads + r1 : nullptr, cigc0, full);
                if (paired) d_unit_emit_read<PU_THREADS>(false, st.rd[1], p2, rep0 + nrep1, (uint32_t)cig0 + c1, rout + r1 + 1, reports, cigar, co, co.reads ? co.reads + r1 + 1 : nullptr, cigc0 + cc1, full);
                n_nw = st.n_nw; n_cells = st.n_cells;
            }
        } else {
            if (slow_at < (uint32_t)n_units) slow_units[slow_at] = (uint32_t)u;
            if ((uint64_t)rep0 + mine.x > cap_rep) atomicMax(err, DG_E_REPORTS);
        }
        if (!heavy && (!st.fast || (write_all_sorted & 1))) {
            const int nt = n1 + n2;
            for (int i = 0; i < nt; i++) seeds[b1 + i] = key[i * PU_THREADS];
            auto put_cands = [&](int first_cw, int first_key, uint32_t seg, int count, int r) {
                for (int i = 0; i < count; i++) {
                    const uint32_t w = cw[(first_cw + i) * PU_THREADS];
                    const int64_t d = sk_diag(key[(first_key + cw_first(w)) * PU_THREADS]);
                    DCand c = d_new_cand(seg + (uint32_t)cw_first(w), cw_count(w), cw_score(w), d < 0 ? 0 : d);
                    c.PairedIdx = cw_mate(w);
                    cands[seg + i] = c;
                }
                ncand[r] = (uint32_t)count;
            };
            put_cands(0, 0, b1, st.nc[0], r1);
            if (paired) put_cands(st.nc[0], n1, b1 + (uint32_t)n1, st.nc[1], r1 + 1);
        } else if (!heavy) { ncand[r1] = (uint32_t)st.nc[0]; if (paired) ncand[r1 + 1] = (uint32_t)st.nc[1]; }
    }
    if (tile == gridDim.x - 1 && threadIdx.x == 0) {
        sizes->total_rep = base.x + tot.x; sizes->n_slow_units = base.y + tot.y; sizes->cig_fast = (uint32_t)(base.z + tot.z);
        sizes->total_cig = sizes->cig_fast;
        sizes->pad[2] = base.w + tot.w;
        *pool_top = (base.x + tot.x) * CIG_SLOT;
    }
    PP_STAMP(st.pp, st.pt, 8);
#ifdef DG_PAIR_PROF
    if ((threadIdx.x & 63) == 0 && (tile % 61u) == 0u)
        printf("kpair tile %u wave %d: total %llu | load %llu sort+cluster %llu rules %llu reports %llu settle %llu rest %llu blockscan %llu lookback %llu emit %llu\n", tile, (int)(threadIdx.x >> 6),
               __builtin_amdgcn_s_memtime() - pp_t0, st.pp[0], st.pp[1], st.pp[2], st.pp[3], st.pp[4], st.pp[5], st.pp[6], st.pp[7], st.pp[8]);
#endif
    if (n_units < 0 && (pf ^ pf2 ^ pf3 ^ pf4 ^ pf5 ^ pf6) == 0x5A17C3E1u) atomicMax(err, DG_E_SCAN);
    d_wave_add(ctr + CTR_CANDS, n_cands);
    d_wave_add(ctr + CTR_NW, n_nw);
    d_wave_add(ctr + CTR_NWCELLS, n_cells);
    d_wave_resident(ctr, CTR_WT_PAIR, t_wave0);
}
```

Baseline: 1175.

## Fuse seed locate into chain and pair kernels, drop k_locate and tile_read

Removes the separate k_locate kernel, which binary-searched each seed's read and walked LF steps to resolve SA positions into a global seeds array. SA resolution now happens inside k_pair (per-thread expansion of hits into register/LDS keys) and k_chain_heavy (per-lane lookups), so one global write and read of the seeds array, one launch and the tile_read mapping are gone. The cost is that LF walks now run inside the pair and chain kernels, which can add latency and register pressure and may load-imbalance threads, since each thread walks its own unit's seeds serially instead of the work being spread evenly across all seeds.

```diff
diff --git a/dart_amd/csrc/dg_api.hip b/dart_amd/csrc/dg_api.hip
--- a/dart_amd/csrc/dg_api.hip
+++ b/dart_amd/csrc/dg_api.hip
@@ -105,7 +105,7 @@
     size_t seq_bytes = 0;
     bool enc_ready = false;
     DBuf<unsigned char> seq; DBuf<uint32_t> seq_off; DBuf<uint16_t> rlen; DBuf<uint32_t> enc; DBuf<uint32_t> packed_in, nlist_in;
-    DBuf<DHit> hits; DBuf<uint32_t> nhits, nseeds, seed_off, ncand, rep_off, tile_sums, tile_read, slow_units;
+    DBuf<DHit> hits; DBuf<uint32_t> nhits, nseeds, seed_off, ncand, rep_off, tile_sums, slow_units;
     DBuf<SKey> seeds; DBuf<DSeed> work; DBuf<DCand> cands; DBuf<DJob> jobs; DBuf<unsigned long long> job_items, job_pool; DBuf<RsChunkOut> job_outs; DBuf<uint32_t> job_pool_next; DBuf<unsigned long long> items; DBuf<uint32_t> hist, heavy; DBuf<DHeavy> seed_heavy; DBuf<int32_t> seed_heavy_sfail; DBuf<int16_t> chain_picks; DBuf<uint8_t> chain_todo;
     DBuf<dg_read_out> reads_out; DBuf<dg_report_out> reports; DBuf<uint32_t> cigpool, cigfinal;
     DBuf<dg_sj_out> sjpool, sjfinal;
@@ -226,7 +226,7 @@
 
 #define SO_PER 8
 __global__ void __launch_bounds__(256)
-k_seed_offsets(int n_reads, int paired, const uint32_t *__restrict__ nseeds, uint32_t *__restrict__ seed_off, uint32_t *__restrict__ tile_read, uint32_t n_tile_read,
+k_seed_offsets(int n_reads, int paired, const uint32_t *__restrict__ nseeds, uint32_t *__restrict__ seed_off,
                uint32_t *__restrict__ heavy_list, unsigned int *n_heavy, uint32_t *total_copy, uint32_t cap, TileScan ts, int *err)
 {
     __shared__ unsigned long long s_scan[20];
@@ -253,10 +253,7 @@
 #pragma unroll
     for (int i = 0; i < SO_PER; i++) {
         const uint32_t r = first + i;
-        if (r < (uint32_t)n_reads) {
-            seed_off[r] = run;
-            for (uint32_t t = (run + 63u) >> 6; (t << 6) < run + v[i] && t < n_tile_read; t++) tile_read[t] = r;
-        }
+        if (r < (uint32_t)n_reads) seed_off[r] = run;
         const bool unit_end = paired ? (i & 1) == 1 : true;
         const uint32_t useeds = paired ? ((i & 1) ? v[i - ((i & 1) ? 1 : 0)] + v[i] : 0u) : v[i];
         const bool heavy = unit_end && r < (uint32_t)n_reads && useeds > (uint32_t)UNIT_MAX_SEEDS;
@@ -528,7 +525,7 @@
     for (void *p : own) if (p) (void)hipFree(p);
     if (c->h_tail) (void)hipHostFree(c->h_tail);
     c->seq.release(); c->seq_off.release(); c->rlen.release(); c->enc.release(); c->packed_in.release(); c->nlist_in.release(); c->hits.release(); c->nhits.release(); c->nseeds.release();
-    c->seed_off.release(); c->ncand.release(); c->rep_off.release(); c->tile_sums.release(); c->tile_read.release(); c->slow_units.release();
+    c->seed_off.release(); c->ncand.release(); c->rep_off.release(); c->tile_sums.release(); c->slow_units.release();
     c->seeds.release(); c->work.release(); c->cands.release(); c->jobs.release(); c->job_items.release(); c->job_outs.release(); c->job_pool.release(); c->job_pool_next.release(); c->items.release(); c->hist.release(); c->heavy.release(); c->seed_heavy.release(); c->seed_heavy_sfail.release(); c->chain_picks.release(); c->chain_todo.release();
     c->reads_out.release(); c->reports.release(); c->cigpool.release(); c->cigfinal.release(); c->sjpool.release(); c->sjfinal.release();
     c->sam_hdr_off.release(); c->sam_qual_off.release(); c->sam_qlen.release(); c->sam_hdr.release(); c->sam_qual.release(); c->sam_text.release(); c->sam_read_off.release(); c->sam_tile.release();
@@ -1106,7 +1103,7 @@
     HIPCHK(c->hits.ensure((size_t)n * H)); HIPCHK(c->nhits.ensure(n)); HIPCHK(c->nseeds.ensure(n)); HIPCHK(c->seed_off.ensure((size_t)n + 1));
     if (c->shared_caps) caps_adopt(c->cap_seeds, c->shared_caps->seeds);
     if (c->cap_seeds < (size_t)n * 3 + 1024) c->cap_seeds = (size_t)n * 3 + 1024;
-    HIPCHK(c->seeds.ensure(c->cap_seeds + 1)); HIPCHK(c->cands.ensure(c->cap_seeds + 1)); HIPCHK(c->tile_read.ensure(c->cap_seeds / 64 + 16));
+    HIPCHK(c->seeds.ensure(c->cap_seeds + 1)); HIPCHK(c->cands.ensure(c->cap_seeds + 1));
     if (timed) c->tname[c->n_t] = "k_encode";
     HIPCHK(launch_seed(c, n, H, timed ? c->ev[c->n_t + 1] : nullptr));
     if (timed) { c->n_t++; TICK("k_seed"); }
@@ -1114,13 +1111,11 @@
         const int paired = (paired_units && (n % 2 == 0)) ? 1 : 0;
         HIPCHK(c->heavy.ensure((size_t)n + 16));
         const TileScan ts_seed = make_tile_scan(c, 0, c->d_tops + TOP_TICKET_SEED, 1);
-        k_seed_offsets<<<(unsigned)((n + 256 * SO_PER - 1) / (256 * SO_PER)), 256, 0, c->stream>>>(n, paired, c->nseeds.p, c->seed_off.p, c->tile_read.p, (uint32_t)c->tile_read.cap,
+        k_seed_offsets<<<(unsigned)((n + 256 * SO_PER - 1) / (256 * SO_PER)), 256, 0, c->stream>>>(n, paired, c->nseeds.p, c->seed_off.p,
                                                                                                  c->heavy.p, c->d_tops + TOP_HEAVY_UNITS, &c->d_sizes->total_seeds, (uint32_t)c->cap_seeds, ts_seed, c->d_err);
         HIPCHK(hipGetLastError());
     }
     if (timed) TICK("seed_offsets");
-    k_locate<<<(unsigned)((c->cap_seeds + 255) / 256), 256, 0, c->stream>>>(c->ix, n, H, c->hits.p, c->tile_read.p, c->seed_off.p, c->seeds.p, c->d_ctr, c->d_err);
-    HIPCHK(hipGetLastError());
     if (timed) TICK("k_locate");
     return DG_OK;
 }
@@ -1204,7 +1199,7 @@
     unsigned int *tops = c->d_tops;
 
     HIPCHK(c->chain_picks.ensure(c->cap_seeds + 16)); HIPCHK(c->chain_todo.ensure((size_t)n_units + 16));
-    k_chain_heavy<<<c->n_cu * c->env_chain_bpc, 64, 0, c->stream>>>(c->ix, c->pr, n_units, paired, c->rlen.p, c->seed_off.p, c->seeds.p, c->cands.p, c->ncand.p,
+    k_chain_heavy<<<c->n_cu * c->env_chain_bpc, 64, 0, c->stream>>>(c->ix, c->pr, n_units, paired, c->rlen.p, c->hits.p, H, c->seed_off.p, c->seeds.p, c->cands.p, c->ncand.p,
                                                      c->heavy.p, tops + TOP_HEAVY_UNITS, c->chain_picks.p, c->chain_todo.p, c->d_ctr, c->d_err);
     k_chain_rules<<<c->n_cu * 4, 64, 0, c->stream>>>(paired, c->seed_off.p, c->cands.p, c->ncand.p, c->heavy.p, tops + TOP_HEAVY_UNITS, c->chain_picks.p, c->chain_todo.p, c->d_err);
     HIPCHK(hipGetLastError());
@@ -1231,7 +1226,7 @@
     const bool packed_pair = c->enc_ready;
     auto launch_pair = [&](auto kernel) {
         kernel<<<(unsigned)((n_units + PU_THREADS - 1) / PU_THREADS), PU_THREADS, 0, c->stream>>>(
-            c->ix, c->pr, n_units, paired, try_fast, (c->want_full || !c->want_compact) ? 0 : 2, c->seq.p, c->seq_off.p, c->enc.p, W2p, c->rlen.p, c->seed_off.p, c->seeds.p, c->cands.p, c->ncand.p, c->rep_off.p,
+            c->ix, c->pr, n_units, paired, try_fast, (c->want_full || !c->want_compact) ? 0 : 2, c->seq.p, c->seq_off.p, c->enc.p, W2p, c->rlen.p, c->hits.p, H, c->seed_off.p, c->seeds.p, c->cands.p, c->ncand.p, c->rep_off.p,
             c->slow_units.p, c->reads_out.p, c->reports.p, c->cigfinal.p, (uint32_t)c->cap_rep, (uint32_t)c->cap_cig, ts_pair, c->d_sizes, tops + TOP_CIG, c->d_ctr, c->d_err, co);
     };
     if (packed_pair) launch_pair(k_pair<true>); else launch_pair(k_pair<false>);
@@ -1832,11 +1827,11 @@
         HIPCHK(c->ncand.ensure(n)); HIPCHK(c->rep_off.ensure((size_t)n + 1)); HIPCHK(c->reads_out.ensure(n));
         HIPCHK(c->heavy.ensure((size_t)n + 16)); HIPCHK(c->slow_units.ensure((size_t)n + 16)); HIPCHK(c->reports.ensure(16)); HIPCHK(c->cigfinal.ensure(16));
         HIPCHK(c->chain_picks.ensure(c->cap_seeds + 16)); HIPCHK(c->chain_todo.ensure((size_t)n + 16));
-        k_chain_heavy<<<c->n_cu * 4, 64, 0, c->stream>>>(c->ix, c->pr, n, 0, c->rlen.p, c->seed_off.p, c->seeds.p, c->cands.p, c->ncand.p, c->heavy.p, c->d_tops + TOP_HEAVY_UNITS, c->chain_picks.p, c->chain_todo.p, c->d_ctr, c->d_err);
+        k_chain_heavy<<<c->n_cu * 4, 64, 0, c->stream>>>(c->ix, c->pr, n, 0, c->rlen.p, c->hits.p, H, c->seed_off.p, c->seeds.p, c->cands.p, c->ncand.p, c->heavy.p, c->d_tops + TOP_HEAVY_UNITS, c->chain_picks.p, c->chain_todo.p, c->d_ctr, c->d_err);
         k_chain_rules<<<c->n_cu * 4, 64, 0, c->stream>>>(0, c->seed_off.p, c->cands.p, c->ncand.p, c->heavy.p, c->d_tops + TOP_HEAVY_UNITS, c->chain_picks.p, c->chain_todo.p, c->d_err);
         const TileScan ts = make_tile_scan(c, scan_tiles_seed(n), c->d_tops + TOP_TICKET_PAIR, 2);
         k_pair<false><<<(unsigned)((n + PU_THREADS - 1) / PU_THREADS), PU_THREADS, 0, c->stream>>>(
-            c->ix, c->pr, n, 0, 0, 1, c->seq.p, c->seq_off.p, c->enc.p, 1, c->rlen.p, c->seed_off.p, c->seeds.p, c->cands.p, c->ncand.p, c->rep_off.p,
+            c->ix, c->pr, n, 0, 0, 1, c->seq.p, c->seq_off.p, c->enc.p, 1, c->rlen.p, c->hits.p, H, c->seed_off.p, c->seeds.p, c->cands.p, c->ncand.p, c->rep_off.p,
             c->slow_units.p, c->reads_out.p, c->reports.p, c->cigfinal.p, 0xFFFFFFFFu, 0xFFFFFFFFu, ts, c->d_sizes, c->d_tops + TOP_CIG, c->d_ctr, c->d_err, CompactOut{nullptr, nullptr, nullptr, nullptr});
         HIPCHK(hipGetLastError());
         k_batch_end<<<1, 256, 0, c->stream>>>(c->d_sizes, c->d_err, c->d_tops, c->d_ctr, c->h_tail);
diff --git a/dart_amd/csrc/dg_chain.h b/dart_amd/csrc/dg_chain.h
--- a/dart_amd/csrc/dg_chain.h
+++ b/dart_amd/csrc/dg_chain.h
@@ -1,5 +1,6 @@
 #pragma once
 #include "dg_common.h"
+#include "dg_fm.h"
 
 __host__ __device__ inline void d_sort_keys(SKey *a, int n)
 {
@@ -258,7 +259,7 @@
 #define CH_LDS_BYTES (CH_LDS_SORT > CH_LDS_PAIR ? CH_LDS_SORT : CH_LDS_PAIR)
 __global__ void __launch_bounds__(64)
 k_chain_heavy(const DIndex ix, const DParams pr, int n_units, int paired, const uint16_t *__restrict__ rlen,
-              const uint32_t *__restrict__ seed_off, SKey *__restrict__ seeds, DCand *__restrict__ cands,
+              const DHit *__restrict__ hits, int H, const uint32_t *__restrict__ seed_off, SKey *__restrict__ seeds, DCand *__restrict__ cands,
               uint32_t *__restrict__ ncand, const uint32_t *__restrict__ heavy_list, const unsigned int *__restrict__ n_heavy_p,
               int16_t *__restrict__ picks, uint8_t *__restrict__ todo, unsigned long long *ctr, const int *__restrict__ abort_p)
 {
@@ -279,6 +280,7 @@
     const int lane = threadIdx.x;
     const unsigned int n_heavy = *n_heavy_p;
     unsigned long long nc_total = 0;
+    LocCtr lc = {0, 0, 0};
     for (unsigned int hi = blockIdx.x; hi < n_heavy; hi += gridDim.x) {
         const int u = (int)heavy_list[hi];
         const int nm = paired ? 2 : 1;
@@ -290,8 +292,9 @@
         for (int m = 0; m < nm; m++) { b[m] = seed_off[r1 + m]; n[m] = seed_off[r1 + m + 1] - b[m]; }
         __syncthreads();
         for (int m = 0; m < nm; m++) {
+            const DHit *hm = hits + (size_t)(r1 + m) * H;
             if (n[m] <= 64) {
-                SKey key = (uint32_t)lane < n[m] ? seeds[b[m] + lane] : ~0ull;
+                SKey key = (uint32_t)lane < n[m] ? d_read_key(ix, hm, (uint32_t)lane, lc) : ~0ull;
                 int mm = 2; while ((uint32_t)mm < n[m]) mm <<= 1;
                 for (int k = 2; k <= mm; k <<= 1)
                     for (int j = k >> 1; j > 0; j >>= 1) {
@@ -304,16 +307,20 @@
                 const int made = d_gen_candidates_wave(lt, pr, rlen[r1 + m], ls, (int)n[m], b[m], cands + b[m], s_pref, s_starts, lane);
                 if (lane == 0) s_n[m] = made;
             } else if (n[m] <= CH_MAXS) {
-                for (uint32_t i = lane; i < n[m]; i += 64) ls[i] = seeds[b[m] + i];
+                for (uint32_t i = lane; i < n[m]; i += 64) ls[i] = d_read_key(ix, hm, i, lc);
                 __syncthreads();
                 d_bitonic_sort_keys(ls, (int)n[m], lane);
                 for (uint32_t i = lane; i < n[m]; i += 64) seeds[b[m] + i] = ls[i];
                 __syncthreads();
                 const int made = d_gen_candidates_wave(lt, pr, rlen[r1 + m], ls, (int)n[m], b[m], cands + b[m], s_pref, s_starts, lane);
                 if (lane == 0) s_n[m] = made;
-            } else if (lane == 0) {
-                d_sort_keys(seeds + b[m], (int)n[m]);
-                s_n[m] = d_gen_candidates(ix, pr, rlen[r1 + m], seeds + b[m], (int)n[m], b[m], cands + b[m]);
+            } else {
+                for (uint32_t i = lane; i < n[m]; i += 64) seeds[b[m] + i] = d_read_key(ix, hm, i, lc);
+                __syncthreads();
+                if (lane == 0) {
+                    d_sort_keys(seeds + b[m], (int)n[m]);
+                    s_n[m] = d_gen_candidates(ix, pr, rlen[r1 + m], seeds + b[m], (int)n[m], b[m], cands + b[m]);
+                }
             }
             __syncthreads();
         }
@@ -363,6 +370,9 @@
         }
     }
     if (lane == 0 && nc_total) atomicAdd(d_ctr_stripe(ctr) + CTR_CANDS, nc_total);
+    d_wave_add(ctr + CTR_LF, lc.lf);
+    d_wave_add(ctr + CTR_LF_ACT, lc.lf_act);
+    d_wave_add(ctr + CTR_SA, lc.sa);
     d_wave_resident(ctr, CTR_WT_CHAIN, t_wave0);
 }
 
diff --git a/dart_amd/csrc/dg_fm.h b/dart_amd/csrc/dg_fm.h
--- a/dart_amd/csrc/dg_fm.h
+++ b/dart_amd/csrc/dg_fm.h
@@ -3,7 +3,7 @@
 
 struct OccBlock { uint4 q0, q1, q2, q3; };
 
-__device__ __forceinline__ OccBlock d_load_block(const DIndex &ix, uint64_t blk)
+__host__ __device__ __forceinline__ OccBlock d_load_block(const DIndex &ix, uint64_t blk)
 {
     const uint4 *p = ix.bwt + (blk << 2);
     OccBlock b;
@@ -11,17 +11,17 @@
     return b;
 }
 
-__device__ __forceinline__ uint64_t d_sel4(uint64_t a0, uint64_t a1, uint64_t a2, uint64_t a3, int i)
+__host__ __device__ __forceinline__ uint64_t d_sel4(uint64_t a0, uint64_t a1, uint64_t a2, uint64_t a3, int i)
 {
     uint64_t lo = (i & 1) ? a1 : a0, hi = (i & 1) ? a3 : a2;
     return (i & 2) ? hi : lo;
 }
-__device__ __forceinline__ uint64_t d_L2(const DIndex &ix, int i)
+__host__ __device__ __forceinline__ uint64_t d_L2(const DIndex &ix, int i)
 {
     return i == 4 ? ix.L2[4] : d_sel4(ix.L2[0], ix.L2[1], ix.L2[2], ix.L2[3], i);
 }
 
-__device__ __forceinline__ void d_plane_counts(const uint4 H, const uint4 Lo, uint32_t hmask, uint32_t o, uint32_t &P, uint32_t &Q)
+__host__ __device__ __forceinline__ void d_plane_counts(const uint4 H, const uint4 Lo, uint32_t hmask, uint32_t o, uint32_t &P, uint32_t &Q)
 {
     const uint32_t wi = o >> 5;
     const uint32_t pm = (2u << (o & 31)) - 1u;
@@ -30,15 +30,15 @@
     const uint32_t m2 = wi == 2 ? pm : (wi > 2 ? 0xFFFFFFFFu : 0u);
     const uint32_t m3 = wi == 3 ? pm : 0u;
     const uint32_t e0 = (H.x ^ hmask) & m0, e1 = (H.y ^ hmask) & m1, e2 = (H.z ^ hmask) & m2, e3 = (H.w ^ hmask) & m3;
-    P = __popc(e0) + __popc(e1) + __popc(e2) + __popc(e3);
-    Q = __popc(e0 & Lo.x) + __popc(e1 & Lo.y) + __popc(e2 & Lo.z) + __popc(e3 & Lo.w);
-}
-
-__device__ __forceinline__ uint4 d_pick4(bool first, const uint4 a, const uint4 b)
+    P = __builtin_popcount(e0) + __builtin_popcount(e1) + __builtin_popcount(e2) + __builtin_popcount(e3);
+    Q = __builtin_popcount(e0 & Lo.x) + __builtin_popcount(e1 & Lo.y) + __builtin_popcount(e2 & Lo.z) + __builtin_popcount(e3 & Lo.w);
+}
+
+__host__ __device__ __forceinline__ uint4 d_pick4(bool first, const uint4 a, const uint4 b)
 {
     return make_uint4(first ? a.x : b.x, first ? a.y : b.y, first ? a.z : b.z, first ? a.w : b.w);
 }
-__device__ __forceinline__ void d_occ_pair(const OccBlock B, int b, uint32_t o, uint64_t &cb, uint64_t &cp)
+__host__ __device__ __forceinline__ void d_occ_pair(const OccBlock B, int b, uint32_t o, uint64_t &cb, uint64_t &cp)
 {
     const bool hi = (b & 2) != 0, lo = (b & 1) != 0;
     uint32_t P, Q;
@@ -49,7 +49,7 @@
     cp = lo ? c_even : c_odd;
 }
 
-__device__ __forceinline__ uint64_t d_lf(const DIndex &ix, uint64_t k)
+__host__ __device__ __forceinline__ uint64_t d_lf(const DIndex &ix, uint64_t k)
 {
     if (k == ix.primary) return 0;
     const uint64_t x = k - (k > ix.primary);
@@ -729,62 +729,75 @@
     }
 }
 
-
-__global__ void __launch_bounds__(256)
-k_locate(const DIndex ix, int n_reads, int H, const DHit *__restrict__ hits, const uint32_t *__restrict__ tile_read,
-         const uint32_t *__restrict__ seed_off, SKey *__restrict__ seeds, unsigned long long *ctr, const int *__restrict__ abort_p)
-{
-    if (*abort_p >= DG_ABORT) return;
-    const uint32_t total = seed_off[n_reads];
-    const int lane = threadIdx.x & 63;
-    const uint32_t tile = blockIdx.x * (blockDim.x >> 6) + (threadIdx.x >> 6);
-    const uint32_t u = (tile << 6) + (uint32_t)lane;
-    unsigned long long lf = 0, lf_act = 0, nsa = 0;
-    if ((tile << 6) < total) {
-        int r0 = (int)tile_read[tile];
-        const uint32_t u_last = (tile << 6) + 63 < total ? (tile << 6) + 63 : total - 1;
-        int r = -1;
-        uint32_t first = 0;
-        while (true) {
-            const int rr = r0 + lane;
-            const uint32_t nxt = rr + 1 <= n_reads ? seed_off[rr + 1] : 0xFFFFFFFFu;
-            int lo = 0;
-#pragma unroll
-            for (int step = 32; step > 0; step >>= 1) {
-                const uint32_t v = __shfl(nxt, lo + step - 1, 64);
-                if (v <= u) lo += step;
+struct LocCtr { unsigned long long lf, lf_act, sa; };
+__host__ __device__ __forceinline__ bool d_hit_located(const DHit &h) { return (h.freq & 0x80000000u) != 0; }
+__host__ __device__ __forceinline__ uint32_t d_hit_rows(const DHit &h) { return h.freq & 0x7FFFFFFFu; }
+__host__ __device__ __forceinline__ uint64_t d_row_walk(const DIndex &ix, uint64_t k, uint32_t &steps)
+{
+    const uint64_t mask = (uint64_t)(ix.sa_dense ? ix.sa_dense_intv : ix.sa_intv) - 1;
+    steps = 0;
+    while (k & mask) { k = d_lf(ix, k); steps++; }
+    return k;
+}
+__host__ __device__ __forceinline__ uint64_t d_row_entry(const DIndex &ix, uint64_t k)
+{
+    return ix.sa_dense ? ix.sa_dense[k >> ix.sa_dense_shift] : ix.sa[k >> __builtin_ctz((uint32_t)ix.sa_intv)];
+}
+__host__ __device__ __forceinline__ int64_t d_row_pos(const DIndex &ix, uint64_t e, uint32_t steps, LocCtr &c)
+{
+    c.sa++; c.lf_act += steps;
+    if (ix.sa_dense) { c.lf += steps + (e >> 40); return (int64_t)(steps + (e & 0xFFFFFFFFFFull) - 1); }
+    c.lf += steps;
+    return (int64_t)(steps + e);
+}
+__host__ __device__ __forceinline__ SKey d_hit_key(const DIndex &ix, const DHit &h, uint32_t w, LocCtr &c)
+{
+    if (d_hit_located(h)) { c.sa++; return sk_make((int64_t)h.x0, (int)h.rPos, (int)h.len); }
+    uint32_t steps;
+    const uint64_t k = d_row_walk(ix, h.x0 + w, steps);
+    return sk_make(d_row_pos(ix, d_row_entry(ix, k), steps, c), (int)h.rPos, (int)h.len);
+}
+__host__ __device__ __forceinline__ SKey d_read_key(const DIndex &ix, const DHit *h, uint32_t u, LocCtr &c)
+{
+    uint32_t w = u, fr = d_hit_rows(*h);
+    while (w >= fr) { w -= fr; h++; fr = d_hit_rows(*h); }
+    return d_hit_key(ix, *h, w, c);
+}
+template <int S>
+__host__ __device__ __forceinline__ void d_expand_hits(const DIndex &ix, const DHit *hits_r, int n, SKey *key, LocCtr &lc)
+{
+    const uint4 zero_hit = make_uint4(0u, 0u, 0u, 0u);
+    const uint4 *h = (const uint4 *)hits_r;
+    int made = 0;
+#pragma unroll 1
+    while (made < n) {
+        const int want = n - made < 4 ? n - made : 4;
+        const uint4 q0 = h[0], q1 = want > 1 ? h[1] : zero_hit, q2 = want > 2 ? h[2] : zero_hit, q3 = want > 3 ? h[3] : zero_hit;
+        h += want;
+#pragma unroll 1
+        for (int q = 0; q < want && made < n; q++) {
+            const bool lo = q < 2, ev = (q & 1) == 0;
+            DHit hv;
+            hv.x0 = d_u64(lo ? (ev ? q0.x : q1.x) : (ev ? q2.x : q3.x), lo ? (ev ? q0.y : q1.y) : (ev ? q2.y : q3.y));
+            hv.freq = lo ? (ev ? q0.z : q1.z) : (ev ? q2.z : q3.z);
+            const uint32_t pl = lo ? (ev ? q0.w : q1.w) : (ev ? q2.w : q3.w);
+            hv.rPos = (uint16_t)(pl & 0xFFFFu); hv.len = (uint16_t)(pl >> 16);
+            if (d_hit_located(hv)) { lc.sa++; key[made * S] = sk_make((int64_t)hv.x0, (int)hv.rPos, (int)hv.len); made++; continue; }
+            const uint32_t rows = d_hit_rows(hv) < (uint32_t)(n - made) ? d_hit_rows(hv) : (uint32_t)(n - made);
+#pragma unroll 1
+            for (uint32_t w = 0; w < rows; w += 4) {
+                const uint32_t nw = rows - w < 4 ? rows - w : 4;
+                uint32_t s0 = 0, s1 = 0, s2 = 0, s3 = 0;
+                const uint64_t k0 = d_row_walk(ix, hv.x0 + w, s0), k1 = nw > 1 ? d_row_walk(ix, hv.x0 + w + 1, s1) : k0, k2 = nw > 2 ? d_row_walk(ix, hv.x0 + w + 2, s2) : k0,
+                               k3 = nw > 3 ? d_row_walk(ix, hv.x0 + w + 3, s3) : k0;
+                const uint64_t e0 = d_row_entry(ix, k0), e1 = d_row_entry(ix, k1), e2 = d_row_entry(ix, k2), e3 = d_row_entry(ix, k3);
+                SKey *dst = key + made * S;
+                dst[0] = sk_make(d_row_pos(ix, e0, s0, lc), (int)hv.rPos, (int)hv.len);
+                if (nw > 1) dst[1 * S] = sk_make(d_row_pos(ix, e1, s1, lc), (int)hv.rPos, (int)hv.len);
+                if (nw > 2) dst[2 * S] = sk_make(d_row_pos(ix, e2, s2, lc), (int)hv.rPos, (int)hv.len);
+                if (nw > 3) dst[3 * S] = sk_make(d_row_pos(ix, e3, s3, lc), (int)hv.rPos, (int)hv.len);
+                made += (int)nw;
             }
-            if (__shfl(nxt, lo, 64) <= u) lo++;
-            const uint32_t win_end = __shfl(nxt, 63, 64);
-            if (r < 0 && u < total && lo < 64) { r = r0 + lo; first = seed_off[r]; }
-            if (win_end > u_last) break;
-            r0 += 64;
-        }
-        if (u < total) {
-            uint32_t w = u - first;
-            const DHit *h = hits + (size_t)r * H;
-            uint32_t fr = h->freq;
-            while (w >= (fr & 0x7FFFFFFFu)) { w -= fr & 0x7FFFFFFFu; h++; fr = h->freq; }
-            uint64_t k = h->x0 + w;
-            uint64_t steps = 0, pos;
-            if (fr & 0x80000000u) pos = h->x0;
-            else if (ix.sa_dense) {
-                const uint64_t mask = (uint64_t)ix.sa_dense_intv - 1;
-                while (k & mask) { k = d_lf(ix, k); steps++; }
-                const uint64_t e = ix.sa_dense[k >> ix.sa_dense_shift];
-                pos = steps + (e & 0xFFFFFFFFFFull) - 1;
-                lf += steps + (e >> 40); lf_act += steps;
-            } else {
-                const uint64_t mask = (uint64_t)ix.sa_intv - 1;
-                while (k & mask) { k = d_lf(ix, k); steps++; }
-                pos = steps + ix.sa[k / (uint64_t)ix.sa_intv];
-                lf += steps; lf_act += steps;
-            }
-            nsa++;
-            seeds[u] = sk_make((int64_t)pos, (int)h->rPos, (int)h->len);
-        }
-    }
-    d_wave_add(ctr + CTR_LF, lf);
-    d_wave_add(ctr + CTR_LF_ACT, lf_act);
-    d_wave_add(ctr + CTR_SA, nsa);
-}
+        }
+    }
+}
diff --git a/dart_amd/csrc/dg_pair.h b/dart_amd/csrc/dg_pair.h
--- a/dart_amd/csrc/dg_pair.h
+++ b/dart_amd/csrc/dg_pair.h
@@ -427,6 +427,7 @@
 __global__ void __launch_bounds__(PU_THREADS)
 k_pair(const DIndex ix, const DParams pr, int n_units, int paired, int try_fast, int write_all_sorted ,
        const unsigned char *__restrict__ seq, const uint32_t *__restrict__ seq_off, const uint32_t *__restrict__ enc, int W2, const uint16_t *__restrict__ rlen,
+       const DHit *__restrict__ hits, int H ,
        const uint32_t *__restrict__ seed_off, SKey *__restrict__ seeds, DCand *__restrict__ cands, uint32_t *__restrict__ ncand,
        uint32_t *__restrict__ rep_off, uint32_t *__restrict__ slow_units,
        dg_read_out *__restrict__ rout, dg_report_out *__restrict__ reports, uint32_t *__restrict__ cigar,
@@ -465,6 +466,7 @@
     uint32_t b1 = 0;
     uint32_t pf = 0, pf2 = 0, pf3 = 0, pf4 = 0, pf5 = 0, pf6 = 0;
     bool heavy = false;
+    LocCtr lc = {0, 0, 0};
     if (valid) {
         r1 = paired ? 2 * u : u;
         len1 = rlen[r1]; len2 = paired ? rlen[r1 + 1] : 0;
@@ -474,15 +476,9 @@
         n1 = (int)(e1 - b1); n2 = (int)(e2 - e1);
         heavy = n1 + n2 > PU_SEEDS;
         if (!heavy) {
-            const SKey *src = seeds + b1;
-            const int nt = n1 + n2;
-            for (int i0 = 0; i0 < nt; i0 += 4) {
-                const SKey k0 = src[i0], k1 = i0 + 1 < nt ? src[i0 + 1] : 0, k2 = i0 + 2 < nt ? src[i0 + 2] : 0, k3 = i0 + 3 < nt ? src[i0 + 3] : 0;
-                key[i0 * PU_THREADS] = k0;
-                if (i0 + 1 < nt) key[(i0 + 1) * PU_THREADS] = k1;
-                if (i0 + 2 < nt) key[(i0 + 2) * PU_THREADS] = k2;
-                if (i0 + 3 < nt) key[(i0 + 3) * PU_THREADS] = k3;
-            }
+#pragma unroll 1
+            for (int m = 0; m < (paired ? 2 : 1); m++)
+                d_expand_hits<PU_THREADS>(ix, hits + (size_t)(r1 + m) * H, m ? n2 : n1, key + (m ? n1 : 0) * PU_THREADS, lc);
 #ifdef __HIP_DEVICE_COMPILE__
             __asm__ volatile("" ::: "memory");
 #endif
@@ -562,6 +558,9 @@
                __builtin_amdgcn_s_memtime() - pp_t0, st.pp[0], st.pp[1], st.pp[2], st.pp[3], st.pp[4], st.pp[5], st.pp[6], st.pp[7], st.pp[8]);
 #endif
     if (n_units < 0 && (pf ^ pf2 ^ pf3 ^ pf4 ^ pf5 ^ pf6) == 0x5A17C3E1u) atomicMax(err, DG_E_SCAN);
+    d_wave_add(ctr + CTR_LF, lc.lf);
+    d_wave_add(ctr + CTR_LF_ACT, lc.lf_act);
+    d_wave_add(ctr + CTR_SA, lc.sa);
     d_wave_add(ctr + CTR_CANDS, n_cands);
     d_wave_add(ctr + CTR_NW, n_nw);
     d_wave_add(ctr + CTR_NWCELLS, n_cells);
```

Measured after the change: 1141. 0.971x the previous value.
